# rail-berkeley/serl

Measured on AMD Instinct MI355X. Metric: learner grad-steps/sec (DrQ, bs256, 2x128x128 img), higher is better.
Workload: dtype f32 (trunk convs as split-fp16 MFMA x3, fp32 accumulate; <=1e-6 vs fp64); 1 GPU; async_drq_sim (DrQ, ResNet-10 frozen trunk, REDQ-10 critic); workload_key=drq, global_batch=256, per_gpu_batch=256, cameras=2, state_dim=24, act_dim=6, replay_capacity=200000, replay_fill=20000, parallelism=dp1, encoder=resnet-pretrained, trunk_passes_per_grad_step=2, trunk_arithmetic=f16x3, schedule=trunk(i+1) overlapped with update(i) on a 2nd stream; gather(i+2) on a 3rd

## Files before the change

### serl_amd/csrc/agent.hip

```cpp
#include <algorithm>
#include <cmath>
#include <cstdlib>
#include <cstring>
#include <string>
#include <vector>

#include "dense_layer.h"
#include "small_encoder.h"

using namespace serl;

namespace {

constexpr int kL = SERL_MAX_MLP_LAYERS;
inline int critic_smax(int layer) { return layer == 0 ? 4 : 2; }
inline int policy_smax(int layer) { return layer == 0 ? 8 : 4; }

struct Offs {
  long enc0, cam_stride;
  DenseLn cam, prop;
  DenseLn c[kL], a[kL];
  int nc, na;
  long c_hw, c_hb;
  long a_Wm, a_bm, a_Ws, a_bs;
// ... 216 lines not shown
    e.rstd = b.take<float>((long)c.n_cam * B);
    e.pxhat = b.take<float>(B * c.proprio_dim);
    e.prstd = b.take<float>(B);
    e.enc = nullptr; e.ld = 0;
  };
  enc(a->encP); enc(a->encT); enc(a->encO);
  float* encP_out = b.take<float>(B * a->E);
  a->encP.enc = encP_out; a->encP.ld = a->E;
  auto mlp = [&](MlpBuf& m, long rows, const serl_mlp_opts& net) {
    for (int j = 0; j < net.n_layers; ++j) {
      LayerBuf* l = &m.l[j];
      l->h = b.take<float>(rows * net.dims[j]); l->xhat = b.take<float>(rows * net.dims[j]); l->rstd = b.take<float>(rows);
    }
  };
  auto crit = [&](CritBuf& cb) {
    cb.x = b.take<float>(B * a->XA);
    mlp(cb.m, N * B, critic);
    cb.q = b.take<float>(N * B);
  };
  crit(a->critT); crit(a->crit);
  a->encT.enc = a->critT.x; a->encT.ld = a->XA;
  a->encO.enc = a->crit.x; a->encO.ld = a->XA;
  for (PolBuf* pbuf : {&a->pol, &a->polT}) {
    mlp(pbuf->m, B, policy);
    pbuf->pre = b.take<float>(2 * B * A); pbuf->std = b.take<float>(B * A); pbuf->logp = b.take<float>(B);
  }
  const long Bp = pad64(B);
  long cap = std::max<long>({(long)c.n_cam * 32 * Bp * c.bottleneck, N * Bp * pad64(a->XA), 8 * Bp * Wp, 4 * N * Bp * Wc, 16L * 64 * Hc});
  a->slabs_cap = cap;
  for (int k = 0; k < 3; ++k) a->slabs_lane[k] = b.take<float>(cap);
  a->slabs = a->slabs_lane[0];
  a->dq = b.take<float>(N * B); a->ytgt = b.take<float>(B);
  for (int j = std::max(critic.n_layers, policy.n_layers) - 1; j >= 0; --j) {
    const long n = std::max<long>(j < critic.n_layers ? N * B * critic.dims[j] : 0, j < policy.n_layers ? B * policy.dims[j] : 0);
    GradBuf* s = &a->s[j];
    s->dy = b.take<float>(n); s->dpre = b.take<float>(n); s->dg = b.take<float>(n);
  }
  a->dx = b.take<float>(B * a->XA);
  a->scam.dpre = b.take<float>((long)c.n_cam * B * c.bottleneck);
  a->scam.dg = b.take<float>((long)c.n_cam * B * c.bottleneck);
  a->df = b.take<float>((long)c.n_cam * B * a->D);
  a->sle_part = b.take<float>((long)c.n_cam * kSleSplit * a->HW * 512 * c.sle_features);
  a->sprop.dpre = b.take<float>(B * c.proprio_dim); a->sprop.dg = b.take<float>(B * c.proprio_dim);
  a->dpre = b.take<float>(2 * B * A); a->sprop.dy = b.take<float>(B * c.proprio_dim);
  for (int k = 0; k < 3; ++k) {
    a->eps_buf[k] = b.take<float>(B * A);
    a->mask_buf[k] = b.take<uint8_t>((long)c.n_cam * B * a->D);
  }
  a->act_tmp = b.take<float>(B * A);
  a->ctr = b.take<int>((long)kCtrPerLane * kCtrLanes);
  a->labels = b.take<float>(B); a->label_logits = b.take<float>(B); a->label_mean = b.take<float>(1);
  a->label_ctr = b.take<int>(1);
  a->eval_info = b.take<float>(8);
  if (a->small) {
    void* smem = b.take<uint8_t>(small_workspace_bytes(c.n_cam * c.batch, c.H, c.W, c.num_stack));
    if (base) small_workspace_bind(a->sws, smem, c.n_cam * c.batch, c.H, c.W, c.num_stack);
  } else if (!a->state_only) {
    const int nimg = 2 * c.n_cam * c.batch;
    void* tmem = b.take<uint8_t>(trunk_workspace_bytes(nimg, c.H, c.W));
    if (base) trunk_workspace_bind(a->tws, tmem, nimg, c.H, c.W);
    void* pmem = b.take<uint8_t>(trunk_packed_bytes());
    if (base) trunk_packed_bind(a->tpk, pmem);
    if (a->live) {
      static_assert(sizeof(a->feats_t_slot) / sizeof(a->feats_t_slot[0]) == serl_agent::kSlots + 1, "one target-feature buffer per slot");
      void* pmem_t = b.take<uint8_t>(trunk_packed_bytes());
      if (base) trunk_packed_bind(a->tpk_t, pmem_t);
      for (int k = 0; k <= serl_agent::kSlots; ++k) a->feats_t_slot[k] = b.take<float>((long)c.n_cam * B * a->HW * 512);
      a->feats_t = a->feats_t_slot[0];
    }
  }
  (void)persistent;
  return b.off;
}

int split_for(long agent_budget, int M, int N, int groups, int smax, long budget = 0) {
  if (budget <= 0) budget = agent_budget > 0 ? agent_budget : 512L;
  return split_under(M, N, groups, smax, budget);
}

struct EncJob {
  const float* P;
  int which;
  const uint8_t* mask;
  EncBuf* e;
  const float* act_src;
  float* act_dst;
  int gen_mask = 0;
  uint64_t mask_seed = 0;
  const uint32_t* tf_key = nullptr; long tf_rows = 0, tf_row0 = 0;
  const float* x = nullptr;
};
DenseLnIo cam_io(const serl_agent* a, const EncBuf& e) {
  return DenseLnIo{e.f, a->D, (long)a->cfg.batch * a->D, e.enc, e.ld, a->cfg.bottleneck, e.xhat, e.rstd};
}
DenseLnIo prop_io(const serl_agent* a, const EncBuf& e, const float* state) {
  return DenseLnIo{state, a->cfg.state_dim, 0, e.enc + (long)a->cfg.n_cam * a->cfg.bottleneck, e.ld, 0, e.pxhat, e.prstd};
}
int encode_multi(serl_agent* a, const EncJob* jobs, int n, int off, int cnt, hipStream_t st) {
  const serl_agent_cfg& c = a->cfg;
  const Offs& o = a->o;
  const long Bfull = a->cur.batch;
  SERL_REQUIRE(n >= 1 && n <= 3, "bad encode instance count");
  if (a->state_only) {
    CopyJob cj[kMaxMulti];
    int m = 0;
    for (int i = 0; i < n; ++i) {
      const EncJob& j = jobs[i];
      cj[m++] = CopyJob{a->cur.state + ((long)j.which * Bfull + off) * c.state_dim, c.state_dim, j.e->enc, j.e->ld, c.state_dim};
      if (j.act_dst) cj[m++] = CopyJob{j.act_src, c.act_dim, j.act_dst, a->XA, c.act_dim};
    }
    return copy_cols_multi(cj, m, cnt, st);
  }
  SleFwdArgs sv[3];
  GemmDesc gd[3];
  LnFwdArgs lv[3];
  ProprioArgs pv[3];
  const int S = split_for(a->split_budget, cnt, c.bottleneck, c.n_cam * n, 32);
  for (int i = 0; i < n; ++i) {
    const EncJob& j = jobs[i];
    EncBuf& e = *j.e;
    sv[i] = SleFwdArgs{};
    sv[i].x = (j.x ? j.x : a->feats + ((long)j.which * c.n_cam) * c.batch * a->HW * 512) + (long)off * a->HW * 512;
    sv[i].K = j.P + o.enc0;
    sv[i].mask = j.mask ? j.mask + (long)off * a->D : nullptr;
    sv[i].f = e.f;
    gd[i] = layer_fwd(o.cam, j.P, cam_io(a, e), cnt, a->slabs_lane[i], S);
    lv[i] = layer_ln_fwd(o.cam, j.P, cam_io(a, e), cnt, gd[i]);
    ProprioArgs& pr = pv[i];
    pr = layer_row_fwd(o.prop, j.P, prop_io(a, e, a->cur.state + ((long)j.which * Bfull + off) * c.state_dim));
    if (j.act_dst) {
      pr.copy_src = j.act_src; pr.ld_copy_src = c.act_dim; pr.copy_dst = j.act_dst; pr.ld_copy_dst = a->XA;
      pr.copy_cols = c.act_dim;
    }
  }
  if (a->fuse) {
    for (int i = 0; i < n; ++i) {
      sv[i].gen = jobs[i].gen_mask; sv[i].seed = jobs[i].mask_seed;
      sv[i].row_offset = a->shard_off + off; sv[i].rows_global = a->shard_global ? a->shard_global : Bfull;
      if (jobs[i].gen_mask == 2) sle_tf_masks(sv[i], jobs[i].tf_key, c.n_cam, jobs[i].tf_rows, jobs[i].tf_row0);
    }
  }
  if (a->small) {
    const size_t fbytes = (size_t)c.H * c.W * 3;
    for (int i = 0; i < n; ++i) {
      const EncJob& j = jobs[i];
      int dup = -1;
      for (int k = i + 1; k < n; ++k)
        if (jobs[k].P == j.P && jobs[k].which == j.which) dup = k;
      if (dup >= 0) { gd[i].A = jobs[dup].e->f; continue; }
      const uint8_t* fr = a->cur.frames + (((size_t)j.which * c.n_cam) * Bfull + off) * c.num_stack * fbytes;
      RC(small_forward(a->sws, j.P, o.enc0, o.cam_stride, fr, Bfull, c.n_cam, cnt, j.e->f, (long)c.batch * a->D, st));
    }
  } else if (a->fuse) {
    RC(sle_proprio_fwd_multi(sv, pv, n, 1.0f - c.dropout, cnt, a->HW, 512, c.n_cam, (long)c.batch * a->HW * 512, o.cam_stride,
                             Bfull * a->D, (long)c.batch * a->D, c.state_dim, st));
  } else {
    RC(sle_fwd_multi(sv, n, 1.0f / (1.0f - c.dropout), cnt, a->HW, 512, c.n_cam, (long)c.batch * a->HW * 512, o.cam_stride,
                     Bfull * a->D, (long)c.batch * a->D, st));
  }
  RC(gemm_f32_multi(gd, n, st));
  RC(ln_fwd_multi(lv, n, c.bottleneck, st));
  if (a->fuse && !a->small) return SERL_OK;
  return proprio_fwd_multi(pv, n, c.state_dim, cnt, st);
}

DenseLnIo mlp_io(const DenseLn& L, const float* x, long ldx, const LayerBuf& b, int rows) {
  return DenseLnIo{x, ldx, 0, b.h, L.N, (long)rows * L.N, b.xhat, b.rstd};
}
DenseLnIo mlp_io(const DenseLn& L, const LayerBuf& below, const LayerBuf& b, int rows) {
  return DenseLnIo{below.h, L.K, L.groups > 1 ? (long)rows * L.K : 0, b.h, L.N, (long)rows * L.N, b.xhat, b.rstd};
}
DenseLnGrad mlp_grad(const DenseLn& L, const GradBuf& s, int rows, bool dy_here = true) {
  return DenseLnGrad{dy_here ? s.dy : nullptr, L.N, (long)rows * L.N, s.dpre, s.dg};
}

struct RowDot { const float *w, *b; float* out; long w_gs, b_gs; };
struct LayerJob { const float* P; DenseLnIo t; RowDot dot; DenseLnDrop drop; };
int dense_ln_multi(serl_agent* a, const DenseLn& L, const LayerJob* jobs, int n, int rows, int smax, hipStream_t st) {
  SERL_REQUIRE(n >= 1 && n <= 3, "bad dense instance count");
  const int splitk = split_for(a->split_budget, rows, L.N, L.groups * n, smax);
  SERL_REQUIRE((long)L.groups * splitk * rows * L.N <= a->slabs_cap,
               "Dense layer: %d groups x %d K-splits x %d rows x width %d exceeds the slab scratch of %ld floats", L.groups, splitk,
               rows, L.N, a->slabs_cap);
  GemmDesc gd[3];
  LnFwdArgs lv[3];
  for (int i = 0; i < n; ++i) {
    const LayerJob& j = jobs[i];
    gd[i] = layer_fwd(L, j.P, j.t, rows, a->slabs_lane[i], splitk);
    lv[i] = layer_ln_fwd(L, j.P, j.t, rows, gd[i], j.drop);
    lv[i].dot_w = j.dot.w; lv[i].dot_b = j.dot.b; lv[i].dot_out = j.dot.out;
    lv[i].dot_gstride = j.dot.w_gs; lv[i].dot_b_gstride = j.dot.b_gs;
  }
  RC(gemm_f32_multi(gd, n, st));
  return ln_fwd_multi(lv, n, L.N, st);
}

struct PolJob {
  const float* P; PolBuf* pb;
  const float* enc; long ld_enc;
  const float* eps;
  float* act_out; long ld_act;
  float* sum_logp;
  float* alpha_out;
  float* eps_out = nullptr; uint64_t eps_seed = 0; long eps_row0 = 0;
  const uint32_t* tf_key = nullptr; long tf_rows = 0, tf_row0 = 0;
  DenseLnDrop drop[kL] = {};
};
int policy_mlp_multi(serl_agent* a, const PolJob* jobs, int n, int cnt, hipStream_t st) {
  const Offs& o = a->o;
  for (int l = 0; l < o.na; ++l) {
    LayerJob d[3];
    for (int i = 0; i < n; ++i) {
      const PolJob& j = jobs[i];
      MlpBuf& m = j.pb->m;
      d[i] = LayerJob{j.P, l ? mlp_io(o.a[l], m.l[l - 1], m.l[l], cnt) : mlp_io(o.a[0], j.enc, j.ld_enc, m.l[0], cnt), {}, j.drop[l]};
    }
    RC(dense_ln_multi(a, o.a[l], d, n, cnt, policy_smax(l), st));
  }
  return SERL_OK;
}
inline long head_stride(const serl_agent* a) { return a->o.a_bs >= 0 ? a->o.a_bs - a->o.a_bm : a->cfg.act_dim; }
inline const float* head_bias_ls(const serl_agent* a, const float* P) { return a->o.a_bs >= 0 ? P + a->o.a_bs : a->fixed_std_dev; }
int policy_fwd_multi(serl_agent* a, const PolJob* jobs, int n, int cnt, hipStream_t st) {
  const serl_agent_cfg& c = a->cfg;
  const Offs& o = a->o;
  const int Hd = o.a[o.na - 1].N, A = c.act_dim;
  SERL_REQUIRE(n >= 1 && n <= 3, "bad policy instance count");
  GemmDesc gd[3];
  PolicyDistArgs pv[3];
  for (int i = 0; i < n; ++i) {
    const PolJob& j = jobs[i];
    const float* P = j.P;
    PolBuf& pb = *j.pb;
    gd[i] = gemm_fwd(pb.m.l[o.na - 1].h, Hd, 0, P + o.a_Wm, head_stride(a), a->slabs_lane[i], a->head_groups, cnt, A, Hd, 4);
    pv[i] = PolicyDistArgs{};
    pv[i].mode = a->pol_mode;
    pv[i].slabs = a->slabs_lane[i]; pv[i].S = 4; pv[i].bias_mean = P + o.a_bm; pv[i].bias_ls = head_bias_ls(a, P); pv[i].pre = pb.pre;
    pv[i].eps = j.eps; pv[i].act = j.act_out; pv[i].ld_act = j.ld_act; pv[i].logp = pb.logp; pv[i].std_out = pb.std;
    pv[i].sum_logp = j.sum_logp; pv[i].lam = P + o.lam; pv[i].alpha_out = j.alpha_out;
  }
  RC(policy_mlp_multi(a, jobs, n, cnt, st));
  if (a->fuse) {
    SERL_REQUIRE(A <= 64, "the fused policy-head epilogue holds one 64-wide slab row per sample (act_dim %d)", A);
    SERL_REQUIRE(cdiv(cnt, 64) <= kCtrPerLane && 8 * pad64(cnt) * 64 <= a->slabs_cap, "policy head exceeds the fused epilogue's scratch");
    for (int i = 0; i < n; ++i) {
      const PolJob& j = jobs[i];
      GemmDesc& g = gd[i];
      g.ldc = 64; g.sCz = pad64(cnt) * 64;
      g.epi = kEpiPolicy; g.ctr = a->ctr + (long)i * kCtrPerLane;
      g.pd = pv[i];
      g.pd.sum_logp = nullptr;
      g.pd.eps_out = j.eps_out; g.pd.seed = j.eps_seed; g.pd.row_offset = j.eps_row0;
      g.pd.tf = j.tf_key ? 1 : 0;
      if (j.tf_key) { g.pd.tf_key[0] = j.tf_key[0]; g.pd.tf_key[1] = j.tf_key[1]; g.pd.tf_rows = j.tf_rows; g.pd.tf_row0 = j.tf_row0; }
      g.pd.B = cnt; g.pd.A = A; g.pd.std_min = c.std_min; g.pd.std_max = c.std_max;
      g.pd.slab_ld = g.ldc; g.pd.slab_stride = g.sCz;
      SERL_REQUIRE(j.eps || j.eps_out, "policy noise: neither draws nor a buffer for hashed ones");
      if (j.sum_logp) {
        SERL_REQUIRE(a->pg_defer && a->pg_ncs < kMaxColsum, "no room for the log-prob sum job");
        a->pg_cs[a->pg_ncs++] = Colsum3Args{j.pb->logp, nullptr, nullptr, 1, cnt, 1, nullptr, j.sum_logp, nullptr, 0, 2};
      }
    }
    return gemm_f32_multi(gd, n, st);
  }
  RC(gemm_f32_multi(gd, n, st));
  return policy_dist_fwd_multi(pv, n, cnt, A, c.std_min, c.std_max, st);
}

struct CritJob { const float* P; CritBuf* cb; DenseLnDrop drop[kL]; };
int critic_fwd_multi(serl_agent* a, const CritJob* jobs, int n, int cnt, hipStream_t st) {
  const Offs& o = a->o;
  SERL_REQUIRE(n >= 1 && n <= 3, "bad critic instance count");
  for (int l = 0; l < o.nc; ++l) {
    LayerJob d[3];
    for (int i = 0; i < n; ++i) {
      const float* P = jobs[i].P;
      CritBuf& cb = *jobs[i].cb;
      d[i] = LayerJob{P, l ? mlp_io(o.c[l], cb.m.l[l - 1], cb.m.l[l], cnt) : mlp_io(o.c[0], cb.x, a->XA, cb.m.l[0], cnt), {}, jobs[i].drop[l]};
      if (l == o.nc - 1)
        d[i].dot = RowDot{P + o.c_hw, P + o.c_hb, cb.q, a->state_only ? o.c[l].N : 0, a->state_only ? 1 : 0};
    }
    RC(dense_ln_multi(a, o.c[l], d, n, cnt, critic_smax(l), st));
  }
  return SERL_OK;
}

int flush_param_grads(serl_agent* a, hipStream_t st) {
  if (a->pg_ncs) RC(colsum3_multi(a->pg_cs, a->pg_ncs, st));
  if (a->pg_nwg) RC(gemm_f32_multi(a->pg_wg, a->pg_nwg, st));
  a->pg_ncs = a->pg_nwg = 0;
  return SERL_OK;
}

int wgrad(serl_agent* a, const GemmDesc& g, hipStream_t st) {
  if (a->pg_defer && a->pg_nwg < kMaxGemmGroups) {
    a->pg_wg[a->pg_nwg++] = g;
    return SERL_OK;
  }
  return gemm_f32(g, st);
}

struct HeadDq {
  const float* dq; const float* w; float dq_const; long w_gs; const LossArgs* loss;
};
int dense_ln_bwd(serl_agent* a, const DenseLn& L, const float* P, const DenseLnIo& t, const DenseLnGrad& d, int rows, float* G,
                 hipStream_t st, const HeadDq* head = nullptr, const DenseLnDrop& site = DenseLnDrop{}) {
  LnBwdArgs l = layer_ln_bwd(L, P, t, d, rows, site);
  if (head) { l.dq = head->dq; l.dq_w = head->w; l.dq_const = head->dq_const; l.dq_w_gstride = head->w_gs; }
  if (head && head->loss) {
    l.dq_inline = 1;
    RC(ln_bwd_multi(&l, 1, *head->loss, st));
  } else {
    RC(ln_bwd(l, st));
  }
  if (!G) return SERL_OK;
  const Colsum3Args cs = layer_colsum(L, t, d, rows, G);
  if (a->pg_defer && a->pg_ncs < kMaxColsum) a->pg_cs[a->pg_ncs++] = cs;
  else RC(colsum3_multi(&cs, 1, st));
  return wgrad(a, layer_wgrad(L, t, d, rows, G), st);
}


int igrad_sum(serl_agent* a, GemmDesc g, float* out, long ldo, hipStream_t st) {
  const int groups = g.nbatch, rows = g.M, Kin = g.N;
  g.C = a->slabs;
  if (!a->fuse) {
    g.ldc = Kin; g.sCz = (long)rows * Kin;
    RC(gemm_f32(g, st));
    return reduce_slabs(a->slabs, groups, (long)rows * Kin, 1, rows, Kin, nullptr, 0, out, ldo, 0, false, st);
  }
  g.ldc = pad64(Kin); g.sCz = pad64(rows) * g.ldc;
  g.epi = kEpiReduce; g.zred = groups; g.ctr = a->ctr; g.out = out; g.ld_out = ldo; g.out_gstride = 0;
  SERL_REQUIRE((long)cdiv(rows, 64) * cdiv(Kin, 64) <= kCtrPerLane && groups * g.sCz <= a->slabs_cap,
               "input gradient: %d groups x %d rows x %d columns exceeds the fused epilogue's slab scratch of %ld floats, or its tiles the %d "
               "arrival counters", groups, rows, Kin, a->slabs_cap, kCtrPerLane);
  return gemm_f32(g, st);
}

int head_kernel_grad(serl_agent* a, CritBuf& cb, int cnt, hipStream_t st) {
  const int Hd = a->o.c[a->o.nc - 1].N, N = a->cfg.ensemble;
  const int groups = a->state_only ? N : 1, K = a->state_only ? cnt : N * cnt, split = K <= 1024 ? 1 : (a->state_only ? 4 : 8);
  float* out = a->Gc + a->o.c_hw;
  GemmDesc g{};
  g.A = a->dq; g.sAm = a->fuse ? 1 : 0; g.sAk = 1; g.sAb = a->state_only ? cnt : 0;
  g.B = cb.m.l[a->o.nc - 1].h; g.sBk = Hd; g.sBn = 1; g.sBb = a->state_only ? (long)cnt * Hd : 0;
  g.C = split == 1 ? out : a->slabs; g.ldc = Hd; g.sCz = Hd;
  g.M = 1; g.N = Hd; g.K = K; g.nbatch = groups; g.splitk = split;
  if (!a->fuse) {
    RC(gemm_f32(g, st));
    return split == 1 ? SERL_OK : reduce_slabs(a->slabs, split, Hd, groups, 1, Hd, nullptr, 0, out, Hd, a->state_only ? Hd : 0, false, st);
  }
  if (split > 1) {
    g.sCz = 64L * Hd;
    g.epi = kEpiReduce; g.zred = split; g.ctr = a->ctr; g.out = out; g.ld_out = Hd; g.out_gstride = Hd;
    SERL_REQUIRE((long)groups * split * g.sCz <= a->slabs_cap && groups * cdiv(Hd, 64) <= kCtrPerLane,
                 "head gradient: %d groups x %d K-splits x 64 rows x width %d exceeds the slab scratch of %ld floats, or its %d tiles the %d "
                 "arrival counters", groups, split, Hd, a->slabs_cap, groups * cdiv(Hd, 64), kCtrPerLane);
  }
  SERL_REQUIRE(a->pg_defer && a->pg_nwg < kMaxGemmGroups, "no room for the deferred head-gradient GEMM");
  a->pg_wg[a->pg_nwg++] = g;
  return SERL_OK;
}

int critic_loss_or_rider(serl_agent* a, const LossArgs& L, hipStream_t st, const LossArgs** rider) {
  *rider = nullptr;
  if (a->fuse) { *rider = &L; return SERL_OK; }
  return critic_loss(L.qt, L.q, L.reward, L.mask, L.sel, L.E, L.B, L.discount, L.inv_norm, L.y_out, L.dq, L.scalars, L.dbias, st,
                     L.per_member != 0, L.logp_next, L.alpha);
}

int head_bias_grad(serl_agent* a, int cnt, float* out, long out_gstride, hipStream_t st) {
  const int A = a->cfg.act_dim;
  const int groups = a->opts.std_param == SERL_STD_FIXED ? 1 : 2;
  if (!a->fuse) return colsum(a->dpre, nullptr, groups, cnt, A, out, out_gstride, false, st);
  SERL_REQUIRE(a->pg_ncs < kMaxColsum, "no room for the head-bias gradient job");
  a->pg_cs[a->pg_ncs++] = Colsum3Args{a->dpre, nullptr, nullptr, groups, cnt, A, nullptr, out, nullptr, out_gstride, 1};
  return SERL_OK;
}

int critic_bwd(serl_agent* a, const float* P, CritBuf& cb, int cnt, bool pg, hipStream_t st, const LossArgs* loss, float dq_const,
               const DenseLnDrop* sites) {
  const Offs& o = a->o;
  float* G = pg ? a->Gc : nullptr;
  const LossArgs* rider = nullptr;
  if (loss) RC(critic_loss_or_rider(a, *loss, st, &rider));
  if (pg) RC(head_kernel_grad(a, cb, cnt, st));
  const int top = o.nc - 1;
  const HeadDq head{loss ? loss->dq : nullptr, P + o.c_hw, dq_const, a->state_only ? o.c[top].N : 0, rider};
  for (int l = top; l >= 0; --l) {
    const DenseLnGrad d = mlp_grad(o.c[l], a->s[l], cnt, l != top);
    const DenseLnIo t = l ? mlp_io(o.c[l], cb.m.l[l - 1], cb.m.l[l], cnt) : mlp_io(o.c[0], cb.x, a->XA, cb.m.l[0], cnt);
    RC(dense_ln_bwd(a, o.c[l], P, t, d, cnt, G, st, l == top ? &head : nullptr, sites[l]));
    if (l) RC(gemm_f32(layer_igrad(o.c[l], P, d, cnt, mlp_grad(o.c[l - 1], a->s[l - 1], cnt)), st));
    else return igrad_sum(a, layer_igrad(o.c[0], P, d, cnt, nullptr, 0, 0), a->dx, a->XA, st);
  }
  return SERL_OK;
}

int enc_bwd_critic(serl_agent* a, const float* P, EncBuf& e, int off, int cnt, hipStream_t st, void* event_bucket0) {
  const serl_agent_cfg& c = a->cfg;
  const Offs& o = a->o;
  const DenseLnIo tc = cam_io(a, e), tp = prop_io(a, e, a->cur.state + (long)off * c.state_dim);
  const DenseLnGrad dc{a->dx, a->XA, o.cam.N, a->scam.dpre, a->scam.dg};
  const DenseLnGrad dp{a->dx + (long)c.n_cam * o.cam.N, a->XA, 0, a->sprop.dpre, a->sprop.dg};
  if (a->fuse && !a->state_only) {
    LnBwdArgs lb[2] = {layer_ln_bwd(o.cam, P, tc, dc, cnt), layer_ln_bwd(o.prop, P, tp, dp, cnt)};
    RC(ln_bwd_multi(lb, 2, LossArgs{}, st));
    SERL_REQUIRE(a->pg_defer && a->pg_ncs + 2 <= kMaxColsum, "no room for the deferred LayerNorm gradients");
    a->pg_cs[a->pg_ncs++] = layer_colsum(o.prop, tp, dp, cnt, a->Gc);
    a->pg_cs[a->pg_ncs++] = layer_colsum(o.cam, tc, dc, cnt, a->Gc);
    RC(wgrad(a, layer_wgrad(o.prop, tp, dp, cnt, a->Gc), st));
  } else if (!a->state_only) {
    RC(dense_ln_bwd(a, o.prop, P, tp, dp, cnt, a->Gc, st));
  }
  if (event_bucket0) {
    RC(flush_param_grads(a, st));
    SERL_HIP(hipEventRecord((hipEvent_t)event_bucket0, st));
  }
  if (a->state_only) return SERL_OK;
  if (a->fuse) RC(wgrad(a, layer_wgrad(o.cam, tc, dc, cnt, a->Gc), st));
  else RC(dense_ln_bwd(a, o.cam, P, tc, dc, cnt, a->Gc, st));
  RC(gemm_f32(layer_igrad(o.cam, P, dc, cnt, a->df, a->D, (long)cnt * a->D), st));
  if (a->small)
    return small_backward(a->sws, P, o.enc0, o.cam_stride, c.n_cam, cnt, a->df, (long)cnt * a->D, a->Gc, st);
  const long sle_n = (long)a->HW * 512 * c.sle_features;
  const float* x = a->feats + (long)off * a->HW * 512;
  if (a->fuse) {
    SERL_REQUIRE((long)c.n_cam * a->HW * 2 <= kCtrPerLane, "SLE gradient exceeds the arrival counters");
    return sle_bwd_fused(x, a->df, a->sle_part, cnt, a->HW, 512, kSleSplit, c.n_cam, (long)c.batch * a->HW * 512, (long)cnt * a->D,
                         (long)kSleSplit * sle_n, a->Gc + o.enc0, o.cam_stride, a->ctr, st);
  }
  RC(sle_bwd(x, a->df, a->sle_part, cnt, a->HW, 512, kSleSplit, c.n_cam, (long)c.batch * a->HW * 512,
             (long)cnt * a->D, (long)kSleSplit * sle_n, st));
  return reduce_slabs(a->sle_part, kSleSplit, sle_n, c.n_cam, 1, (int)sle_n, nullptr, 0, a->Gc + o.enc0, sle_n,
                      o.cam_stride, false, st);
}

static long tf_row0_of(const serl_agent* a, int cnt) {
  return a->shard_global ? (a->shard_off * (long)cnt) / std::max<long>(a->cur.batch, 1) : 0;
}

struct PhaseNoise {
  const float* eps; float* eps_out;
  const uint32_t* tf_eps; uint64_t eps_seed;
  const uint8_t* mask; uint8_t* mask_out;
  int gen_mask; const uint32_t* tf_mask; uint64_t mask_seed;
};
PhaseNoise draw_noise(serl_agent* a, const float* given_eps, const uint8_t* given_mask, int slot, const uint32_t* key_eps,
                      const uint32_t* key_mask) {
  const serl_agent_cfg& c = a->cfg;
  PhaseNoise z{};
  z.eps = given_eps; z.eps_out = a->eps_buf[slot];
  z.mask_out = a->mask_buf[slot];
  if (!given_eps) {
    if (key_eps) z.tf_eps = key_eps;
    else z.eps_seed = c.seed ^ (0xA5A5ull + 7919ull * (++a->noise_ctr));
  }
  if (given_mask || a->state_only || a->small) z.mask = a->small ? nullptr : given_mask;
  else if (key_mask) { z.gen_mask = 2; z.tf_mask = key_mask; }
  else { z.gen_mask = 1; z.mask_seed = c.seed ^ (0x5A5Aull + 104729ull * (++a->noise_ctr)); }
  return z;
}
int materialise_noise(serl_agent* a, PhaseNoise* v, int n, int off, int cnt, long global_count, hipStream_t st) {
  if (a->fuse) return SERL_OK;
  const serl_agent_cfg& c = a->cfg;
  const long rows = a->cur.batch, row0 = tf_row0_of(a, cnt);
  NoiseJob gen[kMaxMulti];
  int ngen = 0;
  for (int i = 0; i < n; ++i) {
    PhaseNoise& z = v[i];
    serl_jax_job jobs[1 + SERL_MAX_CAMS];
    int nj = 0;
    if (!z.eps && z.tf_eps) {
      serl_jax_job& j = jobs[nj++];
      j = serl_jax_job{};
      j.key[0] = z.tf_eps[0]; j.key[1] = z.tf_eps[1]; j.kind = SERL_JAX_NORMAL;
      j.n_total = global_count * c.act_dim; j.first = row0 * c.act_dim; j.count = (long)cnt * c.act_dim;
      j.out = z.eps_out + (long)off * c.act_dim;
    } else if (!z.eps) {
      gen[ngen++] = NoiseJob{z.eps_out, rows * c.act_dim, z.eps_seed, 0, 0.f, rows, a->shard_global, a->shard_off, c.act_dim};
    }
    for (int k = 0; k < c.n_cam && z.gen_mask == 2; ++k) {
      serl_jax_job& j = jobs[nj++];
      j = serl_jax_job{};
      j.key[0] = z.tf_mask[2 * k]; j.key[1] = z.tf_mask[2 * k + 1]; j.kind = SERL_JAX_BERNOULLI_U8; j.p = 1.0f - c.dropout;
      j.n_total = global_count * a->D; j.first = row0 * a->D; j.count = (long)cnt * a->D;
      j.out = z.mask_out + ((long)k * rows + off) * a->D;
    }
    if (z.gen_mask == 1)
      gen[ngen++] = NoiseJob{z.mask_out, (long)c.n_cam * rows * a->D, z.mask_seed, 1, 1.0f - c.dropout, rows, a->shard_global, a->shard_off, a->D};
    if (nj) RC(serl_jax_fill(c.device, jobs, nj, (void*)st));
    z = PhaseNoise{z.eps ? z.eps : z.eps_out, z.eps_out, nullptr, 0, z.gen_mask ? z.mask_out : z.mask, z.mask_out, 0, nullptr, 0};
  }
  return ngen ? gen_noise_multi(gen, ngen, st) : SERL_OK;
}
void set_noise(const serl_agent* a, EncJob& e, PolJob& p, const PhaseNoise& z, long off, int cnt, long global_count) {
  const int A = a->cfg.act_dim;
  const long tf_row0 = tf_row0_of(a, cnt);
  e.mask = z.mask; e.gen_mask = z.gen_mask; e.mask_seed = z.mask_seed;
  e.tf_key = z.tf_mask; e.tf_rows = global_count; e.tf_row0 = tf_row0;
  p.eps = z.eps ? z.eps + off * A : nullptr;
  p.eps_out = z.eps_out + off * A; p.eps_seed = z.eps_seed; p.eps_row0 = a->shard_off + off;
  p.tf_key = z.tf_eps; p.tf_rows = global_count; p.tf_row0 = tf_row0;
}

void mlp_sites(serl_agent* a, int site, double rate, int off, int cnt, long global_count, int key_row, DenseLnDrop (&out)[kL]) {
  for (DenseLnDrop& d : out) d = DenseLnDrop{};
  if (!(rate > 0.0)) return;
  const serl_mlp_noise& z = a->mlp_cur;
  const bool critic = site == SERL_SITE_Q_TARGET || site == SERL_SITE_Q_ONLINE || site == SERL_SITE_Q_ACTOR;
  const serl_mlp_opts& net = critic ? a->opts.critic : a->opts.policy;
  const int* dims = net.dims;
  const int n = net.n_layers;
  long below = 0;
  for (int l = 0; l < n; below += dims[l], ++l) {
    DenseLnDrop& d = out[l];
    d.train = 1;
    if (z.mask[site]) d.mask = z.mask[site] + below * a->cur.batch + (long)off * dims[l];
    else if (z.key[site]) { d.key = z.key[site] + ((long)key_row * n + l) * 2; d.key_rows = global_count; d.key_row0 = tf_row0_of(a, cnt); }
    else { d.seed = a->cfg.seed ^ (0xD0D0ull + 15485863ull * (++a->noise_ctr)); d.hash_row0 = a->shard_off + off; }
  }
}
int mlp_masks_fit(const serl_agent* a) {
  for (int s = 0; s < SERL_MLP_SITES; ++s)
    SERL_REQUIRE(!a->mlp_cur.mask[s] || a->mlp_cur.mask_rows == a->cur.batch,
                 "serl_mlp_noise: the masks of site %d hold %d rows per layer, the batch has %d", s, a->mlp_cur.mask_rows, a->cur.batch);
  return SERL_OK;
}
struct MlpNoiseScope {
  serl_agent* a;
  explicit MlpNoiseScope(serl_agent* a_) : a(a_) {
    if (a && a->mlp_depth++ == 0) { a->mlp_cur = a->mlp_bound; a->mlp_bound = serl_mlp_noise{}; }
  }
  ~MlpNoiseScope() {
    if (a && --a->mlp_depth == 0) a->mlp_cur = serl_mlp_noise{};
  }
};

float lr_at(const serl_agent_cfg& c, int64_t count, int tx) {
  const float peak = (c.tx_lr_set[tx] || c.tx_lr[tx] > 0.f) ? c.tx_lr[tx] : c.lr;
  int warm = (tx == SERL_TX_TEMPERATURE && c.temp_warmup_steps >= 0) ? c.temp_warmup_steps : c.warmup_steps;
  if (c.tx_warmup[tx] > 0) warm = c.tx_warmup[tx] - 1;
  if (count < warm) return (float)((double)peak * (double)count / (double)warm);
  if (c.tx_cosine_steps[tx] > 0) {
    const double T = (double)std::max(c.tx_cosine_steps[tx] - warm, 1);
    const double k = std::min((double)(count - warm), T);
    return (float)((double)peak * 0.5 * (1.0 + std::cos(M_PI * k / T)));
// ... 479 lines not shown
}

static int check_label_fresh(serl_agent* a) {
  if (!a->cls) return SERL_OK;
  const bool mine = a->trunk_gen != a->attach_gen, theirs = classifier_view(a->cls).trunk_gen != a->attach_cls_gen;
  if (mine || theirs) {
    set_error("stale reward-classifier attachment: a trunk leaf of the %s was set after serl_agent_set_reward_classifier; attach again",
              mine ? "agent" : "classifier");
    return SERL_ERR_STATE;
  }
  return SERL_OK;
}

int serl_agent_set_reward_classifier(serl_agent* a, serl_classifier* cls, const int* cam_of, int* mode_out) {
  SERL_REQUIRE(a, "NULL agent");
  if (!cls) {
    a->cls = nullptr;
    a->label_mode = SERL_LABEL_NONE;
    a->labelled = false;
    if (mode_out) *mode_out = SERL_LABEL_NONE;
    return SERL_OK;
  }
  SERL_REQUIRE(cam_of, "NULL camera map");
  const serl_agent_cfg& c = a->cfg;
  SERL_REQUIRE(!a->state_only, "a state-only agent has no frames for a reward classifier to label");
  SERL_REQUIRE(c.num_stack == 1, "the reward classifier reads single frames (its pretrained conv_init takes 3 channels): an agent with num_stack %d "
               "cannot be labelled by it", c.num_stack);
  const ClassifierView v = classifier_view(cls);
  SERL_REQUIRE(v.cfg.device == c.device, "the classifier lives on device %d, the agent on %d", v.cfg.device, c.device);
  for (int k = 0; k < v.cfg.n_cam; ++k)
    SERL_REQUIRE(cam_of[k] >= 0 && cam_of[k] < c.n_cam, "classifier camera %d maps to agent camera %d, the agent has %d", k, cam_of[k], c.n_cam);
  SERL_REQUIRE(v.cfg.H == c.H && v.cfg.W == c.W, "the classifier takes %dx%d images, the agent %dx%d", v.cfg.H, v.cfg.W, c.H, c.W);
  SERL_REQUIRE(v.cfg.max_batch >= c.batch, "classifier max_batch %d is below the agent's batch %d", v.cfg.max_batch, c.batch);
  SERL_HIP(hipSetDevice(c.device));
  int mode = SERL_LABEL_FRAMES;
  if (!a->small && !a->live && v.trunk_count == a->trunk_count) {
    SERL_HIP(hipDeviceSynchronize());
    std::vector<float> mine(a->trunk_count), theirs(a->trunk_count);
    SERL_HIP(hipMemcpy(mine.data(), a->trunk, sizeof(float) * mine.size(), hipMemcpyDeviceToHost));
    SERL_HIP(hipMemcpy(theirs.data(), v.trunk, sizeof(float) * theirs.size(), hipMemcpyDeviceToHost));
    if (std::memcmp(mine.data(), theirs.data(), sizeof(float) * mine.size()) == 0) mode = SERL_LABEL_FEATURES;
  }
  a->cls = cls;
  for (int k = 0; k < v.cfg.n_cam; ++k) a->cls_cam[k] = cam_of[k];
  a->label_mode = mode;
  a->attach_gen = a->trunk_gen;
  a->attach_cls_gen = v.trunk_gen;
  a->labelled = false;
  if (mode_out) *mode_out = mode;
  return SERL_OK;
}

int serl_agent_label_rewards(serl_agent* a, void* stream) {
  SERL_REQUIRE(a && a->has_batch, "serl_agent_encode / serl_agent_select_slot must run first");
  if (!a->cls) {
    set_error("no reward classifier is attached (serl_agent_set_reward_classifier)");
    return SERL_ERR_STATE;
  }
  RC(check_label_fresh(a));
  const serl_agent_cfg& c = a->cfg;
  hipStream_t st = (hipStream_t)stream;
  SERL_HIP(hipSetDevice(c.device));
  const int n = a->cur.batch, nc = classifier_view(a->cls).cfg.n_cam;
  SERL_HIP(hipMemsetAsync(a->label_ctr, 0, sizeof(int), st));
  if (a->label_mode == SERL_LABEL_FEATURES) {
    const long cam_stride = (long)c.batch * a->HW * 512;
    RC(classifier_label(a->cls, a->feats + c.n_cam * cam_stride, cam_stride, a->cls_cam, nullptr, n, a->labels, a->label_logits,
                        a->label_mean, a->label_ctr, st));
  } else {
    const size_t fbytes = (size_t)c.H * c.W * 3;
    const uint8_t* cams[SERL_MAX_CAMS];
    for (int k = 0; k < nc; ++k) cams[k] = a->cur.frames + ((size_t)(c.n_cam + a->cls_cam[k]) * n) * fbytes;
    RC(classifier_label(a->cls, nullptr, 0, nullptr, cams, n, a->labels, a->label_logits, a->label_mean, a->label_ctr, st));
  }
  a->label_n = n;
  a->labelled = true;
  return SERL_OK;
}

int serl_agent_reward_label_rows(serl_agent* a) { return a ? a->label_n : -1; }

int serl_agent_read_reward_labels(serl_agent* a, float* host_labels, float* host_logits, float* mean_out, void* stream) {
  SERL_REQUIRE(a, "NULL agent");
  SERL_REQUIRE(a->label_n > 0, "no rewards were labelled yet");
  hipStream_t st = (hipStream_t)stream;
  SERL_HIP(hipSetDevice(a->cfg.device));
  const size_t bytes = sizeof(float) * a->label_n;
  if (host_labels) SERL_HIP(hipMemcpyAsync(host_labels, a->labels, bytes, hipMemcpyDeviceToHost, st));
  if (host_logits) SERL_HIP(hipMemcpyAsync(host_logits, a->label_logits, bytes, hipMemcpyDeviceToHost, st));
  if (mean_out) SERL_HIP(hipMemcpyAsync(mean_out, a->label_mean, sizeof(float), hipMemcpyDeviceToHost, st));
  SERL_HIP(hipStreamSynchronize(st));
  return SERL_OK;
}

int serl_agent_critic_grads(serl_agent* a, int off, int cnt, int global_count, const serl_noise* noise,
                            int redq_row, void* stream) {
  return serl_agent_critic_grads_bucketed(a, off, cnt, global_count, noise, redq_row, stream, nullptr);
}

int serl_agent_grad_bucket(serl_agent* a, int bucket, float** dev_ptr, int64_t* count) {
  SERL_REQUIRE(a && dev_ptr && count, "NULL argument");
  SERL_REQUIRE(bucket == 0 || bucket == 1, "bucket must be 0 or 1");
  const Offs& o = a->o;
  if (bucket == 0) { *dev_ptr = a->Gc + o.c[0].W; *count = (o.Pc - o.c[0].W) + kScalars; }
  else { *dev_ptr = a->Gc; *count = o.c[0].W; }
  return SERL_OK;
}

int serl_agent_critic_grads_bucketed(serl_agent* a, int off, int cnt, int global_count, const serl_noise* noise,
                                     int redq_row, void* stream, void* event_bucket0) {
  MlpNoiseScope mlp_scope(a);
  SERL_REQUIRE(a && a->has_batch, "serl_agent_encode must run first");
  SERL_REQUIRE(off >= 0 && cnt >= 1 && off + cnt <= a->cur.batch && global_count >= cnt, "bad minibatch range");
  RC(mlp_masks_fit(a));
  if (a->cls && !a->labelled && !a->label_exempt) {
    set_error("a reward classifier is attached: serl_agent_label_rewards must follow serl_agent_select_slot (vice.py:594)");
    return SERL_ERR_STATE;
  }
  const serl_agent_cfg& c = a->cfg;
  const Offs& o = a->o;
  hipStream_t st = (hipStream_t)stream;
  SERL_HIP(hipSetDevice(c.device));
  const int m_sub = c.critic_subsample_size == 0 ? 2 : (c.critic_subsample_size < 0 ? 0 : c.critic_subsample_size);
  SERL_REQUIRE(m_sub <= 16, "critic_subsample_size %d exceeds 16", m_sub);
  RedqSel sel{};
  sel.n = m_sub;
  if (noise && noise->redq_idx) {
    for (int k = 0; k < m_sub; ++k) sel.idx[k] = noise->redq_idx[m_sub * redq_row + k];
  } else {
    uint64_t r = c.seed * 0x9E3779B97F4A7C15ull + (++a->noise_ctr) * 0xBF58476D1CE4E5B9ull;
    for (int k = 0; k < m_sub; ++k) {
      r ^= r >> 29; r *= 0x94D049BB133111EBull; r ^= r >> 32;
      sel.idx[k] = (int)(r % c.ensemble);
      r += 0x9E3779B97F4A7C15ull;
    }
  }
  for (int k = 0; k < m_sub; ++k) SERL_REQUIRE(sel.idx[k] >= 0 && sel.idx[k] < c.ensemble, "REDQ index out of range");
  a->pg_ncs = a->pg_nwg = 0;
  a->pg_defer = true;
  const int A = c.act_dim;
  PhaseNoise nz = draw_noise(a, noise ? noise->eps_next : nullptr, noise ? noise->mask_next : nullptr, 0,
                             noise && noise->key_eps_next ? noise->key_eps_next + 2 * redq_row : nullptr,
                             noise && noise->key_mask_next ? noise->key_mask_next + 2 * c.n_cam * redq_row : nullptr);
  RC(materialise_noise(a, &nz, 1, off, cnt, global_count, st));
  RC(live_features(a, off, cnt, true, st));
  EncJob ej[3] = {{a->theta, 1, nullptr, &a->encP, nullptr, nullptr},
                  {a->theta_t, 1, nullptr, &a->encT, nullptr, nullptr},
                  {a->theta, 0, nullptr, &a->encO, a->cur.action + (long)off * A, a->crit.x + a->E}};
  if (a->live) ej[1].x = a->feats_t;
  PolJob pj{a->theta, &a->pol, a->encP.enc, a->encP.ld, nullptr, a->critT.x + a->E, a->XA, nullptr,
            c.backup_entropy ? a->aux + X_ALPHA : nullptr};
  set_noise(a, ej[0], pj, nz, off, cnt, global_count);
  CritJob cj[2] = {{a->theta_t, &a->critT, {}}, {a->theta, &a->crit, {}}};
  mlp_sites(a, SERL_SITE_PI_NEXT, a->opts.policy.dropout, off, cnt, global_count, redq_row, pj.drop);
  mlp_sites(a, SERL_SITE_Q_TARGET, a->opts.critic.dropout, off, cnt, global_count, redq_row, cj[0].drop);
  mlp_sites(a, SERL_SITE_Q_ONLINE, a->opts.critic.dropout, off, cnt, global_count, redq_row, cj[1].drop);
  RC(encode_multi(a, ej, 3, off, cnt, st));
  RC(policy_fwd_multi(a, &pj, 1, cnt, st));
  RC(critic_fwd_multi(a, cj, 2, cnt, st));
  const float* reward = a->labelled ? a->labels : a->cur.reward;
  const LossArgs L{1, a->critT.q, a->crit.q, reward + off, a->cur.mask + off, sel, c.ensemble, cnt, c.discount,
                   1.0f / ((float)c.ensemble * (float)global_count), a->ytgt, a->dq, a->SC, a->Gc + o.c_hb, a->state_only ? 1 : 0,
                   c.backup_entropy ? a->pol.logp : nullptr, c.backup_entropy ? a->aux + X_ALPHA : nullptr};
  SERL_REQUIRE(!a->state_only || c.ensemble <= 16, "per-member head bias supports ensembles of at most 16");
  RC(critic_bwd(a, a->theta, a->crit, cnt, true, st, &L, 0.f, cj[1].drop));
  RC(enc_bwd_critic(a, a->theta, a->encO, off, cnt, st, event_bucket0));
  RC(flush_param_grads(a, st));
  a->last_global = global_count;
  return SERL_OK;
}

int serl_agent_actor_grads(serl_agent* a, int global_count, const serl_noise* noise, void* stream) {
  MlpNoiseScope mlp_scope(a);
  SERL_REQUIRE(a && a->has_batch, "serl_agent_encode must run first");
  const serl_agent_cfg& c = a->cfg;
  const Offs& o = a->o;
  hipStream_t st = (hipStream_t)stream;
  SERL_HIP(hipSetDevice(c.device));
  const int cnt = a->cur.batch, A = c.act_dim, top = o.na - 1, Hd = o.a[top].N;
  SERL_REQUIRE(global_count >= cnt, "global_count < local batch");
  RC(mlp_masks_fit(a));
  a->pg_ncs = a->pg_nwg = 0;
  a->pg_defer = true;
  enum { PI = 0, TEMP = 1 };
  PhaseNoise nz[2] = {draw_noise(a, noise ? noise->eps_pi : nullptr, noise ? noise->mask_obs_pi : nullptr, 1,
                                 noise ? noise->key_eps_pi : nullptr, noise ? noise->key_mask_obs_pi : nullptr),
                      draw_noise(a, noise ? noise->eps_temp : nullptr, noise ? noise->mask_next_temp : nullptr, 2,
                                 noise ? noise->key_eps_temp : nullptr, noise ? noise->key_mask_next_temp : nullptr)};
  RC(materialise_noise(a, nz, 2, 0, cnt, global_count, st));
  RC(live_features(a, 0, cnt, false, st));
  EncJob ej[3] = {{a->theta, 1, nullptr, &a->encT, nullptr, nullptr},
                  {a->theta, 0, nullptr, &a->encO, nullptr, nullptr},
                  {a->theta, 0, nullptr, &a->encP, nullptr, nullptr}};
  PolJob pj[2] = {{a->theta, &a->polT, a->encT.enc, a->encT.ld, nullptr, a->act_tmp, A, a->SC + S_LOGP_NEXT, a->aux + X_ALPHA},
                  {a->theta, &a->pol, a->encP.enc, a->encP.ld, nullptr, a->crit.x + a->E, a->XA, a->SC + S_LOGP, nullptr}};
  set_noise(a, ej[0], pj[0], nz[TEMP], 0, cnt, global_count);
  set_noise(a, ej[2], pj[1], nz[PI], 0, cnt, global_count);
  CritJob cj{a->theta, &a->crit, {}};
  mlp_sites(a, SERL_SITE_PI, a->opts.policy.dropout, 0, cnt, global_count, 0, pj[1].drop);
  mlp_sites(a, SERL_SITE_Q_ACTOR, a->opts.critic.dropout, 0, cnt, global_count, 0, cj.drop);
  mlp_sites(a, SERL_SITE_PI_TEMP, a->opts.policy.dropout, 0, cnt, global_count, 0, pj[0].drop);
  RC(encode_multi(a, ej, 3, 0, cnt, st));
  RC(policy_fwd_multi(a, pj, 2, cnt, st));
  const float* eps_pi = nz[PI].eps ? nz[PI].eps : nz[PI].eps_out;
  RC(critic_fwd_multi(a, &cj, 1, cnt, st));
  RC(critic_bwd(a, a->theta, a->crit, cnt, false, st, nullptr, -1.0f / ((float)c.ensemble * (float)global_count), cj.drop));
  RC(policy_dist_bwd(a->dx + a->E, a->XA, a->crit.x + a->E, a->XA, a->pol.pre, a->pol.std, eps_pi, a->aux + X_ALPHA,
                     1.0f / (float)global_count, cnt, A, c.std_min, c.std_max, a->dpre, a->crit.q, c.ensemble,
                     a->SC + S_QPI, st, a->pol_mode));
  const long hs = head_stride(a);
  const int hg = a->head_groups;
  float* Ga = a->Ga - o.Pa0;
  const float* P = a->theta;
  const MlpBuf& pm = a->pol.m;
  const auto io = [&](int l) { return l ? mlp_io(o.a[l], pm.l[l - 1], pm.l[l], cnt) : mlp_io(o.a[0], a->encP.enc, a->encP.ld, pm.l[0], cnt); };
  const DenseLnGrad dtop = mlp_grad(o.a[top], a->s[top], cnt), d1 = mlp_grad(o.a[0], a->s[0], cnt);
  RC(wgrad(a, gemm_wgrad(pm.l[top].h, Hd, 0, a->dpre, A, (long)cnt * A, Ga + o.a_Wm, A, hs, hg, Hd, A, cnt), st));
  RC(head_bias_grad(a, cnt, Ga + o.a_bm, hs, st));
  RC(igrad_sum(a, gemm_igrad(a->dpre, A, (long)cnt * A, P + o.a_Wm, A, hs, nullptr, 0, 0, hg, cnt, Hd, A), dtop.dy, dtop.ld_dy, st));
  for (int l = top; l >= 0; --l) {
    const DenseLnGrad d = mlp_grad(o.a[l], a->s[l], cnt);
    RC(dense_ln_bwd(a, o.a[l], P, io(l), d, cnt, Ga, st, nullptr, pj[1].drop[l]));
    if (l) RC(gemm_f32(layer_igrad(o.a[l], P, d, cnt, mlp_grad(o.a[l - 1], a->s[l - 1], cnt)), st));
  }
  if (!a->state_only) {
    const DenseLnGrad dp{a->sprop.dy, o.prop.N, 0, a->sprop.dpre, a->sprop.dg};
    RC(gemm_f32(gemm_igrad(d1.dpre, o.a[0].N, 0, P + o.a[0].W + (long)c.n_cam * o.cam.N * o.a[0].N, o.a[0].N, 0, dp.dy, dp.ld_dy, 0, 1, cnt,
                           o.prop.N, o.a[0].N), st));
    RC(dense_ln_bwd(a, o.prop, P, prop_io(a, a->encP, a->cur.state), dp, cnt, Ga, st));
  }
  RC(flush_param_grads(a, st));
  a->last_global = global_count;
  return SERL_OK;
}

int serl_agent_apply(serl_agent* a, int which, float info_weight, void* stream) {
  SERL_REQUIRE(a, "NULL agent");
  SERL_REQUIRE(which >= 1 && which <= 7, "bad `which` (a non-empty set of SERL_NET_* bits)");
  const serl_agent_cfg& c = a->cfg;
  const Offs& o = a->o;
  hipStream_t st = (hipStream_t)stream;
  SERL_HIP(hipSetDevice(c.device));
  const bool crit = which & SERL_NET_CRITIC, act = which & SERL_NET_ACTOR, temp = which & SERL_NET_TEMPERATURE;
  AdamArgs ad{};
  ad.theta = a->theta; ad.theta_target = a->theta_t;
  ad.P = o.P; ad.Pc = o.Pc; ad.Pa0 = o.Pa0; ad.Pa1 = o.Pa1;
  ad.g_critic = a->Gc; ad.g_actor = a->Ga;
  ad.m_c = a->m_c; ad.v_c = a->v_c; ad.m_a = a->m_a; ad.v_a = a->v_a; ad.m_t = a->m_t; ad.v_t = a->v_t;
  ad.sum_logp_next = a->SC + S_LOGP_NEXT; ad.temp_grad_out = a->aux + X_TGRAD;
  ad.critic_on = crit ? 1 : 0; ad.actor_on = act ? 1 : 0; ad.temp_on = temp ? 1 : 0;
  ad.ema_on = crit ? 1 : 0;
  ad.lr_a = lr_at(c, a->step, SERL_TX_ACTOR);
  ad.lr_c = lr_at(c, a->step, SERL_TX_CRITIC);
  ad.lr_t = lr_at(c, a->step, SERL_TX_TEMPERATURE);
  const int64_t t = a->step + 1;
  ad.bc1 = 1.0f - powf(0.9f, (float)t);
  ad.bc2 = 1.0f - powf(0.999f, (float)t);
  ad.tau = c.tau; ad.target_entropy = c.target_entropy;
  ad.inv_batch = a->last_global > 0 ? 1.0f / (float)a->last_global : 0.f;
  ad.frozen = a->trunk; ad.frozen_target = a->trunk_t; ad.n_frozen = a->trunk_count;
  if (!a->live && a->trunk_count > 0) {
    ad.n_frozen = 0;
    if (crit) a->trunk_ema_pending += 1;
  }
  ad.wd_a = c.tx_weight_decay_on[SERL_TX_ACTOR] ? c.tx_weight_decay[SERL_TX_ACTOR] : 0.f;
  ad.wd_c = c.tx_weight_decay_on[SERL_TX_CRITIC] ? c.tx_weight_decay[SERL_TX_CRITIC] : 0.f;
  ad.wd_t = c.tx_weight_decay_on[SERL_TX_TEMPERATURE] ? c.tx_weight_decay[SERL_TX_TEMPERATURE] : 0.f;
  ad.clip_a = c.tx_clip_norm[SERL_TX_ACTOR]; ad.clip_c = c.tx_clip_norm[SERL_TX_CRITIC]; ad.clip_t = c.tx_clip_norm[SERL_TX_TEMPERATURE];
  ad.norm2 = a->aux + X_NORM2;
  if ((ad.clip_c > 0.f && crit) || (ad.clip_a > 0.f && act))
    RC(grad_norm2(a->Gc, o.Pc, a->Ga, o.Pa1 - o.Pa0, a->aux + X_NORM2, st));
  ad.info_mode = (crit ? 1 : 0) | ((act || temp) ? 2 : 0);
  ad.info_reset = (crit && a->info_reset) ? 1 : 0;
  if (crit) a->info_reset = false;
  ad.scalars = a->SC; ad.alpha = a->aux + X_ALPHA; ad.info_acc = a->info_acc;
  ad.info_w = info_weight;
  ad.inv_eb = a->last_global > 0 ? 1.0f / ((float)c.ensemble * (float)a->last_global) : 0.f;
  RC(adam_ema(ad, st));
  if (a->live) {
    a->tpk.dirty = true; a->trunk_ver += 1;
    if (crit) { a->tpk_t.dirty = true; a->trunk_t_ver += 1; }
  }
  a->step += 1;
  a->lr_last[SERL_TX_ACTOR] = ad.lr_a; a->lr_last[SERL_TX_CRITIC] = ad.lr_c; a->lr_last[SERL_TX_TEMPERATURE] = ad.lr_t;
  return SERL_OK;
}

int serl_agent_grad_view(serl_agent* a, int which, float** dev_ptr, int64_t* count) {
  SERL_REQUIRE(a && dev_ptr && count, "NULL argument");
  SERL_REQUIRE(which >= 1 && which <= 7, "bad `which`");
  const Offs& o = a->o;
  const bool crit = which & SERL_NET_CRITIC, at = which & (SERL_NET_ACTOR | SERL_NET_TEMPERATURE);
  if (crit && at) { *dev_ptr = a->G; *count = o.Pc + kScalars + (o.Pa1 - o.Pa0); }
  else if (crit) { *dev_ptr = a->Gc; *count = o.Pc + kScalars; }
  else { *dev_ptr = a->SC; *count = kScalars + (o.Pa1 - o.Pa0); }
  return SERL_OK;
}

int serl_agent_update(serl_agent* a, const serl_batch* batch, int nets, const serl_noise* noise, void* stream) {
  MlpNoiseScope mlp_scope(a);
  SERL_REQUIRE(a && batch, "NULL argument");
  SERL_REQUIRE(nets >= 1 && nets <= 7, "Invalid gradient steps: %d", nets);
  RC(serl_agent_begin_update(a, stream));
  RC(serl_agent_encode(a, batch, stream));
  a->label_exempt = true;
  if (nets & SERL_NET_CRITIC) RC(serl_agent_critic_grads(a, 0, batch->batch, batch->batch, noise, 0, stream));
  if (nets & (SERL_NET_ACTOR | SERL_NET_TEMPERATURE)) RC(serl_agent_actor_grads(a, batch->batch, noise, stream));
  return serl_agent_apply(a, nets, 1.0f, stream);
}

int serl_agent_update_critics(serl_agent* a, const serl_batch* batch, const serl_noise* noise, void* stream) {
  MlpNoiseScope mlp_scope(a);
  SERL_REQUIRE(a, "NULL agent");
  RC(check_label_fresh(a));
  RC(serl_agent_begin_update(a, stream));
  RC(serl_agent_encode(a, batch, stream));
  if (a->cls) RC(serl_agent_label_rewards(a, stream));
  RC(serl_agent_critic_grads(a, 0, batch->batch, batch->batch, noise, 0, stream));
  return serl_agent_apply(a, SERL_APPLY_CRITIC, 1.0f, stream);
}

int serl_agent_update_high_utd(serl_agent* a, const serl_batch* batch, int utd_ratio, const serl_noise* noise,
                               void* stream) {
  MlpNoiseScope mlp_scope(a);
  SERL_REQUIRE(a && batch, "NULL argument");
  SERL_REQUIRE(utd_ratio >= 1 && batch->batch % utd_ratio == 0,
               "Batch size %d must be divisible by UTD ratio %d", batch->batch, utd_ratio);
  RC(check_label_fresh(a));
  RC(serl_agent_begin_update(a, stream));
  RC(serl_agent_encode(a, batch, stream));
  if (a->cls) RC(serl_agent_label_rewards(a, stream));
  const int mb = batch->batch / utd_ratio;
  for (int i = 0; i < utd_ratio; ++i) {
    RC(serl_agent_critic_grads(a, i * mb, mb, mb, noise, i, stream));
    RC(serl_agent_apply(a, SERL_APPLY_CRITIC, 1.0f / (float)utd_ratio, stream));
  }
  RC(serl_agent_actor_grads(a, batch->batch, noise, stream));
  return serl_agent_apply(a, SERL_APPLY_ACTOR_TEMP, 1.0f, stream);
}

int serl_agent_read_info(serl_agent* a, serl_info* out, void* stream) {
  SERL_REQUIRE(a && out, "NULL argument");
  SERL_HIP(hipSetDevice(a->cfg.device));
  float acc[I_N];
  SERL_HIP(hipMemcpyAsync(acc, a->info_acc, sizeof(acc), hipMemcpyDeviceToHost, (hipStream_t)stream));
  SERL_HIP(hipStreamSynchronize((hipStream_t)stream));
  out->critic_loss = acc[I_CL]; out->predicted_qs = acc[I_PQ]; out->target_qs = acc[I_TQ];
  out->actor_loss = acc[I_AL]; out->temperature = acc[I_TEMP]; out->entropy = acc[I_ENT];
  out->temperature_loss = acc[I_TL];
  out->actor_lr = a->lr_last[SERL_TX_ACTOR]; out->critic_lr = a->lr_last[SERL_TX_CRITIC];
  out->temperature_lr = a->lr_last[SERL_TX_TEMPERATURE];
  return SERL_OK;
}

struct EvalScope {
  serl_agent* a;
  serl_batch cur; bool has_batch, labelled, label_exempt; float* feats; int last_global; uint64_t noise_ctr;
  float* feats_t; serl_agent::FeatRows feats_on, feats_tg;
  explicit EvalScope(serl_agent* a_)
// ... 230 lines not shown
```

### serl_amd/csrc/bc.hip

```cpp
#include <cmath>
#include <string>
#include <vector>

#include "dense_layer.h"
#include "jaxrng.h"

using namespace serl;

namespace {
constexpr int kHidden = 256, kBottleneck = 256, kSleFeatures = 8, kProprio = 64, kMaxAct = 64;
}

struct serl_bc {
  serl_bc_cfg cfg{};
  int HW = 0, D = 0, Eimg = 0, E = 0;
  std::vector<Leaf> leaves;
  long n_params = 0, t0 = 0, nt = 0;
  TrunkOffsets to{};
  CamHeadOffsets cam{};
  DenseLn prop{};
  long o_w1 = 0, o_b1 = 0, o_w2 = 0, o_b2 = 0, o_Wm = 0, o_bm = 0, o_Ws = 0, o_bs = 0;
  void* arena = nullptr;
  float* params = nullptr;
  AdamSlice opt{};
// ... 33 lines not shown
  c->o_bs = add_leaf(L, off, "actor/logstd/bias", A);
  c->nt = off - c->t0;
  c->n_params = off;
}

size_t carve(serl_bc* c, uint8_t* base) {
  const serl_bc_cfg& g = c->cfg;
  Bump b(base);
  const long n = g.max_batch, A = g.act_dim;
  c->params = b.take<float>(c->n_params + 1);
  c->opt.carve(b, c->t0, c->nt);
  c->info = b.take<float>(2);
  uint8_t* pk = b.take<uint8_t>(trunk_packed_bytes());
  uint8_t* ws = b.take<uint8_t>(trunk_workspace_bytes(g.n_cam * g.max_batch, g.H, g.W));
  c->feats = b.take<float>((size_t)g.n_cam * n * c->HW * 512);
  c->f = b.take<float>((size_t)g.n_cam * n * c->D);
  c->slabs_cap = (long)std::max(32 * g.n_cam, 8) * n * kBottleneck;
  c->slabs = b.take<float>(c->slabs_cap);
  c->enc = b.take<float>(n * c->E);
  c->pxhat = b.take<float>(n * kProprio);
  c->prstd = b.take<float>(n);
  c->h1 = b.take<float>(n * kHidden);
  c->h2 = b.take<float>(n * kHidden);
  c->mu = b.take<float>(n * A);
  c->dhead = b.take<float>(2 * n * A);
  c->dpre1 = b.take<float>(n * kHidden);
  c->dpre2 = b.take<float>(n * kHidden);
  c->dprop = b.take<float>(n * kProprio);
  c->dpp = b.take<float>(n * kProprio);
  c->dgp = b.take<float>(n * kProprio);
  if (base) {
    trunk_packed_bind(c->tpk, pk);
    trunk_workspace_bind(c->tws, ws, g.n_cam * g.max_batch, g.H, g.W);
    c->tw = trunk_weights(c->params, c->to);
  }
  return b.off;
}

__global__ __launch_bounds__(256) void bc_dense_tanh_fwd_kernel(const float* slabs, int S, long sstride, const float* bias,
                                                                 float* y, int rows, int N) {
  const long e = (long)blockIdx.x * 256 + threadIdx.x;
  if (e >= (long)rows * N) return;
  const int col = (int)(e % N);
  float acc = 0.f;
  for (int s = 0; s < S; ++s) acc += slabs[(long)s * sstride + e];
  y[e] = tanhf(acc + bias[col]);
}

__global__ __launch_bounds__(256) void bc_dense_tanh_bwd_kernel(const float* slabs, int S, long sstride, const float* y,
                                                                 float* dpre, int rows, int N) {
  const long e = (long)blockIdx.x * 256 + threadIdx.x;
  if (e >= (long)rows * N) return;
  float acc = 0.f;
  for (int s = 0; s < S; ++s) acc += slabs[(long)s * sstride + e];
  const float t = y[e];
  dpre[e] = acc * (1.f - t * t);
}

struct BcHeadArgs {
  const float* slabs; int S; long sstride;
  const float *bias_m, *bias_s;
  int B, A; float std_min, std_max, temp;
  const float* action;
  float* mu;
  float *logp, *mse;
  float *dmu, *dls;
  float* info;
  float* act; const float* eps;
  int sample, tf; uint32_t tf_key[2];
};
__global__ __launch_bounds__(256) void bc_gauss_head_kernel(BcHeadArgs a) {
  __shared__ float red[2][256];
  const int tid = threadIdx.x;
  const float half_log_2pi = 0.918938533204672742f;
  const float sq = sqrtf(a.temp);
  float s_lp = 0.f, s_mse = 0.f;
  for (int b = tid; b < a.B; b += 256) {
    float lp = 0.f, se = 0.f;
    for (int j = 0; j < a.A; ++j) {
      const long e = (long)b * a.A + j;
      float pm = 0.f, ps = 0.f;
      for (int s = 0; s < a.S; ++s) {
        pm += a.slabs[(long)s * a.sstride + e];
        ps += a.slabs[(long)(a.S + s) * a.sstride + e];
      }
      const float mean = pm + a.bias_m[j], ls = ps + a.bias_s[j];
      const float raw = expf(ls);
      const float sd = fminf(fmaxf(raw, a.std_min), a.std_max) * sq;
      if (a.mu) a.mu[e] = mean;
      if (a.act) {
        float out = mean;
        if (a.sample) {
          const float z = a.tf ? normal_from_bits(random_bits_at(a.tf_key[0], a.tf_key[1], (uint64_t)a.B * a.A, (uint64_t)e)) : a.eps[e];
          out = mean + sd * z;
        }
        a.act[e] = out;
      }
      if (a.action) {
        const float d = a.action[e] - mean;
        const float z = d / sd;
        lp += -0.5f * z * z - logf(sd) - half_log_2pi;
        se += d * d;
        if (a.dmu) a.dmu[e] = -(z / sd) / (float)a.B;
        if (a.dls) a.dls[e] = (raw > a.std_min && raw < a.std_max) ? -(z * z - 1.f) / (float)a.B : 0.f;
      }
    }
    if (a.action) {
      if (a.logp) a.logp[b] = lp;
      if (a.mse) a.mse[b] = se;
      s_lp += lp;
      s_mse += se;
    }
  }
  if (!a.info) return;
  red[0][tid] = s_lp;
  red[1][tid] = s_mse;
  __syncthreads();
  for (int o = 128; o > 0; o >>= 1) {
    if (tid < o) { red[0][tid] += red[0][tid + o]; red[1][tid] += red[1][tid + o]; }
    __syncthreads();
  }
  if (tid == 0) {
    a.info[0] = -red[0][0] / (float)a.B;
    a.info[1] = red[1][0] / (float)a.B;
  }
}

int dense_tanh_fwd(const float* slabs, int S, long sstride, const float* bias, float* y, int rows, int N, hipStream_t st) {
  hipLaunchKernelGGL(bc_dense_tanh_fwd_kernel, dim3(cdiv((long)rows * N, 256)), dim3(256), 0, st, slabs, S, sstride, bias, y, rows, N);
  SERL_HIP(hipGetLastError());
  return SERL_OK;
}

int dense_tanh_bwd(const float* slabs, int S, long sstride, const float* y, float* dpre, int rows, int N, hipStream_t st) {
  hipLaunchKernelGGL(bc_dense_tanh_bwd_kernel, dim3(cdiv((long)rows * N, 256)), dim3(256), 0, st, slabs, S, sstride, y, dpre, rows, N);
  SERL_HIP(hipGetLastError());
  return SERL_OK;
}

DenseLnIo prop_io(const serl_bc* c, const float* state) {
  return DenseLnIo{state, c->cfg.state_dim, 0, c->enc + c->Eimg, c->E, 0, c->pxhat, c->prstd};
}

int forward(serl_bc* c, const uint8_t* frames, const float* state, int n, const uint8_t* mask, const uint32_t* mask_keys,
            int* head_split, hipStream_t st) {
  const serl_bc_cfg& g = c->cfg;
  const float* P = c->params;
  const int A = g.act_dim;
  RC(trunk_forward(c->tw, c->tws, frames, g.n_cam * n, c->feats, st, &c->tpk));
  SleFwdArgs sv{};
  sv.x = c->feats; sv.K = P + c->cam.first; sv.mask = mask; sv.f = c->f;
  if (!mask && mask_keys) sle_tf_masks(sv, mask_keys, g.n_cam, n, 0);
  const ProprioArgs pv = layer_row_fwd(c->prop, P, prop_io(c, state));
  RC(sle_proprio_fwd_multi(&sv, &pv, 1, 1.0f - g.dropout, n, c->HW, 512, g.n_cam, (long)n * c->HW * 512, c->cam.stride,
                           (long)n * c->D, (long)n * c->D, g.state_dim, st));
  const int S0 = split_under(n, kBottleneck, g.n_cam, 32);
  const DenseLnIo tc{c->f, c->D, (long)n * c->D, c->enc, c->E, kBottleneck, nullptr, nullptr};
  const GemmDesc g0 = layer_fwd(c->cam.dense, P, tc, n, c->slabs, S0);
  const LnFwdArgs l0 = layer_ln_fwd(c->cam.dense, P, tc, n, g0);
  RC(gemm_f32_multi(&g0, 1, st));
  RC(ln_fwd_multi(&l0, 1, kBottleneck, st));
  const int S1 = split_under(n, kHidden, 1, 8);
  const GemmDesc g1 = gemm_fwd(c->enc, c->E, 0, P + c->o_w1, 0, c->slabs, 1, n, kHidden, c->E, S1);
  RC(gemm_f32_multi(&g1, 1, st));
  RC(dense_tanh_fwd(c->slabs, S1, g1.sCz, P + c->o_b1, c->h1, n, kHidden, st));
  const int S2 = split_under(n, kHidden, 1, 4);
  const GemmDesc g2 = gemm_fwd(c->h1, kHidden, 0, P + c->o_w2, 0, c->slabs, 1, n, kHidden, kHidden, S2);
  RC(gemm_f32_multi(&g2, 1, st));
  RC(dense_tanh_fwd(c->slabs, S2, g2.sCz, P + c->o_b2, c->h2, n, kHidden, st));
  const int S3 = 4;
  const GemmDesc g3 = gemm_fwd(c->h2, kHidden, 0, P + c->o_Wm, c->o_Ws - c->o_Wm, c->slabs, 2, n, A, kHidden, S3);
  RC(gemm_f32_multi(&g3, 1, st));
  *head_split = S3;
  return SERL_OK;
}

BcHeadArgs head_args(serl_bc* c, int n, int S) {
  BcHeadArgs h{};
  h.slabs = c->slabs; h.S = S; h.sstride = (long)n * c->cfg.act_dim;
  h.bias_m = c->params + c->o_bm; h.bias_s = c->params + c->o_bs;
  h.B = n; h.A = c->cfg.act_dim; h.std_min = c->cfg.std_min; h.std_max = c->cfg.std_max; h.temp = 1.0f;
  return h;
}

int launch_head(const BcHeadArgs& h, hipStream_t st) {
  hipLaunchKernelGGL(bc_gauss_head_kernel, dim3(1), dim3(256), 0, st, h);
  SERL_HIP(hipGetLastError());
  return SERL_OK;
}

int check_batch(serl_bc* c, const serl_batch* b) {
  const serl_bc_cfg& g = c->cfg;
  SERL_REQUIRE(b && b->frames && b->state && b->action, "serl_batch has NULL members");
  SERL_REQUIRE(b->batch >= 1 && b->batch <= g.max_batch, "batch %d not in [1,%d]", b->batch, g.max_batch);
  SERL_REQUIRE(b->n_cam == g.n_cam && b->H == g.H && b->W == g.W && b->C == 3 && b->state_dim == g.state_dim &&
                   b->act_dim == g.act_dim, "serl_batch shape does not match the BC agent");
  SERL_REQUIRE(b->num_stack <= 1, "the BC agent takes single-frame observations (serl_batch.num_stack %d)", b->num_stack);
  return SERL_OK;
}

int resolve(serl_bc* c, const char* section, const char* leaf, float** ptr, long* count) {
  const Leaf* l = find(c->leaves, leaf);
  SERL_REQUIRE(l, "unknown BC leaf '%s'", leaf);
  *count = l->count;
  if (std::string(section) == "params") { *ptr = c->params + l->off; return SERL_OK; }
  SERL_REQUIRE(c->opt.moment(section, *l, ptr), "unknown BC section '%s' (params, opt/mu, opt/nu)", section);
  return SERL_OK;
}

}

extern "C" {

int serl_bc_create(const serl_bc_cfg* cfg, serl_bc** out) {
  SERL_REQUIRE(cfg && out, "NULL argument");
  SERL_REQUIRE(cfg->n_cam >= 1 && cfg->n_cam <= SERL_MAX_CAMS, "n_cam %d not in [1,%d]", cfg->n_cam, SERL_MAX_CAMS);
  SERL_REQUIRE(cfg->H >= 32 && cfg->W >= 32 && cfg->max_batch >= 1, "bad BC shape");
  SERL_REQUIRE(cfg->state_dim >= 1 && cfg->act_dim >= 1 && cfg->act_dim <= kMaxAct, "state_dim %d / act_dim %d unsupported",
               cfg->state_dim, cfg->act_dim);
  SERL_REQUIRE(cfg->dropout >= 0.f && cfg->dropout < 1.f && cfg->std_min > 0.f && cfg->std_max > cfg->std_min, "bad BC hyper-parameters");
  SERL_HIP(hipSetDevice(cfg->device));
  serl_bc* c = new serl_bc();
  c->cfg = *cfg;
  layout(c);
  if (int rc = alloc_zeroed(&c->arena, carve(c, nullptr), "BC arena")) {
    delete c;
    return rc;
  }
  carve(c, (uint8_t*)c->arena);
  *out = c;
  return SERL_OK;
}

int serl_bc_destroy(serl_bc* c) {
  if (!c) return SERL_OK;
  if (c->arena) (void)hipFree(c->arena);
  delete c;
  return SERL_OK;
}

int serl_bc_num_leaves(serl_bc* c) { return c ? (int)c->leaves.size() : 0; }

int serl_bc_leaf_info(serl_bc* c, int i, char* name_out, int name_cap, int64_t* count, int* trainable) {
  SERL_REQUIRE(c && i >= 0 && i < (int)c->leaves.size(), "leaf index %d out of range", i);
  const Leaf& l = c->leaves[i];
  if (name_out && name_cap > 0) snprintf(name_out, name_cap, "%s", l.name.c_str());
  if (count) *count = l.count;
  if (trainable) *trainable = l.off >= c->t0 ? 1 : 0;
  return SERL_OK;
}

int serl_bc_set(serl_bc* c, const char* section, const char* leaf, const float* host, int64_t count) {
  SERL_REQUIRE(c && section && leaf && host, "NULL argument");
  float* p = nullptr;
  long n = 0;
  RC(resolve(c, section, leaf, &p, &n));
  SERL_REQUIRE(count == n, "leaf '%s' has %ld elements, got %ld", leaf, n, (long)count);
  SERL_HIP(hipSetDevice(c->cfg.device));
  RC(leaf_copy(p, host, n, hipMemcpyHostToDevice, section, leaf, kFrozenMoment));
  if (std::string(leaf).rfind("trunk/", 0) == 0 && std::string(section) == "params") c->tpk.dirty = true;
  return SERL_OK;
}

int serl_bc_get(serl_bc* c, const char* section, const char* leaf, float* host_out, int64_t count) {
  SERL_REQUIRE(c && section && leaf && host_out, "NULL argument");
  float* p = nullptr;
  long n = 0;
  RC(resolve(c, section, leaf, &p, &n));
  SERL_REQUIRE(count == n, "leaf '%s' has %ld elements, got %ld", leaf, n, (long)count);
  SERL_HIP(hipSetDevice(c->cfg.device));
  return leaf_copy(host_out, p, n, hipMemcpyDeviceToHost, section, leaf, kFrozenMoment);
}

int serl_bc_set_step(serl_bc* c, int64_t step) {
  SERL_REQUIRE(c && step >= 0, "bad step");
  c->opt.step = step;
  return SERL_OK;
}

int64_t serl_bc_get_step(serl_bc* c) { return c ? c->opt.step : -1; }

int serl_bc_update(serl_bc* c, const serl_batch* batch, const uint8_t* dev_masks, const uint32_t* host_mask_keys, void* stream) {
  SERL_REQUIRE(c, "NULL BC agent");
  RC(check_batch(c, batch));
  SERL_REQUIRE(dev_masks || host_mask_keys, "the Dropout of the update needs keep-masks or jax.random keys");
  const serl_bc_cfg& g = c->cfg;
  SERL_HIP(hipSetDevice(g.device));
  hipStream_t st = (hipStream_t)stream;
  const int n = batch->batch, A = g.act_dim;
  const float* P = c->params;
  float* G = c->opt.grad();
  int S3 = 0;
  RC(forward(c, batch->frames, batch->state, n, dev_masks, host_mask_keys, &S3, st));
  BcHeadArgs h = head_args(c, n, S3);
  h.action = batch->action; h.mu = c->mu;
  h.dmu = c->dhead; h.dls = c->dhead + (long)n * A; h.info = c->info;
  RC(launch_head(h, st));
  const GemmDesc gh = gemm_igrad(c->dhead, A, (long)n * A, P + c->o_Wm, A, c->o_Ws - c->o_Wm, c->slabs, kHidden, (long)n * kHidden, 2, n, kHidden, A);
  RC(gemm_f32_multi(&gh, 1, st));
  RC(dense_tanh_bwd(c->slabs, 2, gh.sCz, c->h2, c->dpre2, n, kHidden, st));
  const int S2 = split_under(n, kHidden, 1, 4);
  const GemmDesc gd = gemm_igrad(c->dpre2, kHidden, 0, P + c->o_w2, kHidden, 0, c->slabs, kHidden, (long)n * kHidden, 1, n, kHidden, kHidden, S2);
  RC(gemm_f32_multi(&gd, 1, st));
  RC(dense_tanh_bwd(c->slabs, S2, gd.sCz, c->h1, c->dpre1, n, kHidden, st));
  const GemmDesc gp = gemm_igrad(c->dpre1, kHidden, 0, P + c->o_w1 + (long)c->Eimg * kHidden, kHidden, 0, c->dprop, kProprio, 0, 1, n, kProprio, kHidden);
  RC(gemm_f32_multi(&gp, 1, st));
  const DenseLnIo tp = prop_io(c, batch->state);
// ... 67 lines not shown
```

### serl_amd/csrc/classifier.hip

```cpp
#include <algorithm>
#include <cmath>
#include <string>
#include <vector>

#include "dense_layer.h"
#include "jaxrng.h"
#include "ln_stats.h"

using namespace serl;

namespace {
constexpr int kHidden = 256, kBottleneck = 256, kSleFeatures = 8, kSleSplit = 8;

struct ClsTrain {
  int max_batch = 0;
  float lr = 0.f;
  void* arena = nullptr;
  AdamSlice opt{};
  float *info = nullptr;
  TrunkWorkspace tws{};
  float *feats = nullptr;
  float *f = nullptr;
  float *slabs = nullptr;
  float *enc = nullptr;
// ... 259 lines not shown
  const bool train = inst == 0;
  const float* sl = a.slabs + inst * a.istride + (long)row * kHidden;
  float v[4];
  bool keep[4];
#pragma unroll
  for (int j = 0; j < 4; ++j) {
    const int col = lane * 4 + j;
    float x = a.b1[col];
    for (int s = 0; s < a.S; ++s) x += sl[(long)s * a.sstride + col];
    keep[j] = true;
    if (train) {
      const long e = (long)row * kHidden + col;
      keep[j] = a.mask ? a.mask[e] != 0
                       : (a.gen ? bits_to_unit(random_bits_at(a.key[0], a.key[1], (uint64_t)a.n * kHidden, (uint64_t)e)) < a.keep : true);
      x = keep[j] ? x / a.keep : 0.f;
    }
    v[j] = x;
  }
  float s1 = 0.f, s2 = 0.f;
#pragma unroll
  for (int j = 0; j < 4; ++j) { s1 += v[j]; s2 += v[j] * v[j]; }
  wave_sum2(s1, s2);
  float mean, rstd;
  ln_mean_rstd<kHidden>(s1, s2, mean, rstd);
  float xh[4], pre[4], h[4], d = 0.f;
#pragma unroll
  for (int j = 0; j < 4; ++j) {
    const int col = lane * 4 + j;
    xh[j] = (v[j] - mean) * rstd;
    pre[j] = xh[j] * a.g1[col] + a.be1[col];
    h[j] = fmaxf(pre[j], 0.f);
    d += h[j] * a.w2[col];
  }
#pragma unroll
  for (int off = 1; off < 64; off <<= 1) d += __shfl_xor(d, off);
  const float logit = d + a.b2[0];
  if (lane == 0) a.logits[(long)inst * a.n + row] = logit;
  if (!a.labels) return;
  const float y = a.labels[row];
  const float p = 1.f / (1.f + expf(-logit));
  if (!train) {
    if (lane == 0) a.rowcorr[row] = ((p >= 0.5f ? 1.f : 0.f) == y) ? 1.f : 0.f;
    return;
  }
  const float dl = (p - y) / (float)a.n;
  if (lane == 0) {
    a.rowloss[row] = y * cls_softplus(-logit) + (1.f - y) * cls_softplus(logit);
    a.dlogit[row] = dl;
  }
  float dA[4], dxh[4];
  s1 = 0.f; s2 = 0.f;
#pragma unroll
  for (int j = 0; j < 4; ++j) {
    const int col = lane * 4 + j;
    dA[j] = pre[j] > 0.f ? dl * a.w2[col] : 0.f;
    dxh[j] = dA[j] * a.g1[col];
    s1 += dxh[j];
    s2 += dxh[j] * xh[j];
  }
  wave_sum2(s1, s2);
  const float m1 = s1 * (1.0f / kHidden), m2 = s2 * (1.0f / kHidden);
#pragma unroll
  for (int j = 0; j < 4; ++j) {
    const long e = (long)row * kHidden + lane * 4 + j;
    const float dx = rstd * (dxh[j] - m1 - xh[j] * m2);
    a.dz[e] = keep[j] ? dx / a.keep : 0.f;
    a.xhat[e] = xh[j];
    a.dg[e] = dA[j];
    a.dw2in[e] = dl * h[j];
  }
}

__global__ __launch_bounds__(256) void cls_info_kernel(const float* rowloss, const float* rowcorr, int n, float* info) {
  __shared__ float red[2][256];
  const int tid = threadIdx.x;
  float sl = 0.f, sc = 0.f;
  for (int r = tid; r < n; r += 256) { sl += rowloss[r]; sc += rowcorr[r]; }
  red[0][tid] = sl;
  red[1][tid] = sc;
  __syncthreads();
  for (int o = 128; o > 0; o >>= 1) {
    if (tid < o) { red[0][tid] += red[0][tid + o]; red[1][tid] += red[1][tid + o]; }
    __syncthreads();
  }
  if (tid == 0) {
    info[0] = red[0][0] / (float)n;
    info[1] = red[1][0] / (float)n;
  }
}

struct ClsDropArgs { float* df; long per_cam; const uint8_t* mask; uint32_t key[SERL_MAX_CAMS][2]; float keep; };
__global__ __launch_bounds__(256) void cls_dropout_bwd_kernel(ClsDropArgs a) {
  const long e = (long)blockIdx.x * 256 + threadIdx.x;
  if (e >= a.per_cam) return;
  const int cam = blockIdx.y;
  const long i = (long)cam * a.per_cam + e;
  const bool k = a.mask ? a.mask[i] != 0
                        : bits_to_unit(random_bits_at(a.key[cam][0], a.key[cam][1], (uint64_t)a.per_cam, (uint64_t)e)) < a.keep;
  a.df[i] = k ? a.df[i] / a.keep : 0.f;
}

size_t carve_train(serl_classifier* c, ClsTrain* t, uint8_t* base) {
  const serl_classifier_cfg& g = c->cfg;
  Bump b(base);
  const long n = t->max_batch, nc = g.n_cam;
  t->opt.carve(b, c->t0, c->nt);
  t->info = b.take<float>(2);
  uint8_t* ws = b.take<uint8_t>(trunk_workspace_bytes((int)(nc * n), g.H, g.W));
  t->feats = b.take<float>((size_t)nc * n * c->HW * 512);
  t->f = b.take<float>((size_t)2 * nc * n * c->D);
  t->slabs_cap = 2L * 32 * nc * n * kBottleneck;
  t->slabs = b.take<float>(t->slabs_cap);
  t->enc = b.take<float>((size_t)2 * n * c->E);
  t->xhat = b.take<float>((size_t)nc * n * kBottleneck);
  t->rstd = b.take<float>((size_t)nc * n);
  t->logits = b.take<float>((size_t)2 * n);
  t->hxhat = b.take<float>((size_t)n * kHidden);
  t->hdg = b.take<float>((size_t)n * kHidden);
  t->dz = b.take<float>((size_t)n * kHidden);
  t->dw2in = b.take<float>((size_t)n * kHidden);
  t->dlogit = b.take<float>(n);
  t->rowloss = b.take<float>(n);
  t->rowcorr = b.take<float>(n);
  t->denc = b.take<float>((size_t)n * c->E);
  t->dzc = b.take<float>((size_t)nc * n * kBottleneck);
  t->dgc = b.take<float>((size_t)nc * n * kBottleneck);
  t->df = b.take<float>((size_t)nc * n * c->D);
  t->sle_part = b.take<float>((size_t)nc * kSleSplit * c->HW * 512 * kSleFeatures);
  t->ctr = b.take<int>((size_t)nc * c->HW * cdiv(512, 256));
  if (base) trunk_workspace_bind(t->tws, ws, (int)(nc * n), g.H, g.W);
  return b.off;
}

constexpr float kKeep = 0.9f;

DenseLnIo train_cam_io(const serl_classifier* c, int n, int i) {
  const ClsTrain* t = c->tr;
  const long nD = (long)n * c->D;
  return DenseLnIo{t->f + i * c->cfg.n_cam * nD, c->D, nD, t->enc + (long)i * n * c->E, c->E, kBottleneck, i ? nullptr : t->xhat, i ? nullptr : t->rstd};
}

int train_forward(serl_classifier* c, const uint8_t* frames, int n, const float* labels, const uint8_t* masks,
                  const uint32_t* keys, bool eval, hipStream_t st) {
  const serl_classifier_cfg& g = c->cfg;
  ClsTrain* t = c->tr;
  const float* P = c->params;
  const int nc = g.n_cam, ni = eval ? 2 : 1;
  const long nD = (long)n * c->D;
  RC(trunk_forward(c->tw, t->tws, frames, nc * n, t->feats, st, &c->tpk));
  SleFwdArgs sv[2] = {SleFwdArgs{}, SleFwdArgs{}};
  for (int i = 0; i < ni; ++i) { sv[i].x = t->feats; sv[i].K = P + c->cam.first; sv[i].f = t->f + i * nc * nD; }
  sv[0].mask = masks;
  if (!masks) sle_tf_masks(sv[0], keys, nc, n, 0);
  RC(sle_proprio_fwd_multi(sv, nullptr, ni, kKeep, n, c->HW, 512, nc, (long)n * c->HW * 512, c->cam.stride, nD, nD, 0, st));
  const int S0 = split_under(n, kBottleneck, nc * ni, 32);
  GemmDesc g0[2];
  LnFwdArgs l0[2];
  for (int i = 0; i < ni; ++i) {
    g0[i] = layer_fwd(c->cam.dense, P, train_cam_io(c, n, i), n, t->slabs + (long)i * nc * S0 * n * kBottleneck, S0);
    l0[i] = layer_ln_fwd(c->cam.dense, P, train_cam_io(c, n, i), n, g0[i]);
  }
  RC(gemm_f32_multi(g0, ni, st));
  RC(ln_fwd_multi(l0, ni, kBottleneck, st));
  const int S1 = split_under(n, kHidden, ni, 8);
  GemmDesc g1[2];
  for (int i = 0; i < ni; ++i)
    g1[i] = gemm_fwd(t->enc + (long)i * n * c->E, c->E, 0, P + c->o_w1, 0, t->slabs + (long)i * S1 * n * kHidden, 1, n, kHidden, c->E, S1);
  RC(gemm_f32_multi(g1, ni, st));
  ClsHeadArgs h{};
  h.slabs = t->slabs; h.S = S1; h.sstride = (long)n * kHidden; h.istride = (long)S1 * n * kHidden;
  h.b1 = P + c->o_b1; h.g1 = P + c->o_g1; h.be1 = P + c->o_be1; h.w2 = P + c->o_w2; h.b2 = P + c->o_b2;
  h.n = n; h.keep = kKeep;
  h.mask = masks ? masks + (long)nc * nD : nullptr;
  if (!masks) { h.gen = 1; h.key[0] = keys[2 * nc]; h.key[1] = keys[2 * nc + 1]; }
  h.labels = labels; h.logits = t->logits;
  h.xhat = t->hxhat; h.dg = t->hdg; h.dz = t->dz; h.dw2in = t->dw2in; h.dlogit = t->dlogit; h.rowloss = t->rowloss; h.rowcorr = t->rowcorr;
  hipLaunchKernelGGL(cls_head_kernel, dim3(cdiv(n, 4), ni), dim3(256), 0, st, h);
  SERL_HIP(hipGetLastError());
  return SERL_OK;
}

int check_train(serl_classifier* c, int n) {
  SERL_REQUIRE(c, "NULL classifier");
  if (!c->tr) {
    serl::set_error("classifier training is not initialised (serl_classifier_train_init)");
    return SERL_ERR_STATE;
  }
  SERL_REQUIRE(n >= 1 && n <= c->tr->max_batch, "n = %d not in [1, training max_batch = %d]", n, c->tr->max_batch);
  return SERL_OK;
}

int resolve_moment(serl_classifier* c, const char* section, const char* leaf, float** ptr, long* count) {
  SERL_REQUIRE(section && leaf, "NULL argument");
  const Leaf* l = find(c->leaves, leaf);
  SERL_REQUIRE(l, "unknown classifier leaf '%s'", leaf);
  *count = l->count;
  SERL_REQUIRE(c->tr->opt.moment(section, *l, ptr), "unknown classifier section '%s' (opt/mu, opt/nu)", section);
  return SERL_OK;
}

}

extern "C" {

int serl_classifier_train_init(serl_classifier* c, int max_batch, float lr, float b1, float b2, float eps) {
  SERL_REQUIRE(c, "NULL classifier");
  SERL_REQUIRE(!c->tr, "classifier training is already initialised");
  SERL_REQUIRE(max_batch >= 1 && lr > 0.f, "bad training max_batch %d / learning rate %g", max_batch, (double)lr);
  SERL_REQUIRE(b1 == 0.9f && b2 == 0.999f && eps == 1e-8f, "only optax.adam's defaults b1 = 0.9, b2 = 0.999, eps = 1e-8 are implemented");
  SERL_HIP(hipSetDevice(c->cfg.device));
  ClsTrain* t = new ClsTrain();
  t->max_batch = max_batch;
  t->lr = lr;
  if (int rc = alloc_zeroed(&t->arena, carve_train(c, t, nullptr), "classifier training arena")) {
    delete t;
    return rc;
  }
  carve_train(c, t, (uint8_t*)t->arena);
  c->tr = t;
  return SERL_OK;
}

int serl_classifier_train_forward(serl_classifier* c, const uint8_t* dev_frames, int n, const uint8_t* dev_masks,
                                  const uint32_t* host_mask_keys, float* dev_logits, void* stream) {
  RC(check_train(c, n));
  SERL_REQUIRE(dev_frames && dev_logits && (dev_masks || host_mask_keys), "NULL argument (the Dropout needs keep-masks or keys)");
  hipStream_t st = (hipStream_t)stream;
  SERL_HIP(hipSetDevice(c->cfg.device));
  RC(train_forward(c, dev_frames, n, nullptr, dev_masks, host_mask_keys, false, st));
  SERL_HIP(hipMemcpyAsync(dev_logits, c->tr->logits, (size_t)n * 4, hipMemcpyDeviceToDevice, st));
  return SERL_OK;
}

int serl_classifier_train_step(serl_classifier* c, const uint8_t* dev_frames, int n, const float* dev_labels,
                               const uint8_t* dev_masks, const uint32_t* host_mask_keys, void* stream) {
  RC(check_train(c, n));
  SERL_REQUIRE(dev_frames && dev_labels && (dev_masks || host_mask_keys), "NULL argument (the Dropout needs keep-masks or keys)");
  const serl_classifier_cfg& g = c->cfg;
  ClsTrain* t = c->tr;
  hipStream_t st = (hipStream_t)stream;
  SERL_HIP(hipSetDevice(g.device));
  const float* P = c->params;
  float* G = t->opt.grad();
  const int nc = g.n_cam;
  const long nD = (long)n * c->D;
  RC(train_forward(c, dev_frames, n, dev_labels, dev_masks, host_mask_keys, true, st));
  hipLaunchKernelGGL(cls_info_kernel, dim3(1), dim3(256), 0, st, t->rowloss, t->rowcorr, n, t->info);
  SERL_HIP(hipGetLastError());
  const GemmDesc gi = gemm_igrad(t->dz, kHidden, 0, P + c->o_w1, kHidden, 0, t->denc, c->E, 0, 1, n, c->E, kHidden);
  RC(gemm_f32_multi(&gi, 1, st));
  const DenseLn& cam = c->cam.dense;
  const DenseLnIo tc = train_cam_io(c, n, 0);
  const DenseLnGrad dc{t->denc, c->E, kBottleneck, t->dzc, t->dgc};
  RC(ln_bwd(layer_ln_bwd(cam, P, tc, dc, n), st));
  const GemmDesc gf = layer_igrad(cam, P, dc, n, t->df, c->D, nD);
  RC(gemm_f32_multi(&gf, 1, st));
  ClsDropArgs da{};
  da.df = t->df; da.per_cam = nD; da.mask = dev_masks; da.keep = kKeep;
  if (!dev_masks)
    for (int k = 0; k < nc; ++k) { da.key[k][0] = host_mask_keys[2 * k]; da.key[k][1] = host_mask_keys[2 * k + 1]; }
  hipLaunchKernelGGL(cls_dropout_bwd_kernel, dim3(cdiv(nD, 256), nc), dim3(256), 0, st, da);
  SERL_HIP(hipGetLastError());
  const long sle_n = (long)c->HW * 512 * kSleFeatures;
  RC(sle_bwd_fused(t->feats, t->df, t->sle_part, n, c->HW, 512, kSleSplit, nc, (long)n * c->HW * 512, nD, kSleSplit * sle_n,
                   G + c->cam.first, c->cam.stride, t->ctr, st));
  const Colsum3Args cs[4] = {
      {t->hdg, t->hxhat, t->dz, 1, n, kHidden, G + c->o_g1, G + c->o_be1, G + c->o_b1, 0, 0},
      {t->dw2in, nullptr, nullptr, 1, n, kHidden, nullptr, G + c->o_w2, nullptr, 0, 1},
      {t->dlogit, nullptr, nullptr, 1, n, 1, nullptr, G + c->o_b2, nullptr, 0, 2},
      layer_colsum(cam, tc, dc, n, G),
  };
  RC(colsum3_multi(cs, 4, st));
  const GemmDesc wg[2] = {
      gemm_wgrad(t->enc, c->E, 0, t->dz, kHidden, 0, G + c->o_w1, kHidden, 0, 1, c->E, kHidden, n),
      layer_wgrad(cam, tc, dc, n, G),
  };
  RC(gemm_f32_multi(wg, 2, st));
  return t->opt.apply(c->params, t->lr, st);
}

int serl_classifier_read_train_info(serl_classifier* c, float out[2], void* stream) {
  RC(check_train(c, 1));
  SERL_REQUIRE(out, "NULL argument");
  SERL_HIP(hipSetDevice(c->cfg.device));
  SERL_HIP(hipMemcpyAsync(out, c->tr->info, 2 * sizeof(float), hipMemcpyDefault, (hipStream_t)stream));
  return SERL_OK;
}

int serl_classifier_train_set_step(serl_classifier* c, int64_t step) {
  RC(check_train(c, 1));
  SERL_REQUIRE(step >= 0, "negative step");
  c->tr->opt.step = step;
  return SERL_OK;
}

int serl_classifier_train_get_step(serl_classifier* c, int64_t* step_out) {
  RC(check_train(c, 1));
  SERL_REQUIRE(step_out, "NULL argument");
  *step_out = c->tr->opt.step;
  return SERL_OK;
}

int serl_classifier_train_set(serl_classifier* c, const char* section, const char* leaf, const float* host, int64_t count) {
  RC(check_train(c, 1));
  SERL_REQUIRE(host, "NULL argument");
  float* p = nullptr;
  long n = 0;
// ... 19 lines not shown
```

### serl_amd/csrc/dense_layer.h

```cpp
#pragma once
#include "heads.h"

namespace serl {

struct DenseLn {
  long W, b, g, be;
  long w_gs, p_gs;
  int groups, K, N, act;
  int ln;
  float keep;
};
struct DenseLnDrop {
  int train;
  const uint8_t* mask;
  const uint32_t* key;
  uint64_t seed;
  long key_rows, key_row0, hash_row0;
};
inline LnDrop layer_drop(const DenseLn& L, const DenseLnDrop& s) {
  LnDrop d{};
  if (!(L.keep > 0.f) || !s.train) return d;
  d.keep = L.keep;
  if (s.mask) { d.mode = kLnDropMask; d.mask = s.mask; }
  else if (s.key) { d.mode = kLnDropKey; d.key[0] = s.key[0]; d.key[1] = s.key[1]; d.total_rows = s.key_rows; d.row0 = s.key_row0; }
  else { d.mode = kLnDropHash; d.seed = s.seed; d.row0 = s.hash_row0; }
  return d;
}
inline DenseLn add_dense_ln_leaves(std::vector<Leaf>& v, long& off, const std::string& kernel, const std::string& bias,
                                   const std::string& ln, int groups, int K, int N, int act, double drop = 0.0, bool layer_norm = true) {
  DenseLn l{};
  l.W = add_leaf(v, off, kernel, (long)groups * K * N);
  l.b = add_leaf(v, off, bias, (long)groups * N);
  l.ln = layer_norm ? 1 : 0;
  l.g = layer_norm ? add_leaf(v, off, ln + "/scale", (long)groups * N) : -1;
  l.be = layer_norm ? add_leaf(v, off, ln + "/bias", (long)groups * N) : -1;
  l.w_gs = groups > 1 ? (long)K * N : 0; l.p_gs = groups > 1 ? N : 0; l.groups = groups; l.K = K; l.N = N; l.act = act;
  l.keep = drop > 0.0 ? (float)(1.0 - drop) : 0.f;
  return l;
}

struct DenseLnIo {
  const float* x; long ldx, x_gs;
  float* y; long ld_y, y_goff;
  float *xhat, *rstd;
};
struct DenseLnGrad {
  float* dy; long ld_dy, dy_goff;
  float *dpre, *dg;
};

inline GemmDesc layer_fwd(const DenseLn& L, const float* P, const DenseLnIo& t, int rows, float* slabs, int splitk) {
  return gemm_fwd(t.x, t.ldx, t.x_gs, P + L.W, L.w_gs, slabs, L.groups, rows, L.N, L.K, splitk);
}
inline LnFwdArgs layer_ln_fwd(const DenseLn& L, const float* P, const DenseLnIo& t, int rows, const GemmDesc& g,
                              const DenseLnDrop& site = DenseLnDrop{}) {
  LnFwdArgs l{};
  l.slabs = g.C; l.S = g.splitk; l.slab_stride = g.sCz;
  l.bias = P + L.b; l.pstride = L.p_gs;
  if (L.ln) { l.gamma = P + L.g; l.beta = P + L.be; }
  l.rows = L.groups * rows; l.rows_per_group = rows;
  l.y = t.y; l.ld_y = t.ld_y; l.y_goff = t.y_goff;
  l.xhat = t.xhat; l.rstd = t.rstd; l.act = L.act;
  l.drop = layer_drop(L, site);
  return l;
}
inline ProprioArgs layer_row_fwd(const DenseLn& L, const float* P, const DenseLnIo& t) {
  return ProprioArgs{t.x, P + L.W, P + L.b, P + L.g, P + L.be, t.y, t.ld_y, t.xhat, t.rstd, nullptr, 0, nullptr, 0, 0};
}
inline LnBwdArgs layer_ln_bwd(const DenseLn& L, const float* P, const DenseLnIo& t, const DenseLnGrad& d, int rows,
                              const DenseLnDrop& site = DenseLnDrop{}) {
  LnBwdArgs l{};
  l.dy = d.dy; l.ld_dy = d.ld_dy; l.dy_goff = d.dy_goff;
  l.y = t.y; l.ld_y = t.ld_y; l.y_goff = t.y_goff;
  l.xhat = t.xhat; l.rstd = t.rstd; l.pstride = L.p_gs;
  if (L.ln) { l.gamma = P + L.g; l.beta = P + L.be; }
  l.rows = L.groups * rows; l.rows_per_group = rows; l.D = L.N;
  l.dx = d.dpre; l.dg = d.dg; l.act = L.act;
  l.drop = layer_drop(L, site);
  return l;
}
inline Colsum3Args layer_colsum(const DenseLn& L, const DenseLnIo& t, const DenseLnGrad& d, int rows, float* G) {
  if (!L.ln) return Colsum3Args{d.dpre, nullptr, nullptr, L.groups, rows, L.N, nullptr, G + L.b, nullptr, L.p_gs, 1};
  return Colsum3Args{d.dg, t.xhat, d.dpre, L.groups, rows, L.N, G + L.g, G + L.be, G + L.b, L.p_gs, 0};
}
inline GemmDesc layer_wgrad(const DenseLn& L, const DenseLnIo& t, const DenseLnGrad& d, int rows, float* G) {
  return gemm_wgrad(t.x, t.ldx, t.x_gs, d.dpre, L.N, (long)rows * L.N, G + L.W, L.N, L.w_gs, L.groups, L.K, L.N, rows);
}
inline GemmDesc layer_igrad(const DenseLn& L, const float* P, const DenseLnGrad& d, int rows, float* out, long ldo, long out_zs,
                            int splitk = 1) {
  return gemm_igrad(d.dpre, L.N, (long)rows * L.N, P + L.W, L.N, L.w_gs, out, ldo, out_zs, L.groups, rows, L.K, L.N, splitk);
}
inline GemmDesc layer_igrad(const DenseLn& L, const float* P, const DenseLnGrad& d, int rows, const DenseLnGrad& below) {
  return layer_igrad(L, P, d, rows, below.dy, below.ld_dy, below.dy_goff);
}

struct CamHeadOffsets { long first, stride; DenseLn dense; };
template <typename F>
CamHeadOffsets add_cam_head_leaves(std::vector<Leaf>& v, long& off, int n_cam, int D, int N, F front) {
  CamHeadOffsets o{};
  for (int k = 0; k < n_cam; ++k) {
    const std::string p = "enc/" + std::to_string(k) + "/";
    const long first = off;
    front(p);
    const DenseLn l = add_dense_ln_leaves(v, off, p + "dense/kernel", p + "dense/bias", p + "ln", 1, D, N, kActTanh);
    if (k == 0) o = CamHeadOffsets{first, off - first, l};
  }
  o.dense.groups = n_cam; o.dense.w_gs = o.dense.p_gs = o.stride;
  return o;
}

}
```

### serl_amd/csrc/heads.h

```cpp
#pragma once
#include <cmath>

#include "internal.h"

namespace serl {

extern long g_chain_launches;

constexpr int kMaxMulti = 4;
template <typename T>
struct Multi { T v[kMaxMulti]; };
constexpr int kMaxGemmGroups = 6;
int gemm_f32_multi(const GemmDesc* groups, int n, hipStream_t stream);

int reduce_slabs(const float* slabs, int S, long slab_stride, int groups, int rows, int N, const float* bias,
                 long bias_gstride, float* out, long ld_out, long out_gstride, bool accumulate,
                 hipStream_t stream, float scale = 1.0f);

int ln_fwd_multi(const LnFwdArgs* a, int n, int D, hipStream_t stream);
int label_rows(const LnFwdArgs& a, float* label, float* mean, int* ctr, hipStream_t stream);

struct RedqSel { int n; int idx[16]; };
struct LossArgs {
  int on;
  const float *qt, *q, *reward, *mask; RedqSel sel; int E, B; float discount, inv_norm;
  float *y_out, *dq, *scalars, *dbias; int per_member; const float *logp_next, *alpha;
};
struct LnBwdArgs {
  const float* dy; long ld_dy; long dy_goff;
  const float* dq; const float* dq_w; float dq_const;
  long dq_w_gstride;
  const float* y; long ld_y; long y_goff;
  const float* xhat; const float* rstd;
  const float* gamma; long pstride;
  int rows, rows_per_group;
  float* dx;
  float* dg;
  int act;
  const float* beta;
  int D;
  int dq_inline;
  LnDrop drop;
};
int ln_bwd_multi(const LnBwdArgs* a, int n, const LossArgs& loss, hipStream_t stream);
inline int ln_bwd(const LnBwdArgs& a, hipStream_t stream) { return ln_bwd_multi(&a, 1, LossArgs{}, stream); }

int colsum(const float* X, const float* Y, int groups, int rows_per_group, int D, float* out,
           long out_gstride, bool accumulate, hipStream_t stream);
struct Colsum3Args {
  const float *dg, *xhat, *dpre; int groups, rows_per_group, D;
  float *o_gamma, *o_beta, *o_bias; long gstride;
  int mode;
};
constexpr int kMaxColsum = 8;
int colsum3_multi(const Colsum3Args* layers, int n, hipStream_t stream);
int colsum3(const float* dg, const float* xhat, const float* dpre, int groups, int rows_per_group, int D,
            float* o_gamma, float* o_beta, float* o_bias, long gstride, hipStream_t stream);
struct SleFwdArgs {
  const float* x; const float* K; const uint8_t* mask; float* f;
  int gen; uint64_t seed; long row_offset, rows_global;
  uint32_t tf_key[4][2]; long tf_rows, tf_row0;
};
struct ProprioArgs;
int sle_proprio_fwd_multi(const SleFwdArgs* v, const ProprioArgs* pv, int n, float keep, int N, int HW, int Cc, int groups, long x_gs,
                          long k_gs, long mask_gs, long f_gs, int state_dim, hipStream_t stream);
int sle_fwd_multi(const SleFwdArgs* v, int n, float keep_scale, int N, int HW, int Cc, int groups, long x_gs, long k_gs,
                  long mask_gs, long f_gs, hipStream_t stream);
int sle_bwd(const float* x, const float* df, float* partial, int N, int HW, int Cc, int nsplit, int groups,
            long x_gs, long df_gs, long part_gs, hipStream_t stream);
int sle_bwd_fused(const float* x, const float* df, float* partial, int N, int HW, int Cc, int nsplit, int groups,
                  long x_gs, long df_gs, long part_gs, float* out, long out_gs, int* ctr, hipStream_t stream);
int critic_loss(const float* qt, const float* q, const float* reward, const float* mask, RedqSel sel, int E,
                int B, float discount, float inv_norm, float* y_out, float* dq, float* scalars, float* dbias,
                hipStream_t stream, bool per_member_bias = false, const float* logp_next = nullptr, const float* alpha = nullptr);
int policy_dist_fwd_multi(const PolicyDistArgs* v, int n, int B, int A, float std_min, float std_max, hipStream_t stream);
struct PolicyStatsArgs {
  const float* slabs; int S;
  const float *bias_mean, *bias_ls, *act;
  float *mean, *std, *mode_out, *logp;
  int rows, A; float std_min, std_max;
  int mode;
};
int policy_stats(const PolicyStatsArgs& v, hipStream_t stream);
struct ProprioArgs {
  const float* state; const float *W, *b, *gamma, *beta;
  float* y; long ld_y; float* xhat; float* rstd;
  const float* copy_src; long ld_copy_src; float* copy_dst; long ld_copy_dst; int copy_cols;
};
int proprio_fwd_multi(const ProprioArgs* v, int n, int S, int rows, hipStream_t stream);
int policy_dist_bwd(const float* da, long ld_da, const float* act, long ld_act, const float* pre,
                    const float* stdv, const float* eps, const float* alpha, float coef, int B, int A,
                    float std_min, float std_max, float* dpre, const float* q, int E, float* qmean_out,
                    hipStream_t stream, int mode = kPolExp);
struct CopyJob { const float* src; long ld_src; float* dst; long ld_dst; int cols; };
int copy_cols_multi(const CopyJob* jobs, int n, int rows, hipStream_t stream);
int fill(float* p, float v, long n, hipStream_t stream);

struct AdamArgs {
  float *theta, *theta_target;
  long P, Pc, Pa0, Pa1;
  const float *g_critic, *g_actor;
  float *m_c, *v_c, *m_a, *v_a, *m_t, *v_t;
  const float* sum_logp_next;
  float* temp_grad_out;
  int critic_on, actor_on, temp_on;
  float lr_c, lr_a, lr_t, bc1, bc2, tau, target_entropy, inv_batch;
  int ema_on;
  float wd_c, wd_a, wd_t;
  float clip_c, clip_a, clip_t;
  const float* norm2;
  float* frozen; float* frozen_target; long n_frozen;
  long n_frozen_live; int vec_ok;
  int info_mode, info_reset;
  const float* scalars; const float* alpha; float* info_acc;
  float info_w, inv_eb;
};
int adam_ema(const AdamArgs& a, hipStream_t stream);
int adam_info_only(const AdamArgs& a, hipStream_t stream);
inline AdamArgs adam_slice(float* theta, long nt, const float* g, float* m, float* v, float lr, int64_t step) {
  AdamArgs a{};
  a.theta = theta; a.theta_target = nullptr;
  a.P = nt + 1; a.Pc = 0; a.Pa0 = 0; a.Pa1 = nt;
  a.g_actor = g; a.m_a = m; a.v_a = v;
  a.m_t = m + nt; a.v_t = v + nt;
  a.actor_on = 1;
  a.lr_a = lr;
  a.bc1 = 1.0f - powf(0.9f, (float)step);
  a.bc2 = 1.0f - powf(0.999f, (float)step);
  return a;
}
constexpr const char* kFrozenMoment = "'%s' of the frozen leaf '%s' must be zero";
struct AdamSlice {
  long t0 = 0, nt = 0;
  float *m = nullptr, *v = nullptr, *G = nullptr;
  int64_t step = 0;
  void carve(Bump& b, long t0_, long nt_) {
    t0 = t0_; nt = nt_;
    m = b.take<float>(nt + 1);
    v = b.take<float>(nt + 1);
    G = b.take<float>(nt);
  }
  float* grad() const { return G - t0; }
  bool moment(const char* section, const Leaf& l, float** ptr) const {
    const std::string s = section;
    if (s != "opt/mu" && s != "opt/nu") return false;
    *ptr = l.off < t0 ? nullptr : (s == "opt/mu" ? m : v) + (l.off - t0);
    return true;
  }
  int apply(float* params, float lr, hipStream_t stream) {
    RC(adam_ema(adam_slice(params + t0, nt, G, m, v, lr, step + 1), stream));
    step += 1;
    return SERL_OK;
  }
};
int frozen_ema(const float* frozen, float* frozen_target, long n, float tau, long steps, hipStream_t stream);
int grad_norm2(const float* g_critic, long nc, const float* g_actor, long na, float* out, hipStream_t stream);
struct NoiseJob { void* out; long n; uint64_t seed; int kind; float keep; long rows_local, rows_global, row_offset, row_elems; };
int gen_noise_multi(const NoiseJob* v, int n, hipStream_t stream);

inline GemmDesc gemm_fwd(const float* X, long ldx, long x_gs, const float* W, long w_gs, float* slabs, int groups, int rows, int N,
                         int K, int splitk) {
  GemmDesc g{};
  g.A = X; g.sAm = ldx; g.sAk = 1; g.sAb = x_gs;
  g.B = W; g.sBk = N; g.sBn = 1; g.sBb = w_gs;
  g.C = slabs; g.ldc = N; g.sCz = (long)rows * N;
  g.M = rows; g.N = N; g.K = K; g.nbatch = groups; g.splitk = splitk;
  return g;
}
inline GemmDesc gemm_igrad(const float* dY, long ldy, long dy_gs, const float* W, long ldw, long w_gs, float* out, long ldo,
                           long out_zs, int groups, int rows, int Kin, int Nout, int splitk = 1) {
  GemmDesc g{};
  g.A = dY; g.sAm = ldy; g.sAk = 1; g.sAb = dy_gs;
  g.B = W; g.sBk = 1; g.sBn = ldw; g.sBb = w_gs;
  g.C = out; g.ldc = ldo; g.sCz = out_zs;
  g.M = rows; g.N = Kin; g.K = Nout; g.nbatch = groups; g.splitk = splitk;
  return g;
}
inline GemmDesc gemm_wgrad(const float* X, long ldx, long x_gs, const float* dY, long ldy, long dy_gs, float* out, long ldo,
                           long out_gs, int groups, int Mx, int Ny, int rows) {
  GemmDesc g{};
  g.A = X; g.sAm = 1; g.sAk = ldx; g.sAb = x_gs;
  g.B = dY; g.sBk = ldy; g.sBn = 1; g.sBb = dy_gs;
  g.C = out; g.ldc = ldo; g.sCz = out_gs;
  g.M = Mx; g.N = Ny; g.K = rows; g.nbatch = groups; g.splitk = 1;
  return g;
}

inline void sle_tf_masks(SleFwdArgs& s, const uint32_t* keys, int n_cam, long rows, long row0) {
  s.gen = 2;
  for (int k = 0; k < n_cam; ++k) { s.tf_key[k][0] = keys[2 * k]; s.tf_key[k][1] = keys[2 * k + 1]; }
  s.tf_rows = rows; s.tf_row0 = row0;
}

}
```

### serl_amd/csrc/heads.hip

```cpp
#include <algorithm>
#include <cstdlib>

#include "heads.h"
#include "jaxrng.h"
#include "ln_stats.h"
#include "prof.h"

namespace serl {

long g_chain_launches = 0;
#define SERL_LAUNCH_CHAIN(...) do { ++g_chain_launches; hipLaunchKernelGGL(__VA_ARGS__); } while (0)

typedef float f32x16 __attribute__((ext_vector_type(16)));

constexpr int kGBM = 64, kGBN = 64, kGBK = 32, kGP = 36, kGPT = 68;
constexpr int kGTile = kGBM * kGP;
static_assert(kGBK * kGPT <= kGTile, "the [k][row] layout must fit the tile");
typedef float f32x4 __attribute__((ext_vector_type(4)));
typedef float f32x4u __attribute__((ext_vector_type(4), aligned(4)));

__device__ __forceinline__ f32x4 ld4(const float* p, int valid) {
  f32x4 v = {0.f, 0.f, 0.f, 0.f};
  if (valid >= 4) {
    v = *reinterpret_cast<const f32x4u*>(p);
// ... 683 lines not shown
          acc = __builtin_amdgcn_mfma_f32_32x32x16_bf16(a[0], b[0], acc, 0, 0, 0);
        }
        __syncthreads();
      }
    }
  }
  if (g.epi) { gemm_epilogue<ALT>(g, acc, C, z, batch, m0, n0, reinterpret_cast<float*>(AB), tid); return; }
#pragma unroll
  for (int r = 0; r < 16; ++r) {
    const int m = m0 + wm * 32 + (r & 3) + 8 * (r >> 2) + 4 * lh;
    const int n = n0 + wn * 32 + li;
    if (m < g.M && n < g.N) C[(long)m * g.ldc + n] = g.relu ? fmaxf(acc[r], 0.f) : acc[r];
  }
}

__global__ __launch_bounds__(256) void gemm_f32_strided_kernel(GemmDesc g) {
  constexpr int BK = 16, P = 68, LD = kGBM * BK / 256;
  __shared__ float As[BK][P];
  __shared__ float Bs[BK][P];
  const int tid = threadIdx.x, lane = tid & 63, wave = tid >> 6;
  const int wm = wave >> 1, wn = wave & 1;
  const int z = blockIdx.z, batch = z / g.splitk, split = z - batch * g.splitk;
  const int m0 = blockIdx.y * kGBM, n0 = blockIdx.x * kGBN;
  const int kper = ((g.K + g.splitk - 1) / g.splitk + kGBK - 1) / kGBK * kGBK;
  const int k_begin = split * kper, k_end = min(g.K, k_begin + kper);
  const float* A = g.A + (long)batch * g.sAb;
  const float* B = g.B + (long)batch * g.sBb;
  float* C = g.C + (long)z * g.sCz;
  f32x16 acc;
#pragma unroll
  for (int r = 0; r < 16; ++r) acc[r] = 0.f;
  const int li = lane & 31, lh = lane >> 5;
  for (int k0 = k_begin; k0 < k_end; k0 += BK) {
#pragma unroll
    for (int i = 0; i < LD; ++i) {
      const int x = tid & 63, k = (tid >> 6) + 4 * i, gk = k0 + k;
      As[k][x] = (m0 + x < g.M && gk < k_end) ? A[(long)(m0 + x) * g.sAm + (long)gk * g.sAk] : 0.f;
      Bs[k][x] = (n0 + x < g.N && gk < k_end) ? B[(long)gk * g.sBk + (long)(n0 + x) * g.sBn] : 0.f;
    }
    __syncthreads();
#pragma unroll
    for (int ks = 0; ks < BK / 2; ++ks)
      acc = __builtin_amdgcn_mfma_f32_32x32x2f32(As[2 * ks + lh][wm * 32 + li], Bs[2 * ks + lh][wn * 32 + li], acc, 0, 0, 0);
    __syncthreads();
  }
#pragma unroll
  for (int r = 0; r < 16; ++r) {
    const int m = m0 + wm * 32 + (r & 3) + 8 * (r >> 2) + 4 * lh;
    const int n = n0 + wn * 32 + li;
    if (m < g.M && n < g.N) C[(long)m * g.ldc + n] = acc[r];
  }
}

int gemm_f32_multi(const GemmDesc* gs, int n, hipStream_t stream) {
  SERL_REQUIRE(n >= 1 && n <= kMaxGemmGroups, "bad GEMM group count %d", n);
  GemmMulti mm{};
  mm.n = n;
  int gx = 0, gy = 0, z = 0;
  bool a_k = true, a_m = true, b_k = true, b_n = true;
  for (int i = 0; i < n; ++i) {
    a_k = a_k && gs[i].sAk == 1; a_m = a_m && gs[i].sAm == 1;
    b_k = b_k && gs[i].sBk == 1; b_n = b_n && gs[i].sBn == 1;
  }
  const bool vec = (a_k || a_m) && (b_k || b_n);
  SERL_REQUIRE(vec || n == 1, "mixed operand layouts in a GEMM group");
  bool gather = false;
  for (int i = 0; i < n; ++i) {
    gather = gather || gs[i].gtab != nullptr || gs[i].relu;
    SERL_REQUIRE(!gs[i].gtab || (gs[i].gseg > 0 && gs[i].gseg % 16 == 0 && (gs[i].sAk == 1 || gs[i].sAm == 1)), "bad gather GEMM");
    SERL_REQUIRE(!gs[i].relu || gs[i].splitk == 1, "relu epilogue with a K-split");
  }
  SERL_REQUIRE(!gather || vec, "gather GEMM needs a vector layout");
  for (int i = 0; i < n; ++i) {
    const GemmDesc& g = gs[i];
    SERL_REQUIRE(g.M > 0 && g.N > 0 && g.K > 0 && g.nbatch > 0 && g.splitk > 0, "bad GEMM shape");
    mm.d[i] = g;
    gx = std::max(gx, cdiv(g.N, kGBN));
    gy = std::max(gy, cdiv(g.M, kGBM));
    z += g.nbatch * g.splitk;
    mm.zend[i] = z;
  }
  dim3 grid(gx, gy, z);
  static const bool exact = []() { const char* e = getenv("SERL_GEMM"); return e && e[0] == 'f'; }();
  bool any_epi = false;
  for (int i = 0; i < n; ++i) any_epi = any_epi || gs[i].epi != kEpiNone;
  SERL_REQUIRE(!any_epi || vec, "epilogue GEMMs need a vector layout");
  bool alt = false;
  for (int i = 0; i < n; ++i) alt = alt || (gs[i].epi == kEpiPolicy && gs[i].pd.mode != kPolExp);
  if (alt) {
    for (int i = 0; i < n; ++i)
      SERL_REQUIRE(gs[i].epi == kEpiPolicy && gs[i].pd.mode == gs[0].pd.mode && !gs[i].gtab, "a policy-head launch mixes distributions or kinds of GEMM");
    SERL_REQUIRE(a_k && b_n, "the policy head's GEMM reads row-major activations and a row-major kernel");
    if (!exact) SERL_LAUNCH_CHAIN((gemm_bf16x3_kernel<true, false, 16, false, true>), grid, dim3(256), 0, stream, mm);
    else SERL_LAUNCH_CHAIN((gemm_f32_kernel<true, false, true>), grid, dim3(256), 0, stream, mm);
    SERL_HIP(hipGetLastError());
    return SERL_OK;
  }
  if (vec && (!exact || gather)) {
    bool any_tab = false;
    for (int i = 0; i < n; ++i) any_tab = any_tab || gs[i].gtab != nullptr;
    for (int i = 0; i < n; ++i) SERL_REQUIRE(!any_tab || gs[i].gtab != nullptr, "a gather launch mixes gathered and plain operands");
    if (any_tab) {
      if (a_k && b_k) SERL_LAUNCH_CHAIN((gemm_bf16x3_kernel<true, true, 16, true>), grid, dim3(256), 0, stream, mm);
      else if (a_k) SERL_LAUNCH_CHAIN((gemm_bf16x3_kernel<true, false, 16, true>), grid, dim3(256), 0, stream, mm);
      else if (b_k) SERL_LAUNCH_CHAIN((gemm_bf16x3_kernel<false, true, 16, true>), grid, dim3(256), 0, stream, mm);
      else SERL_LAUNCH_CHAIN((gemm_bf16x3_kernel<false, false, 16, true>), grid, dim3(256), 0, stream, mm);
    } else if (a_k && b_k) SERL_LAUNCH_CHAIN((gemm_bf16x3_kernel<true, true, 16>), grid, dim3(256), 0, stream, mm);
    else if (a_k) SERL_LAUNCH_CHAIN((gemm_bf16x3_kernel<true, false, 16>), grid, dim3(256), 0, stream, mm);
    else if (b_k) SERL_LAUNCH_CHAIN((gemm_bf16x3_kernel<false, true, 16>), grid, dim3(256), 0, stream, mm);
    else SERL_LAUNCH_CHAIN((gemm_bf16x3_kernel<false, false, 16>), grid, dim3(256), 0, stream, mm);
  } else if (vec) {
    if (a_k && b_k) SERL_LAUNCH_CHAIN((gemm_f32_kernel<true, true>), grid, dim3(256), 0, stream, mm);
    else if (a_k) SERL_LAUNCH_CHAIN((gemm_f32_kernel<true, false>), grid, dim3(256), 0, stream, mm);
    else if (b_k) SERL_LAUNCH_CHAIN((gemm_f32_kernel<false, true>), grid, dim3(256), 0, stream, mm);
    else SERL_LAUNCH_CHAIN((gemm_f32_kernel<false, false>), grid, dim3(256), 0, stream, mm);
  } else {
    for (int i = 0; i < n; ++i) {
      const GemmDesc& g = gs[i];
      SERL_LAUNCH_CHAIN(gemm_f32_strided_kernel, dim3(cdiv(g.N, kGBN), cdiv(g.M, kGBM), g.nbatch * g.splitk), dim3(256), 0,
                         stream, g);
    }
  }
  SERL_HIP(hipGetLastError());
  return SERL_OK;
}

int gemm_f32(const GemmDesc& g, hipStream_t stream) { return gemm_f32_multi(&g, 1, stream); }

__global__ void reduce_slabs_kernel(const float* slabs, int S, long slab_stride, int rows, int N,
                                    const float* bias, long bias_gstride, float* out, long ld_out,
                                    long out_gstride, int accumulate, float scale) {
  const long e = (long)blockIdx.x * blockDim.x + threadIdx.x;
  const int grp = blockIdx.y;
  if (e >= (long)rows * N) return;
  const int row = (int)(e / N), col = (int)(e - (long)row * N);
  float v = 0.f;
  for (int s = 0; s < S; ++s) v += slabs[((long)grp * S + s) * slab_stride + e];
  v *= scale;
  if (bias) v += bias[(long)grp * bias_gstride + col];
  float* o = out + (long)grp * out_gstride + (long)row * ld_out + col;
  *o = accumulate ? *o + v : v;
}

int reduce_slabs(const float* slabs, int S, long slab_stride, int groups, int rows, int N, const float* bias,
                 long bias_gstride, float* out, long ld_out, long out_gstride, bool accumulate,
                 hipStream_t stream, float scale) {
  dim3 grid(cdiv((long)rows * N, 256), groups);
  SERL_LAUNCH_CHAIN(reduce_slabs_kernel, grid, dim3(256), 0, stream, slabs, S, slab_stride, rows, N, bias,
                     bias_gstride, out, ld_out, out_gstride, accumulate ? 1 : 0, scale);
  SERL_HIP(hipGetLastError());
  return SERL_OK;
}

template <int VPL, bool BLOCKED>
__global__ __launch_bounds__(256) void ln_fwd_kernel(Multi<LnFwdArgs> mv) {
  const LnFwdArgs& a = mv.v[blockIdx.y];
  const int row = blockIdx.x * 4 + (threadIdx.x >> 6), lane = threadIdx.x & 63;
  if (row >= a.rows) return;
  ln_row<VPL, BLOCKED>(a, row, lane);
}
template <int VPL, bool BLOCKED>
__global__ __launch_bounds__(256) void ln_fwd_drop_kernel(Multi<LnFwdArgs> mv) {
  const LnFwdArgs& a = mv.v[blockIdx.y];
  const int row = blockIdx.x * 4 + (threadIdx.x >> 6), lane = threadIdx.x & 63;
  if (row >= a.rows) return;
  ln_row<VPL, BLOCKED, true>(a, row, lane);
}
template <int VPL, bool BLOCKED>
__global__ __launch_bounds__(256) void plain_fwd_kernel(Multi<LnFwdArgs> mv) {
  const LnFwdArgs& a = mv.v[blockIdx.y];
  const int row = blockIdx.x * 4 + (threadIdx.x >> 6), lane = threadIdx.x & 63;
  if (row >= a.rows) return;
  plain_row<VPL, BLOCKED>(a, row, lane);
}

__global__ __launch_bounds__(256) void label_rows_kernel(LnFwdArgs a, float* label, float* mean, int* ctr) {
  __shared__ float red[256 + 1];
  const int tid = threadIdx.x, row = blockIdx.x * 4 + (tid >> 6), lane = tid & 63;
  const __amdgpu_buffer_rsrc_t lab = rsrc_of(label);
  if (row < a.rows) {
    const float logit = ln_row<4, true>(a, row, lane);
    const float p = 1.f / (1.f + expf(-logit));
    if (lane == 0) __builtin_amdgcn_raw_buffer_store_b32(__builtin_bit_cast(unsigned, p >= 0.5f ? 1.f : 0.f), lab, row * 4, 0, kSc1);
  }
  if (!arrive_is_last(ctr, (int)gridDim.x, reinterpret_cast<int*>(&red[256]))) return;
  float s = 0.f;
  for (int r = tid; r < a.rows; r += 256) s += ld1_sc1(lab, r);
  red[tid] = s;
  __syncthreads();
  for (int o = 128; o > 0; o >>= 1) {
    if (tid < o) red[tid] += red[tid + o];
    __syncthreads();
  }
  if (tid == 0) mean[0] = red[0] / (float)a.rows;
}

int label_rows(const LnFwdArgs& a, float* label, float* mean, int* ctr, hipStream_t stream) {
  SERL_REQUIRE(a.rows >= 1 && a.rows == a.rows_per_group && a.act == kActRelu && a.dot_out && label && mean && ctr, "bad label launch");
  SERL_LAUNCH_CHAIN(label_rows_kernel, dim3(cdiv(a.rows, 4)), dim3(256), 0, stream, a, label, mean, ctr);
  SERL_HIP(hipGetLastError());
  return SERL_OK;
}

#define SERL_LN_WIDTH_OK(D) ((D) >= 64 && (D) <= 1024 && (D) % 64 == 0)
static bool ln_drop_ok(const LnDrop& d, long rows) {
  if (d.mode == kLnDropNone) return true;
  if (!(d.keep > 0.f && d.keep <= 1.f)) return false;
  if (d.mode == kLnDropMask) return d.mask != nullptr;
  if (d.mode == kLnDropKey) return d.row0 >= 0 && d.row0 + rows <= d.total_rows;
  return d.mode == kLnDropHash && d.row0 >= 0;
}
#define SERL_LN_CASE(V, K, ...) case V: SERL_LAUNCH_CHAIN(K, __VA_ARGS__); break;
#define SERL_LN_STRIDED(V, K, ...) SERL_LN_CASE(V, (K<V, false>), __VA_ARGS__)
#define SERL_LN_LAUNCH(D, K64, K256, K, ...)                                                                              \
  switch ((D) / 64) {                                                                                                     \
    SERL_LN_CASE(1, K64, __VA_ARGS__) SERL_LN_CASE(4, K256, __VA_ARGS__)                                                  \
    SERL_LN_STRIDED(2, K, __VA_ARGS__) SERL_LN_STRIDED(3, K, __VA_ARGS__) SERL_LN_STRIDED(5, K, __VA_ARGS__)              \
    SERL_LN_STRIDED(6, K, __VA_ARGS__) SERL_LN_STRIDED(7, K, __VA_ARGS__) SERL_LN_STRIDED(8, K, __VA_ARGS__)              \
    SERL_LN_STRIDED(9, K, __VA_ARGS__) SERL_LN_STRIDED(10, K, __VA_ARGS__) SERL_LN_STRIDED(11, K, __VA_ARGS__)            \
    SERL_LN_STRIDED(12, K, __VA_ARGS__) SERL_LN_STRIDED(13, K, __VA_ARGS__) SERL_LN_STRIDED(14, K, __VA_ARGS__)           \
    SERL_LN_STRIDED(15, K, __VA_ARGS__) SERL_LN_STRIDED(16, K, __VA_ARGS__)                                               \
    default: serl::set_error("LayerNorm width %d has no kernel", (int)(D)); return SERL_ERR_INVALID;                      \
  }

int ln_fwd_multi(const LnFwdArgs* as, int n, int D, hipStream_t stream) {
  SERL_REQUIRE(SERL_LN_WIDTH_OK(D), "LayerNorm width %d unsupported (a multiple of 64 in [64, 1024])", D);
  SERL_REQUIRE(n >= 1 && n <= kMaxMulti, "bad instance count %d", n);
  Multi<LnFwdArgs> mv{};
  int rows = 0;
  bool drop = false;
  for (int i = 0; i < n; ++i) {
    SERL_REQUIRE(as[i].act >= 0 && as[i].act < kActCount, "LayerNorm row: activation code %d is not tanh (0), relu (1) or swish (2)", as[i].act);
    SERL_REQUIRE(ln_drop_ok(as[i].drop, as[i].rows_per_group), "LayerNorm row: bad Dropout description (mode %d, keep %g)", as[i].drop.mode, as[i].drop.keep);
    mv.v[i] = as[i];
    rows = std::max(rows, as[i].rows);
    drop = drop || as[i].drop.mode != kLnDropNone;
    SERL_REQUIRE((as[i].gamma == nullptr) == (as[0].gamma == nullptr) && (as[i].gamma == nullptr) == (as[i].beta == nullptr),
                 "LayerNorm row: instance %d %s a LayerNorm and instance 0 %s; plain and LayerNorm rows do not share a launch", i,
                 as[i].gamma ? "has" : "lacks", as[0].gamma ? "has" : "lacks");
  }
  dim3 grid(cdiv(rows, 4), n);
  if (!as[0].gamma) {
    SERL_REQUIRE(!drop, "plain row (no LayerNorm) with Dropout: not served");
    SERL_LN_LAUNCH(D, (plain_fwd_kernel<1, false>), (plain_fwd_kernel<4, true>), plain_fwd_kernel, grid, dim3(256), 0, stream, mv)
  } else if (drop) SERL_LN_LAUNCH(D, (ln_fwd_drop_kernel<1, false>), (ln_fwd_drop_kernel<4, true>), ln_fwd_drop_kernel, grid, dim3(256), 0, stream, mv)
  else SERL_LN_LAUNCH(D, (ln_fwd_kernel<1, false>), (ln_fwd_kernel<4, true>), ln_fwd_kernel, grid, dim3(256), 0, stream, mv)
  SERL_HIP(hipGetLastError());
  return SERL_OK;
}

__device__ __forceinline__ float redq_target(const LossArgs& L, int b) {
  float mq;
  if (L.sel.n > 0) {
    mq = L.qt[(long)L.sel.idx[0] * L.B + b];
    for (int k = 1; k < L.sel.n; ++k) mq = fminf(mq, L.qt[(long)L.sel.idx[k] * L.B + b]);
  } else {
    mq = L.qt[b];
    for (int e = 1; e < L.E; ++e) mq = fminf(mq, L.qt[(long)e * L.B + b]);
  }
  float y = L.reward[b] + L.discount * L.mask[b] * mq;
  if (L.logp_next) y -= L.alpha[0] * L.logp_next[b];
  return y;
}

__device__ void critic_loss_body(const LossArgs& L, float (*red)[256]) {
  float s_d2 = 0.f, s_q = 0.f, s_y = 0.f, s_dq = 0.f;
  float s_e[16];
#pragma unroll
  for (int e = 0; e < 16; ++e) s_e[e] = 0.f;
  for (int b = threadIdx.x; b < L.B; b += 256) {
    const float y = redq_target(L, b);
    L.y_out[b] = y;
    s_y += y;
    for (int e = 0; e < L.E; ++e) {
      const float qv = L.q[(long)e * L.B + b];
      const float d = qv - y;
      const float g = 2.f * d * L.inv_norm;
      L.dq[(long)e * L.B + b] = g;
      s_d2 += d * d;
      s_q += qv;
      s_dq += g;
      if (L.per_member) {
#pragma unroll
        for (int k = 0; k < 16; ++k)
          if (k == e) s_e[k] += g;
      }
    }
  }
  red[0][threadIdx.x] = s_d2; red[1][threadIdx.x] = s_q; red[2][threadIdx.x] = s_y; red[3][threadIdx.x] = s_dq;
  __syncthreads();
  for (int o = 128; o > 0; o >>= 1) {
    if ((int)threadIdx.x < o)
      for (int k = 0; k < 4; ++k) red[k][threadIdx.x] += red[k][threadIdx.x + o];
    __syncthreads();
  }
  if (threadIdx.x == 0) {
    L.scalars[0] = red[0][0]; L.scalars[1] = red[1][0]; L.scalars[2] = red[2][0];
    if (!L.per_member) *L.dbias = red[3][0];
  }
  if (L.per_member) {
#pragma unroll
    for (int k = 0; k < 16; ++k) {
      if (k < L.E) {
        __syncthreads();
        red[0][threadIdx.x] = s_e[k];
        __syncthreads();
        for (int o = 128; o > 0; o >>= 1) {
          if ((int)threadIdx.x < o) red[0][threadIdx.x] += red[0][threadIdx.x + o];
          __syncthreads();
        }
        if (threadIdx.x == 0) L.dbias[k] = red[0][0];
      }
    }
  }
}

template <int VPL, bool BLOCKED, bool DROP = false>
__device__ __forceinline__ void ln_bwd_row(const LnBwdArgs& a, const LossArgs& L, int row, int lane) {
  const int grp = row / a.rows_per_group;
  constexpr int D = VPL * 64;
  float dg[VPL], dxh[VPL], xh[VPL], y[VPL], gam[VPL];
  float s1 = 0.f, s2 = 0.f;
  const long lr = row - grp * a.rows_per_group;
  const int c0 = ln_col0<VPL, BLOCKED>(lane);
  float dqr = 0.f;
  if (a.dq_w) dqr = a.dq_inline ? 2.f * (L.q[row] - redq_target(L, (int)lr)) * L.inv_norm : (a.dq ? a.dq[row] : a.dq_const);
#pragma unroll
  for (int j = 0; j < VPL; ++j) {
    const int col = c0 + kLnStep<BLOCKED> * j;
    y[j] = a.y[lr * a.ld_y + (long)grp * a.y_goff + col];
    dg[j] = a.dq_w ? dqr * a.dq_w[(long)grp * a.dq_w_gstride + col] : a.dy[lr * a.ld_dy + (long)grp * a.dy_goff + col];
    xh[j] = a.xhat[(long)row * D + col];
    gam[j] = a.gamma[(long)grp * a.pstride + col];
  }
  ln_act_grad<VPL, BLOCKED ? 1 : 64>(a.act, dg, y, xh, gam, a.beta, (long)grp * a.pstride + c0);
#pragma unroll
  for (int j = 0; j < VPL; ++j) {
    dxh[j] = dg[j] * gam[j];
    s1 += dxh[j];
    s2 += dxh[j] * xh[j];
  }
  wave_sum2(s1, s2);
  const float m1 = s1 * (1.0f / D), m2 = s2 * (1.0f / D), rstd = a.rstd[row];
  if constexpr (!DROP) {
#pragma unroll
    for (int j = 0; j < VPL; ++j) {
      const int col = c0 + kLnStep<BLOCKED> * j;
      a.dx[(long)row * D + col] = rstd * (dxh[j] - m1 - xh[j] * m2);
      a.dg[(long)row * D + col] = dg[j];
    }
  } else {
#pragma unroll
    for (int j = 0; j < VPL; ++j) dxh[j] = rstd * (dxh[j] - m1 - xh[j] * m2);
    if (a.drop.mode != kLnDropNone) ln_dropout<VPL, BLOCKED>(a.drop, lr, c0, dxh);
#pragma unroll
    for (int j = 0; j < VPL; ++j) {
      const int col = c0 + kLnStep<BLOCKED> * j;
      a.dx[(long)row * D + col] = dxh[j];
      a.dg[(long)row * D + col] = dg[j];
    }
  }
}

template <int VPL, bool BLOCKED>
__device__ __forceinline__ void plain_bwd_row(const LnBwdArgs& a, const LossArgs& L, int row, int lane) {
  const int grp = row / a.rows_per_group;
  constexpr int D = VPL * 64, kStep = kLnStep<BLOCKED>;
  float dg[VPL], y[VPL];
  const long lr = row - grp * a.rows_per_group;
  const int c0 = ln_col0<VPL, BLOCKED>(lane);
  float dqr = 0.f;
  if (a.dq_w) dqr = a.dq_inline ? 2.f * (L.q[row] - redq_target(L, (int)lr)) * L.inv_norm : (a.dq ? a.dq[row] : a.dq_const);
#pragma unroll
  for (int j = 0; j < VPL; ++j) {
    const int col = c0 + kStep * j;
    y[j] = a.y[lr * a.ld_y + (long)grp * a.y_goff + col];
    dg[j] = a.dq_w ? dqr * a.dq_w[(long)grp * a.dq_w_gstride + col] : a.dy[lr * a.ld_dy + (long)grp * a.dy_goff + col];
  }
  if (a.act == kActTanh) {
#pragma unroll
    for (int j = 0; j < VPL; ++j) dg[j] *= 1.f - y[j] * y[j];
  } else if (a.act == kActRelu) {
#pragma unroll
    for (int j = 0; j < VPL; ++j) dg[j] = y[j] > 0.f ? dg[j] : 0.f;
  } else {
#pragma unroll
    for (int j = 0; j < VPL; ++j) {
      const float sg = sigmoid_stable(a.xhat[(long)row * D + c0 + kStep * j]);
      dg[j] *= sg + y[j] * (1.f - sg);
    }
  }
#pragma unroll
  for (int j = 0; j < VPL; ++j) a.dx[(long)row * D + c0 + kStep * j] = dg[j];
}
// ... 88 lines not shown
  if (part == 0 && col < D) {
    const float t = (red[0][threadIdx.x] + red[1][threadIdx.x]) + (red[2][threadIdx.x] + red[3][threadIdx.x]);
    float* o = out + (long)grp * out_gstride + col;
    *o = accumulate ? *o + t : t;
  }
}

int colsum(const float* X, const float* Y, int groups, int rows_per_group, int D, float* out,
           long out_gstride, bool accumulate, hipStream_t stream) {
  SERL_LAUNCH_CHAIN(colsum_kernel, dim3(cdiv(D, 64), groups), dim3(256), 0, stream, X, Y, rows_per_group, D,
                     out, out_gstride, accumulate ? 1 : 0);
  SERL_HIP(hipGetLastError());
  return SERL_OK;
}

struct ColsumMulti { Colsum3Args v[kMaxColsum]; };
__global__ __launch_bounds__(512) void colsum3_kernel(ColsumMulti mv) {
  const Colsum3Args& a = mv.v[blockIdx.z];
  __shared__ float red[3][8][64];
  const int grp = blockIdx.y, col = blockIdx.x * 64 + (threadIdx.x & 63), part = threadIdx.x >> 6;
  if (grp >= a.groups || (int)blockIdx.x * 64 >= a.D) return;
  float s0 = 0.f, s1 = 0.f, s2 = 0.f;
  if (a.mode == 2) {
    float* r1 = &red[0][0][0];
    if (threadIdx.x < 256) {
      for (int r = threadIdx.x; r < a.rows_per_group; r += 256) s1 += a.dg[r];
      r1[threadIdx.x] = s1;
    }
    __syncthreads();
    for (int o = 128; o > 0; o >>= 1) {
      if ((int)threadIdx.x < o) r1[threadIdx.x] += r1[threadIdx.x + o];
      __syncthreads();
    }
    if (threadIdx.x == 0) a.o_beta[0] = r1[0];
    return;
  }
  if (col < a.D) {
    const long base = (long)grp * a.rows_per_group;
    if (a.mode == 1) {
      if (part < 4)
        for (int r = part; r < a.rows_per_group; r += 4) s1 += a.dg[(base + r) * a.D + col];
    } else {
      for (int r = part; r < a.rows_per_group; r += 8) {
        const long e = (base + r) * a.D + col;
        const float g = a.dg[e];
        s0 += g * a.xhat[e];
        s1 += g;
        s2 += a.dpre[e];
      }
    }
  }
  red[0][part][threadIdx.x & 63] = s0;
  red[1][part][threadIdx.x & 63] = s1;
  red[2][part][threadIdx.x & 63] = s2;
  __syncthreads();
  if (a.mode == 1) {
    if (part == 1 && col < a.D) {
      const int c = threadIdx.x & 63;
      a.o_beta[(long)grp * a.gstride + col] = (red[1][0][c] + red[1][1][c]) + (red[1][2][c] + red[1][3][c]);
    }
    return;
  }
  if (part < 3 && col < a.D) {
    const int c = threadIdx.x & 63;
    float t = 0.f;
#pragma unroll
    for (int k = 0; k < 8; ++k) t += red[part][k][c];
    float* o = (part == 0 ? a.o_gamma : (part == 1 ? a.o_beta : a.o_bias)) + (long)grp * a.gstride + col;
    *o = t;
  }
}

int colsum3_multi(const Colsum3Args* vs, int n, hipStream_t stream) {
  SERL_REQUIRE(n >= 1 && n <= kMaxColsum, "bad layer count %d", n);
  ColsumMulti mv{};
  int gx = 0, gy = 0;
  for (int i = 0; i < n; ++i) {
    mv.v[i] = vs[i];
    gx = std::max(gx, cdiv(vs[i].D, 64));
    gy = std::max(gy, vs[i].groups);
  }
  SERL_LAUNCH_CHAIN(colsum3_kernel, dim3(gx, gy, n), dim3(512), 0, stream, mv);
  SERL_HIP(hipGetLastError());
  return SERL_OK;
}

int colsum3(const float* dg, const float* xhat, const float* dpre, int groups, int rows_per_group, int D,
            float* o_gamma, float* o_beta, float* o_bias, long gstride, hipStream_t stream) {
  const Colsum3Args v{dg, xhat, dpre, groups, rows_per_group, D, o_gamma, o_beta, o_bias, gstride, 0};
  return colsum3_multi(&v, 1, stream);
}

__global__ __launch_bounds__(256) void sle_fwd_kernel(Multi<SleFwdArgs> mv, float keep_scale, int N, int HW, int Cc,
                                                     long xs, long ks, long ms, long fs) {
  const long e = (long)blockIdx.x * 256 + threadIdx.x;
  if (e >= (long)N * Cc) return;
  const SleFwdArgs& v = mv.v[blockIdx.z];
  const float* x = v.x + blockIdx.y * xs;
  const float* K = v.K + blockIdx.y * ks;
  float* f = v.f + blockIdx.y * fs;
  const uint8_t* mask = v.mask ? v.mask + blockIdx.y * ms : nullptr;
  const int n = (int)(e / Cc), c = (int)(e - (long)n * Cc);
  float acc[8] = {0, 0, 0, 0, 0, 0, 0, 0};
#pragma unroll 4
  for (int hw = 0; hw < HW; ++hw) {
    const float xv = x[((long)n * HW + hw) * Cc + c];
    const float4 k0 = *reinterpret_cast<const float4*>(K + ((long)hw * Cc + c) * 8);
    const float4 k1 = *reinterpret_cast<const float4*>(K + ((long)hw * Cc + c) * 8 + 4);
    acc[0] += xv * k0.x; acc[1] += xv * k0.y; acc[2] += xv * k0.z; acc[3] += xv * k0.w;
    acc[4] += xv * k1.x; acc[5] += xv * k1.y; acc[6] += xv * k1.z; acc[7] += xv * k1.w;
  }
  float* o = f + (long)n * Cc * 8 + (long)c * 8;
  if (mask) {
    const uint8_t* m = mask + (long)n * Cc * 8 + (long)c * 8;
#pragma unroll
    for (int j = 0; j < 8; ++j) acc[j] = m[j] ? acc[j] * keep_scale : 0.f;
  }
  *reinterpret_cast<float4*>(o) = make_float4(acc[0], acc[1], acc[2], acc[3]);
  *reinterpret_cast<float4*>(o + 4) = make_float4(acc[4], acc[5], acc[6], acc[7]);
}

int sle_fwd_multi(const SleFwdArgs* vs, int n, float keep_scale, int N, int HW, int Cc, int groups, long x_gs, long k_gs,
                  long mask_gs, long f_gs, hipStream_t stream) {
  SERL_REQUIRE(n >= 1 && n <= kMaxMulti, "bad instance count %d", n);
  Multi<SleFwdArgs> mv{};
  for (int i = 0; i < n; ++i) mv.v[i] = vs[i];
  SERL_LAUNCH_CHAIN(sle_fwd_kernel, dim3(cdiv((long)N * Cc, 256), groups, n), dim3(256), 0, stream, mv, keep_scale, N,
                     HW, Cc, x_gs, k_gs, mask_gs, f_gs);
  SERL_HIP(hipGetLastError());
  return SERL_OK;
}


__device__ __forceinline__ void proprio_row(const ProprioArgs& a, int S, int row, int lane) {
  float v = a.b[lane];
  for (int s0 = 0; s0 < S; s0 += 64) {
    const float mine = (s0 + lane < S) ? a.state[(long)row * S + s0 + lane] : 0.f;
    const int cnt = min(64, S - s0);
    int s = 0;
    for (; s + 8 <= cnt; s += 8) {
      float w[8];
#pragma unroll
      for (int j = 0; j < 8; ++j) w[j] = a.W[(s0 + s + j) * 64 + lane];
#pragma unroll
      for (int j = 0; j < 8; ++j) v += __shfl(mine, s + j) * w[j];
    }
    for (; s < cnt; ++s) v += __shfl(mine, s) * a.W[(s0 + s) * 64 + lane];
  }
  float s1 = v, s2 = v * v;
  wave_sum2(s1, s2);
  float mean, rstd;
  ln_mean_rstd<64>(s1, s2, mean, rstd);
  const float xh = (v - mean) * rstd;
  a.y[(long)row * a.ld_y + lane] = tanhf(xh * a.gamma[lane] + a.beta[lane]);
  if (a.xhat) a.xhat[(long)row * 64 + lane] = xh;
  if (a.rstd && lane == 0) a.rstd[row] = rstd;
  if (a.copy_dst && lane < a.copy_cols) a.copy_dst[(long)row * a.ld_copy_dst + lane] = a.copy_src[(long)row * a.ld_copy_src + lane];
}

template <int kSleNb, int kPx>
__global__ __launch_bounds__(256) void sle_proprio_fwd_kernel(Multi<SleFwdArgs> mv, Multi<ProprioArgs> pv, int has_proprio,
                                                              float keep_scale, unsigned keep_thr, float keep_p, int N, int HW, int Cc,
                                                              long xs, long ks, long ms, long fs, int S, int nb_sle) {
  if ((int)blockIdx.x >= nb_sle) {
    if (!has_proprio || blockIdx.y != 0) return;
    const int row = ((int)blockIdx.x - nb_sle) * 4 + (threadIdx.x >> 6);
    if (row < N) proprio_row(pv.v[blockIdx.z], S, row, threadIdx.x & 63);
    return;
  }
  const SleFwdArgs& v = mv.v[blockIdx.z];
  const int cblocks = (Cc + 255) / 256;
  const int c = ((int)blockIdx.x % cblocks) * 256 + threadIdx.x, n0 = ((int)blockIdx.x / cblocks) * kSleNb;
  if (c >= Cc) return;
  const float* x = v.x + blockIdx.y * xs + (long)n0 * HW * Cc + c;
  const float* K = v.K + blockIdx.y * ks + (long)c * 8;
  const int ns = min(kSleNb, N - n0);
  float acc[kSleNb][8];
#pragma unroll
  for (int s = 0; s < kSleNb; ++s)
#pragma unroll
    for (int j = 0; j < 8; ++j) acc[s][j] = 0.f;
  for (int hw0 = 0; hw0 < HW; hw0 += kPx) {
    float4 k0[kPx], k1[kPx];
#pragma unroll
    for (int i = 0; i < kPx; ++i) {
      const int hw = min(hw0 + i, HW - 1);
      k0[i] = *reinterpret_cast<const float4*>(K + (long)hw * Cc * 8);
      k1[i] = *reinterpret_cast<const float4*>(K + (long)hw * Cc * 8 + 4);
    }
    float xv[kSleNb][kPx];
#pragma unroll
    for (int s = 0; s < kSleNb; ++s)
#pragma unroll
      for (int i = 0; i < kPx; ++i) xv[s][i] = x[((long)min(s, ns - 1) * HW + min(hw0 + i, HW - 1)) * Cc];
#pragma unroll
    for (int i = 0; i < kPx; ++i) {
      if (hw0 + i < HW) {
#pragma unroll
        for (int s = 0; s < kSleNb; ++s) {
          acc[s][0] += xv[s][i] * k0[i].x; acc[s][1] += xv[s][i] * k0[i].y; acc[s][2] += xv[s][i] * k0[i].z; acc[s][3] += xv[s][i] * k0[i].w;
          acc[s][4] += xv[s][i] * k1[i].x; acc[s][5] += xv[s][i] * k1[i].y; acc[s][6] += xv[s][i] * k1[i].z; acc[s][7] += xv[s][i] * k1[i].w;
        }
      }
    }
  }
  float* f = v.f + blockIdx.y * fs + (long)n0 * Cc * 8 + (long)c * 8;
  const uint8_t* mask = v.mask ? v.mask + blockIdx.y * ms + (long)n0 * Cc * 8 + (long)c * 8 : nullptr;
#pragma unroll
  for (int s = 0; s < kSleNb; ++s) {
    if (s >= ns) break;
    if (mask) {
      const uint8_t* m = mask + (long)s * Cc * 8;
#pragma unroll
      for (int j = 0; j < 8; ++j) acc[s][j] = m[j] ? acc[s][j] * keep_scale : 0.f;
    } else if (v.gen == 2) {
      const uint32_t k0 = v.tf_key[blockIdx.y][0], k1 = v.tf_key[blockIdx.y][1];
      const uint64_t rowlen = (uint64_t)Cc * 8ull, total = (uint64_t)v.tf_rows * rowlen;
      const uint64_t e0 = (uint64_t)(v.tf_row0 + n0 + s) * rowlen + (uint64_t)c * 8ull;
#pragma unroll
      for (int j = 0; j < 8; ++j)
        acc[s][j] = bits_to_unit(random_bits_at(k0, k1, total, e0 + (uint64_t)j)) < keep_p ? acc[s][j] * keep_scale : 0.f;
    } else if (v.gen) {
      const uint64_t ctr = (((uint64_t)blockIdx.y * (uint64_t)v.rows_global + (uint64_t)(v.row_offset + n0 + s)) * (uint64_t)Cc + (uint64_t)c) * 3ull;
      const uint64_t h0 = mix64(v.seed ^ mix64(ctr)), h1 = mix64(v.seed ^ mix64(ctr + 1)), h2 = mix64(v.seed ^ mix64(ctr + 2));
      const unsigned u[8] = {(unsigned)(h0 & 0xFFFFFF), (unsigned)((h0 >> 24) & 0xFFFFFF), (unsigned)((h0 >> 48) | ((h1 & 0xFF) << 16)),
                             (unsigned)((h1 >> 8) & 0xFFFFFF), (unsigned)((h1 >> 32) & 0xFFFFFF), (unsigned)((h1 >> 56) | ((h2 & 0xFFFF) << 8)),
                             (unsigned)((h2 >> 16) & 0xFFFFFF), (unsigned)(h2 >> 40)};
#pragma unroll
      for (int j = 0; j < 8; ++j) acc[s][j] = u[j] < keep_thr ? acc[s][j] * keep_scale : 0.f;
    }
    *reinterpret_cast<float4*>(f + (long)s * Cc * 8) = make_float4(acc[s][0], acc[s][1], acc[s][2], acc[s][3]);
    *reinterpret_cast<float4*>(f + (long)s * Cc * 8 + 4) = make_float4(acc[s][4], acc[s][5], acc[s][6], acc[s][7]);
  }
}

int sle_proprio_fwd_multi(const SleFwdArgs* vs, const ProprioArgs* ps, int n, float keep, int N, int HW, int Cc, int groups, long x_gs,
                          long k_gs, long mask_gs, long f_gs, int state_dim, hipStream_t stream) {
  SERL_REQUIRE(n >= 1 && n <= kMaxMulti, "bad instance count %d", n);
  Multi<SleFwdArgs> mv{};
  Multi<ProprioArgs> pv{};
  for (int i = 0; i < n; ++i) {
    mv.v[i] = vs[i];
    if (ps) { pv.v[i] = ps[i]; SERL_REQUIRE(!ps[i].copy_dst || ps[i].copy_cols <= 64, "copy_cols > 64"); }
  }
  const int nb = N <= 64 ? 2 : 4;
  const int nb_sle = cdiv(Cc, 256) * cdiv(N, nb), nb_prop = ps ? cdiv(N, 4) : 0;
  if (nb == 2)
    SERL_LAUNCH_CHAIN((sle_proprio_fwd_kernel<2, 4>), dim3(nb_sle + nb_prop, groups, n), dim3(256), 0, stream, mv, pv, ps ? 1 : 0,
                      1.0f / keep, (unsigned)(keep * 16777216.0f), keep, N, HW, Cc, x_gs, k_gs, mask_gs, f_gs, state_dim, nb_sle);
  else
    SERL_LAUNCH_CHAIN((sle_proprio_fwd_kernel<4, 2>), dim3(nb_sle + nb_prop, groups, n), dim3(256), 0, stream, mv, pv, ps ? 1 : 0,
                      1.0f / keep, (unsigned)(keep * 16777216.0f), keep, N, HW, Cc, x_gs, k_gs, mask_gs, f_gs, state_dim, nb_sle);
  SERL_HIP(hipGetLastError());
  return SERL_OK;
}

__global__ __launch_bounds__(256) void sle_bwd_kernel(const float* x, const float* df, float* partial, int N,
                                                     int HW, int Cc, int nsplit, long x_gs, long df_gs, long part_gs) {
  const int c = blockIdx.x * 256 + threadIdx.x, hw = blockIdx.y, sp = blockIdx.z % nsplit, grp = blockIdx.z / nsplit;
  if (c >= Cc) return;
  x += grp * x_gs; df += grp * df_gs; partial += grp * part_gs;
  const int per = (N + nsplit - 1) / nsplit;
  const int nb = sp * per, ne = min(N, nb + per);
  float acc[8] = {0, 0, 0, 0, 0, 0, 0, 0};
  for (int n = nb; n < ne; ++n) {
    const float xv = x[((long)n * HW + hw) * Cc + c];
    const float4 d0 = *reinterpret_cast<const float4*>(df + (long)n * Cc * 8 + (long)c * 8);
    const float4 d1 = *reinterpret_cast<const float4*>(df + (long)n * Cc * 8 + (long)c * 8 + 4);
    acc[0] += xv * d0.x; acc[1] += xv * d0.y; acc[2] += xv * d0.z; acc[3] += xv * d0.w;
    acc[4] += xv * d1.x; acc[5] += xv * d1.y; acc[6] += xv * d1.z; acc[7] += xv * d1.w;
  }
  float* o = partial + (((long)sp * HW + hw) * Cc + c) * 8;
  *reinterpret_cast<float4*>(o) = make_float4(acc[0], acc[1], acc[2], acc[3]);
  *reinterpret_cast<float4*>(o + 4) = make_float4(acc[4], acc[5], acc[6], acc[7]);
}

__global__ __launch_bounds__(256) void sle_bwd_fused_kernel(const float* x, const float* df, float* partial, int N, int HW, int Cc,
                                                           int nsplit, long x_gs, long df_gs, long part_gs, float* out, long out_gs,
                                                           int* ctr) {
  __shared__ int s_last;
  const int c = blockIdx.x * 256 + threadIdx.x, hw = blockIdx.y, sp = blockIdx.z % nsplit, grp = blockIdx.z / nsplit;
  x += grp * x_gs; df += grp * df_gs; partial += grp * part_gs;
  const int per = (N + nsplit - 1) / nsplit;
  const int nb = sp * per, ne = min(N, nb + per);
  float acc[8] = {0, 0, 0, 0, 0, 0, 0, 0};
  if (c < Cc) {
    for (int n = nb; n < ne; ++n) {
      const float xv = x[((long)n * HW + hw) * Cc + c];
      const float4 d0 = *reinterpret_cast<const float4*>(df + (long)n * Cc * 8 + (long)c * 8);
      const float4 d1 = *reinterpret_cast<const float4*>(df + (long)n * Cc * 8 + (long)c * 8 + 4);
      acc[0] += xv * d0.x; acc[1] += xv * d0.y; acc[2] += xv * d0.z; acc[3] += xv * d0.w;
      acc[4] += xv * d1.x; acc[5] += xv * d1.y; acc[6] += xv * d1.z; acc[7] += xv * d1.w;
    }
    const __amdgpu_buffer_rsrc_t rs = rsrc_of(partial);
    const long o = (((long)sp * HW + hw) * Cc + c) * 8;
    __builtin_amdgcn_raw_buffer_store_b128(__builtin_bit_cast(u32x4_t, (f32x4){acc[0], acc[1], acc[2], acc[3]}), rs, (int)(o * 4), 0, kSc1);
    __builtin_amdgcn_raw_buffer_store_b128(__builtin_bit_cast(u32x4_t, (f32x4){acc[4], acc[5], acc[6], acc[7]}), rs, (int)(o * 4 + 16), 0, kSc1);
  }
  if (!arrive_is_last(ctr + ((long)grp * HW + hw) * gridDim.x + blockIdx.x, nsplit, &s_last)) return;
  if (c >= Cc) return;
  const __amdgpu_buffer_rsrc_t rs = rsrc_of(partial);
  f32x4 s0 = {0.f, 0.f, 0.f, 0.f}, s1 = {0.f, 0.f, 0.f, 0.f};
  for (int s = 0; s < nsplit; ++s) {
    const long o = (((long)s * HW + hw) * Cc + c) * 8;
    s0 += ld_sc1(rs, o);
    s1 += ld_sc1(rs, o + 4);
  }
  float* o = out + grp * out_gs + ((long)hw * Cc + c) * 8;
  *reinterpret_cast<f32x4*>(o) = s0;
  *reinterpret_cast<f32x4*>(o + 4) = s1;
}

int sle_bwd_fused(const float* x, const float* df, float* partial, int N, int HW, int Cc, int nsplit, int groups,
                  long x_gs, long df_gs, long part_gs, float* out, long out_gs, int* ctr, hipStream_t stream) {
  SERL_REQUIRE((long)nsplit * HW * Cc * 8 * 4 < (1L << 31), "SLE partial sums exceed 2 GB");
  SERL_LAUNCH_CHAIN(sle_bwd_fused_kernel, dim3(cdiv(Cc, 256), HW, nsplit * groups), dim3(256), 0, stream, x, df, partial, N,
                     HW, Cc, nsplit, x_gs, df_gs, part_gs, out, out_gs, ctr);
  SERL_HIP(hipGetLastError());
  return SERL_OK;
}

int sle_bwd(const float* x, const float* df, float* partial, int N, int HW, int Cc, int nsplit, int groups,
            long x_gs, long df_gs, long part_gs, hipStream_t stream) {
  SERL_LAUNCH_CHAIN(sle_bwd_kernel, dim3(cdiv(Cc, 256), HW, nsplit * groups), dim3(256), 0, stream, x, df, partial, N,
                     HW, Cc, nsplit, x_gs, df_gs, part_gs);
  SERL_HIP(hipGetLastError());
  return SERL_OK;
}

__global__ __launch_bounds__(256) void critic_loss_kernel(LossArgs L) {
  __shared__ float red[4][256];
  critic_loss_body(L, red);
}

int critic_loss(const float* qt, const float* q, const float* reward, const float* mask, RedqSel sel, int E,
                int B, float discount, float inv_norm, float* y_out, float* dq, float* scalars, float* dbias,
                hipStream_t stream, bool per_member_bias, const float* logp_next, const float* alpha) {
  SERL_REQUIRE(!per_member_bias || E <= 16, "per-member head bias supports ensembles of at most 16 (got %d)", E);
  SERL_REQUIRE(sel.n >= 0 && sel.n <= 16, "critic_subsample_size %d not in [0, 16]", sel.n);
  const LossArgs L{1, qt, q, reward, mask, sel, E, B, discount, inv_norm, y_out, dq, scalars, dbias, per_member_bias ? 1 : 0, logp_next, alpha};
  SERL_LAUNCH_CHAIN(critic_loss_kernel, dim3(1), dim3(256), 0, stream, L);
  SERL_HIP(hipGetLastError());
  return SERL_OK;
}

template <int MODE>
__global__ void policy_dist_fwd_kernel(Multi<PolicyDistArgs> mv, int B, int A, float std_min, float std_max) {
  const PolicyDistArgs& v = mv.v[blockIdx.x];
  __shared__ float red[256];
  float local = 0.f;
  for (int b = threadIdx.x; b < B; b += 256) {
    float lp = 0.f;
    for (int j = 0; j < A; ++j) {
      float mean = v.bias_mean[j], ls = v.bias_ls[j];
      for (int sp = 0; sp < v.S; ++sp) {
        mean += v.slabs[((long)sp * B + b) * A + j];
        if (policy_ls_group<MODE>()) ls += v.slabs[(((long)v.S + sp) * B + b) * A + j];
      }
      const float e = v.eps[(long)b * A + j];
      v.pre[(long)b * A + j] = mean;
      if (!policy_fixed<MODE>()) v.pre[((long)B + b) * A + j] = ls;
      const float sd = policy_std<MODE>(ls, std_min, std_max);
      const float u = mean + sd * e;
      v.act[(long)b * v.ld_act + j] = (MODE & kPolNoTanh) ? u : tanhf(u);
      v.std_out[(long)b * A + j] = sd;
      lp += -0.5f * e * e - logf(sd) - 0.91893853320467274f;
      if (!(MODE & kPolNoTanh)) lp -= 2.f * (0.69314718055994531f - u - softplusf(-2.f * u));
    }
    v.logp[b] = lp;
    local += lp;
  }
  red[threadIdx.x] = local;
  __syncthreads();
  for (int o = 128; o > 0; o >>= 1) {
    if ((int)threadIdx.x < o) red[threadIdx.x] += red[threadIdx.x + o];
    __syncthreads();
  }
  if (threadIdx.x == 0 && v.sum_logp) *v.sum_logp = red[0];
  if (threadIdx.x == 0 && v.alpha_out) v.alpha_out[0] = softplusf(v.lam[0]);
}

int policy_dist_fwd_multi(const PolicyDistArgs* vs, int n, int B, int A, float std_min, float std_max, hipStream_t stream) {
  SERL_REQUIRE(n >= 1 && n <= kMaxMulti, "bad instance count %d", n);
  Multi<PolicyDistArgs> mv{};
  for (int i = 0; i < n; ++i) {
    mv.v[i] = vs[i];
    SERL_REQUIRE(vs[i].mode == vs[0].mode, "the policy heads of one launch share a distribution mode");
  }
#define SERL_X(M) SERL_LAUNCH_CHAIN(policy_dist_fwd_kernel<M>, dim3(n), dim3(256), 0, stream, mv, B, A, std_min, std_max)
  SERL_POLICY_MODE_SWITCH(vs[0].mode, SERL_X, SERL_REQUIRE(false, "bad policy distribution mode %d", vs[0].mode))
#undef SERL_X
  SERL_HIP(hipGetLastError());
  return SERL_OK;
}

template <int MODE>
__global__ __launch_bounds__(256) void policy_stats_kernel(PolicyStatsArgs v) {
  const int row = blockIdx.x * 4 + (threadIdx.x >> 6), lane = threadIdx.x & 63;
  if (row >= v.rows) return;
  const int A = v.A;
  const bool live = lane < A;
  const int j = live ? lane : 0;
  const long e = (long)row * A + j;
  float mean = v.bias_mean[j], ls = v.bias_ls[j];
// ... 230 lines not shown
      if (a.info_reset)
        for (int k = 0; k < 8; ++k) acc[k] = 0.f;
      acc[0] += a.info_w * sc[0] * a.inv_eb;
      acc[1] += a.info_w * sc[1] * a.inv_eb;
      acc[2] += a.info_w * sc[2] * a.inv_batch;
    }
    if (a.info_mode & 2) {
      const float alpha = a.alpha[0];
      acc[3] = -(sc[3] - alpha * sc[4]) * a.inv_batch;
      acc[4] = alpha;
      acc[5] = -sc[4] * a.inv_batch;
      acc[6] = alpha * (-sc[5] * a.inv_batch - a.target_entropy);
    }
  }
  float cs_c = 1.f, cs_a = 1.f;
  if (a.clip_c > 0.f && a.critic_on) { const float n = sqrtf(a.norm2[0]); if (!(n < a.clip_c)) cs_c = a.clip_c / n; }
  if (a.clip_a > 0.f && a.actor_on) { const float n = sqrtf(a.norm2[1]); if (!(n < a.clip_a)) cs_a = a.clip_a / n; }
  const long i4 = 4 * t;
  const bool c_all = i4 + 3 < a.Pc, c_none = i4 >= a.Pc;
  const bool a_all = i4 >= a.Pa0 && i4 + 3 < a.Pa1, a_none = i4 + 3 < a.Pa0 || i4 >= a.Pa1;
  if (a.vec_ok && i4 + 3 < a.P - 1 && (c_all || c_none) && (a_all || a_none)) {
    const float b1 = 0.9f, b2 = 0.999f, eps = 1e-8f;
    const long ic = c_all ? i4 : 0, ka = a_all ? i4 - a.Pa0 : 0;
    const float4 p0 = *reinterpret_cast<const float4*>(a.theta + i4);
    const float4 tt = *reinterpret_cast<const float4*>((a.ema_on ? a.theta_target : a.theta) + i4);
    const float4 gc = *reinterpret_cast<const float4*>(a.g_critic + ic);
    const float4 mc = *reinterpret_cast<const float4*>(a.m_c + ic), vc = *reinterpret_cast<const float4*>(a.v_c + ic);
    const f32x4 ga = *reinterpret_cast<const f32x4u*>(a.g_actor + ka);
    const f32x4 ma = *reinterpret_cast<const f32x4u*>(a.m_a + ka), va = *reinterpret_cast<const f32x4u*>(a.v_a + ka);
    const float p0e[4] = {p0.x, p0.y, p0.z, p0.w}, tte[4] = {tt.x, tt.y, tt.z, tt.w};
    const float gce[4] = {gc.x, gc.y, gc.z, gc.w}, mce[4] = {mc.x, mc.y, mc.z, mc.w}, vce[4] = {vc.x, vc.y, vc.z, vc.w};
    const float gae[4] = {ga[0], ga[1], ga[2], ga[3]}, mae[4] = {ma[0], ma[1], ma[2], ma[3]}, vae[4] = {va[0], va[1], va[2], va[3]};
    float pn[4], tn[4], mcn[4], vcn[4], man[4], van[4];
#pragma unroll
    for (int e = 0; e < 4; ++e) {
      float ua = 0.f, uc = 0.f;
      {
        const float g = a.critic_on ? gce[e] * cs_c : 0.f;
        const float m = b1 * mce[e] + (1.f - b1) * g;
        const float v = b2 * vce[e] + (1.f - b2) * g * g;
        mcn[e] = m; vcn[e] = v;
        if (c_all) uc = -a.lr_c * (m / a.bc1) / (sqrtf(v / a.bc2) + eps);
      }
      {
        const float g = a.actor_on ? gae[e] * cs_a : 0.f;
        const float m = b1 * mae[e] + (1.f - b1) * g;
        const float v = b2 * vae[e] + (1.f - b2) * g * g;
        man[e] = m; van[e] = v;
        if (a_all) ua = -a.lr_a * (m / a.bc1) / (sqrtf(v / a.bc2) + eps);
      }
      float ut = 0.f;
      if (a.wd_a != 0.f) ua -= a.lr_a * a.wd_a * p0e[e];
      if (a.wd_c != 0.f) uc -= a.lr_c * a.wd_c * p0e[e];
      if (a.wd_t != 0.f) ut -= a.lr_t * a.wd_t * p0e[e];
      pn[e] = p0e[e] + ((ua + uc) + ut);
      tn[e] = pn[e] * a.tau + tte[e] * (1.f - a.tau);
    }
    if (c_all) {
      *reinterpret_cast<float4*>(a.m_c + i4) = make_float4(mcn[0], mcn[1], mcn[2], mcn[3]);
      *reinterpret_cast<float4*>(a.v_c + i4) = make_float4(vcn[0], vcn[1], vcn[2], vcn[3]);
    }
    if (a_all) {
      *reinterpret_cast<f32x4u*>(a.m_a + ka) = (f32x4){man[0], man[1], man[2], man[3]};
      *reinterpret_cast<f32x4u*>(a.v_a + ka) = (f32x4){van[0], van[1], van[2], van[3]};
    }
    *reinterpret_cast<float4*>(a.theta + i4) = make_float4(pn[0], pn[1], pn[2], pn[3]);
    if (a.ema_on) *reinterpret_cast<float4*>(a.theta_target + i4) = make_float4(tn[0], tn[1], tn[2], tn[3]);
    return;
  }
  const long total = a.P + a.n_frozen_live;
#pragma unroll 1
  for (int e = 0; e < 4; ++e)
    if (i4 + e < total) adam_elem(a, i4 + e, cs_c, cs_a);
}

__global__ __launch_bounds__(256) void frozen_ema_kernel(const float* frozen, float* frozen_target, long n, float tau, long steps) {
  const long i = (long)blockIdx.x * 256 + threadIdx.x;
  if (i >= n) return;
  const float p = frozen[i];
  float t = frozen_target[i];
  for (long k = 0; k < steps; ++k) {
    const float u = p * tau + t * (1.f - tau);
    if (u == t) break;
    t = u;
  }
  frozen_target[i] = t;
}
int frozen_ema(const float* frozen, float* frozen_target, long n, float tau, long steps, hipStream_t stream) {
  if (n <= 0 || steps <= 0) return SERL_OK;
  SERL_LAUNCH_CHAIN(frozen_ema_kernel, dim3(cdiv(n, 256)), dim3(256), 0, stream, frozen, frozen_target, n, tau, steps);
  SERL_HIP(hipGetLastError());
  return SERL_OK;
}

int adam_ema(const AdamArgs& a, hipStream_t stream) {
  ProfScope prof("adam_ema", stream);
  const bool frozen = a.n_frozen > 0 && (a.ema_on || a.wd_c != 0.f || a.wd_a != 0.f || a.wd_t != 0.f);
  AdamArgs v = a;
  v.n_frozen_live = frozen ? a.n_frozen : 0;
  auto al16 = [](const void* p) { return (reinterpret_cast<uintptr_t>(p) & 15) == 0; };
  v.vec_ok = a.Pc >= 4 && a.Pa1 - a.Pa0 >= 4 && al16(a.theta) && al16(a.theta_target) && al16(a.g_critic) && al16(a.m_c) &&
             al16(a.v_c) && a.g_critic && a.g_actor && a.m_a && a.v_a;
  SERL_LAUNCH_CHAIN(adam_ema_kernel, dim3(cdiv(cdiv(a.P + v.n_frozen_live, 4), 256)), dim3(256), 0, stream, v);
  SERL_HIP(hipGetLastError());
  return SERL_OK;
}

int adam_info_only(const AdamArgs& a, hipStream_t stream) {
  AdamArgs v = a;
  v.P = v.Pc = v.Pa0 = v.Pa1 = 0;
  v.n_frozen = v.n_frozen_live = 0;
  v.vec_ok = 0;
  v.critic_on = v.actor_on = v.temp_on = v.ema_on = 0;
  v.clip_c = v.clip_a = v.clip_t = 0.f;
  SERL_REQUIRE(v.info_mode != 0 && v.info_acc && v.scalars, "the info rider needs its mode, its scalars and a place for the result");
  SERL_LAUNCH_CHAIN(adam_ema_kernel, dim3(1), dim3(256), 0, stream, v);
  SERL_HIP(hipGetLastError());
  return SERL_OK;
}

__global__ __launch_bounds__(1024) void grad_norm2_kernel(const float* gc, long nc, const float* ga, long na, float* out) {
  const float* g = blockIdx.x ? ga : gc;
  const long n = blockIdx.x ? na : nc;
  double s = 0.0;
  for (long i = threadIdx.x; i < n; i += 1024) s += (double)g[i] * (double)g[i];
  __shared__ double red[1024];
  red[threadIdx.x] = s;
  __syncthreads();
  for (int o = 512; o > 0; o >>= 1) {
    if ((int)threadIdx.x < o) red[threadIdx.x] += red[threadIdx.x + o];
    __syncthreads();
  }
  if (threadIdx.x == 0) out[blockIdx.x] = (float)red[0];
}
int grad_norm2(const float* g_critic, long nc, const float* g_actor, long na, float* out, hipStream_t stream) {
  SERL_LAUNCH_CHAIN(grad_norm2_kernel, dim3(2), dim3(1024), 0, stream, g_critic, nc, g_actor, na, out);
  SERL_HIP(hipGetLastError());
  return SERL_OK;
}

__device__ __forceinline__ void gen_one(const NoiseJob& j, long i0) {
  if (i0 >= j.n) return;
  long i = i0;
  if (j.rows_global) {
    const long e = i0 % j.row_elems, rr = i0 / j.row_elems, r = rr % j.rows_local, plane = rr / j.rows_local;
    i = (plane * j.rows_global + j.row_offset + r) * j.row_elems + e;
  }
  if (j.kind == 0) {
    const uint64_t r = mix64(j.seed ^ mix64((uint64_t)i));
    const float u1 = ((float)(uint32_t)(r >> 40) + 1.0f) * (1.0f / 16777217.0f);
    const float u2 = (float)(uint32_t)((r >> 8) & 0xFFFFFF) * (1.0f / 16777216.0f);
    static_cast<float*>(j.out)[i0] = sqrtf(-2.f * logf(u1)) * cosf(6.283185307179586f * u2);
  } else {
    const uint64_t r = mix64(j.seed ^ mix64((uint64_t)i + 0x51ED270Bull));
    static_cast<uint8_t*>(j.out)[i0] = ((float)(uint32_t)(r >> 40) * (1.0f / 16777216.0f)) < j.keep ? 1 : 0;
  }
}
__global__ void gen_noise_kernel(Multi<NoiseJob> mv) {
  gen_one(mv.v[blockIdx.y], (long)blockIdx.x * 256 + threadIdx.x);
}
int gen_noise_multi(const NoiseJob* vs, int n, hipStream_t stream) {
  SERL_REQUIRE(n >= 1 && n <= kMaxMulti, "bad job count %d", n);
  Multi<NoiseJob> mv{};
  long nmax = 0;
  for (int i = 0; i < n; ++i) { mv.v[i] = vs[i]; nmax = std::max(nmax, vs[i].n); }
  SERL_LAUNCH_CHAIN(gen_noise_kernel, dim3(cdiv(nmax, 256), n), dim3(256), 0, stream, mv);
  SERL_HIP(hipGetLastError());
  return SERL_OK;
}
}
```

Before: 438.6 grad-steps/s.

## Compute only REDQ-selected target critic members and share duplicate encoder passes

The target critic forward now runs only the REDQ-sampled ensemble members, using per-group dense jobs with slab slots, instead of all ensemble groups. Duplicate encoder SLE/proprio jobs are merged so one pass writes both outputs. The policy-loss critic backward computes the input gradient only for the action columns. LayerNorm launches switch to a flattened variable-length grid, and host-side mask generation now uses the kernel's hash so both paths agree. This adds bookkeeping, and the mask RNG stream changes.

```diff
diff --git a/serl_amd/csrc/agent.hip b/serl_amd/csrc/agent.hip
--- a/serl_amd/csrc/agent.hip
+++ b/serl_amd/csrc/agent.hip
@@ -392,7 +392,18 @@
       RC(small_forward(a->sws, j.P, o.enc0, o.cam_stride, fr, Bfull, c.n_cam, cnt, j.e->f, (long)c.batch * a->D, st));
     }
   } else if (a->fuse) {
-    RC(sle_proprio_fwd_multi(sv, pv, n, 1.0f - c.dropout, cnt, a->HW, 512, c.n_cam, (long)c.batch * a->HW * 512, o.cam_stride,
+    SleFwdArgs s1[3], s2[3];
+    ProprioArgs p1[3];
+    int m = 0, first[3];
+    for (int i = 0; i < n; ++i) {
+      int k = 0;
+      while (k < m && !(!s2[k].f && !jobs[i].act_dst && jobs[first[k]].P == jobs[i].P && jobs[first[k]].which == jobs[i].which &&
+                        jobs[first[k]].x == jobs[i].x)) ++k;
+      if (k == m) { first[m] = i; s1[m] = sv[i]; s2[m] = SleFwdArgs{}; p1[m] = pv[i]; ++m; continue; }
+      s2[k] = sv[i];
+      p1[k].y2 = pv[i].y; p1[k].ld_y2 = pv[i].ld_y; p1[k].xhat2 = pv[i].xhat; p1[k].rstd2 = pv[i].rstd;
+    }
+    RC(sle_proprio_fwd_multi(s1, s2, p1, m, 1.0f - c.dropout, cnt, a->HW, 512, c.n_cam, (long)c.batch * a->HW * 512, o.cam_stride,
                              Bfull * a->D, (long)c.batch * a->D, c.state_dim, st));
   } else {
     RC(sle_fwd_multi(sv, n, 1.0f / (1.0f - c.dropout), cnt, a->HW, 512, c.n_cam, (long)c.batch * a->HW * 512, o.cam_stride,
@@ -415,19 +426,29 @@
 }
 
 struct RowDot { const float *w, *b; float* out; long w_gs, b_gs; };
-struct LayerJob { const float* P; DenseLnIo t; RowDot dot; DenseLnDrop drop; };
-int dense_ln_multi(serl_agent* a, const DenseLn& L, const LayerJob* jobs, int n, int rows, int smax, hipStream_t st) {
-  SERL_REQUIRE(n >= 1 && n <= 3, "bad dense instance count");
-  const int splitk = split_for(a->split_budget, rows, L.N, L.groups * n, smax);
+struct LayerJob {
+  const float* P; DenseLnIo t; RowDot dot; DenseLnDrop drop;
+  int group = -1, lane = -1, slot = 0;
+};
+int dense_ln_multi(serl_agent* a, const DenseLn& L, const LayerJob* jobs, int n, int rows, int smax, hipStream_t st, int whole = 0) {
+  SERL_REQUIRE(n >= 1 && n <= kMaxMulti && whole >= 0 && whole <= 3, "bad dense instance count");
+  const int splitk = split_for(a->split_budget, rows, L.N, L.groups * (whole ? whole : n), smax);
   SERL_REQUIRE((long)L.groups * splitk * rows * L.N <= a->slabs_cap,
                "Dense layer: %d groups x %d K-splits x %d rows x width %d exceeds the slab scratch of %ld floats", L.groups, splitk,
                rows, L.N, a->slabs_cap);
-  GemmDesc gd[3];
-  LnFwdArgs lv[3];
+  GemmDesc gd[kMaxMulti];
+  LnFwdArgs lv[kMaxMulti];
   for (int i = 0; i < n; ++i) {
-    const LayerJob& j = jobs[i];
-    gd[i] = layer_fwd(L, j.P, j.t, rows, a->slabs_lane[i], splitk);
-    lv[i] = layer_ln_fwd(L, j.P, j.t, rows, gd[i], j.drop);
+    LayerJob j = jobs[i];
+    const int lane = j.lane < 0 ? i : j.lane;
+    SERL_REQUIRE(lane < 3 && j.group < L.groups && j.slot >= 0 && j.slot < L.groups, "bad dense job (lane %d, group %d, slot %d)", lane, j.group, j.slot);
+    const DenseLn Lj = j.group < 0 ? L : layer_group(L, j.group);
+    if (j.group >= 0) {
+      j.t = io_group(L, j.t, j.group, rows);
+      if (j.dot.out) { j.dot.w += j.group * j.dot.w_gs; j.dot.b += j.group * j.dot.b_gs; j.dot.out += (long)j.group * rows; }
+    }
+    gd[i] = layer_fwd(Lj, j.P, j.t, rows, a->slabs_lane[lane] + (long)j.slot * splitk * rows * L.N, splitk);
+    lv[i] = layer_ln_fwd(Lj, j.P, j.t, rows, gd[i], j.drop);
     lv[i].dot_w = j.dot.w; lv[i].dot_b = j.dot.b; lv[i].dot_out = j.dot.out;
     lv[i].dot_gstride = j.dot.w_gs; lv[i].dot_b_gstride = j.dot.b_gs;
   }
@@ -507,20 +528,39 @@
   return policy_dist_fwd_multi(pv, n, cnt, A, c.std_min, c.std_max, st);
 }
 
-struct CritJob { const float* P; CritBuf* cb; DenseLnDrop drop[kL]; };
+struct MemberSet { int n; int m[kMaxMulti]; };
+struct CritJob { const float* P; CritBuf* cb; DenseLnDrop drop[kL]; MemberSet only = {}; };
+MemberSet redq_members(const serl_agent* a, const RedqSel& sel, int others) {
+  MemberSet s{};
+  if (sel.n <= 0 || sel.n >= a->cfg.ensemble || a->opts.critic.dropout > 0.0) return s;
+  for (int k = 0; k < sel.n; ++k) {
+    bool seen = false;
+    for (int i = 0; i < s.n; ++i) seen = seen || s.m[i] == sel.idx[k];
+    if (seen) continue;
+    if (s.n + others >= kMaxMulti) return MemberSet{};
+    s.m[s.n++] = sel.idx[k];
+  }
+  return s;
+}
 int critic_fwd_multi(serl_agent* a, const CritJob* jobs, int n, int cnt, hipStream_t st) {
   const Offs& o = a->o;
   SERL_REQUIRE(n >= 1 && n <= 3, "bad critic instance count");
   for (int l = 0; l < o.nc; ++l) {
-    LayerJob d[3];
+    LayerJob d[kMaxMulti];
+    int nd = 0;
     for (int i = 0; i < n; ++i) {
       const float* P = jobs[i].P;
       CritBuf& cb = *jobs[i].cb;
-      d[i] = LayerJob{P, l ? mlp_io(o.c[l], cb.m.l[l - 1], cb.m.l[l], cnt) : mlp_io(o.c[0], cb.x, a->XA, cb.m.l[0], cnt), {}, jobs[i].drop[l]};
+      const MemberSet& only = jobs[i].only;
+      LayerJob j{P, l ? mlp_io(o.c[l], cb.m.l[l - 1], cb.m.l[l], cnt) : mlp_io(o.c[0], cb.x, a->XA, cb.m.l[0], cnt), {}, jobs[i].drop[l]};
       if (l == o.nc - 1)
-        d[i].dot = RowDot{P + o.c_hw, P + o.c_hb, cb.q, a->state_only ? o.c[l].N : 0, a->state_only ? 1 : 0};
+        j.dot = RowDot{P + o.c_hw, P + o.c_hb, cb.q, a->state_only ? o.c[l].N : 0, a->state_only ? 1 : 0};
+      j.lane = i;
+      SERL_REQUIRE(nd + std::max(only.n, 1) <= kMaxMulti, "critic forward: more jobs than a launch has instances");
+      if (!only.n) d[nd++] = j;
+      for (int k = 0; k < only.n; ++k) { j.group = only.m[k]; j.slot = k; d[nd++] = j; }
     }
-    RC(dense_ln_multi(a, o.c[l], d, n, cnt, critic_smax(l), st));
+    RC(dense_ln_multi(a, o.c[l], d, nd, cnt, critic_smax(l), st, n));
   }
   return SERL_OK;
 }
@@ -619,7 +659,7 @@
 }
 
 int critic_bwd(serl_agent* a, const float* P, CritBuf& cb, int cnt, bool pg, hipStream_t st, const LossArgs* loss, float dq_const,
-               const DenseLnDrop* sites) {
+               const DenseLnDrop* sites, int col0 = 0, int ncol = 0) {
   const Offs& o = a->o;
   float* G = pg ? a->Gc : nullptr;
   const LossArgs* rider = nullptr;
@@ -632,7 +672,13 @@
     const DenseLnIo t = l ? mlp_io(o.c[l], cb.m.l[l - 1], cb.m.l[l], cnt) : mlp_io(o.c[0], cb.x, a->XA, cb.m.l[0], cnt);
     RC(dense_ln_bwd(a, o.c[l], P, t, d, cnt, G, st, l == top ? &head : nullptr, sites[l]));
     if (l) RC(gemm_f32(layer_igrad(o.c[l], P, d, cnt, mlp_grad(o.c[l - 1], a->s[l - 1], cnt)), st));
-    else return igrad_sum(a, layer_igrad(o.c[0], P, d, cnt, nullptr, 0, 0), a->dx, a->XA, st);
+    else if (!ncol) return igrad_sum(a, layer_igrad(o.c[0], P, d, cnt, nullptr, 0, 0), a->dx, a->XA, st);
+    else {
+      const DenseLn& L = o.c[0];
+      SERL_REQUIRE(col0 >= 0 && ncol > 0 && col0 + ncol <= L.K, "critic backward: input columns [%d, %d) of %d", col0, col0 + ncol, L.K);
+      return igrad_sum(a, gemm_igrad(d.dpre, L.N, (long)cnt * L.N, P + L.W + (long)col0 * L.N, L.N, L.w_gs, nullptr, 0, 0, L.groups, cnt,
+                                     ncol, L.N), a->dx + col0, a->XA, st);
+    }
   }
   return SERL_OK;
 }
@@ -1418,6 +1464,7 @@
             c.backup_entropy ? a->aux + X_ALPHA : nullptr};
   set_noise(a, ej[0], pj, nz, off, cnt, global_count);
   CritJob cj[2] = {{a->theta_t, &a->critT, {}}, {a->theta, &a->crit, {}}};
+  cj[0].only = redq_members(a, sel, 1);
   mlp_sites(a, SERL_SITE_PI_NEXT, a->opts.policy.dropout, off, cnt, global_count, redq_row, pj.drop);
   mlp_sites(a, SERL_SITE_Q_TARGET, a->opts.critic.dropout, off, cnt, global_count, redq_row, cj[0].drop);
   mlp_sites(a, SERL_SITE_Q_ONLINE, a->opts.critic.dropout, off, cnt, global_count, redq_row, cj[1].drop);
@@ -1470,7 +1517,7 @@
   RC(policy_fwd_multi(a, pj, 2, cnt, st));
   const float* eps_pi = nz[PI].eps ? nz[PI].eps : nz[PI].eps_out;
   RC(critic_fwd_multi(a, &cj, 1, cnt, st));
-  RC(critic_bwd(a, a->theta, a->crit, cnt, false, st, nullptr, -1.0f / ((float)c.ensemble * (float)global_count), cj.drop));
+  RC(critic_bwd(a, a->theta, a->crit, cnt, false, st, nullptr, -1.0f / ((float)c.ensemble * (float)global_count), cj.drop, a->E, A));
   RC(policy_dist_bwd(a->dx + a->E, a->XA, a->crit.x + a->E, a->XA, a->pol.pre, a->pol.std, eps_pi, a->aux + X_ALPHA,
                      1.0f / (float)global_count, cnt, A, c.std_min, c.std_max, a->dpre, a->crit.q, c.ensemble,
                      a->SC + S_QPI, st, a->pol_mode));
diff --git a/serl_amd/csrc/bc.hip b/serl_amd/csrc/bc.hip
--- a/serl_amd/csrc/bc.hip
+++ b/serl_amd/csrc/bc.hip
@@ -209,7 +209,7 @@
   sv.x = c->feats; sv.K = P + c->cam.first; sv.mask = mask; sv.f = c->f;
   if (!mask && mask_keys) sle_tf_masks(sv, mask_keys, g.n_cam, n, 0);
   const ProprioArgs pv = layer_row_fwd(c->prop, P, prop_io(c, state));
-  RC(sle_proprio_fwd_multi(&sv, &pv, 1, 1.0f - g.dropout, n, c->HW, 512, g.n_cam, (long)n * c->HW * 512, c->cam.stride,
+  RC(sle_proprio_fwd_multi(&sv, nullptr, &pv, 1, 1.0f - g.dropout, n, c->HW, 512, g.n_cam, (long)n * c->HW * 512, c->cam.stride,
                            (long)n * c->D, (long)n * c->D, g.state_dim, st));
   const int S0 = split_under(n, kBottleneck, g.n_cam, 32);
   const DenseLnIo tc{c->f, c->D, (long)n * c->D, c->enc, c->E, kBottleneck, nullptr, nullptr};
diff --git a/serl_amd/csrc/classifier.hip b/serl_amd/csrc/classifier.hip
--- a/serl_amd/csrc/classifier.hip
+++ b/serl_amd/csrc/classifier.hip
@@ -435,7 +435,7 @@
   for (int i = 0; i < ni; ++i) { sv[i].x = t->feats; sv[i].K = P + c->cam.first; sv[i].f = t->f + i * nc * nD; }
   sv[0].mask = masks;
   if (!masks) sle_tf_masks(sv[0], keys, nc, n, 0);
-  RC(sle_proprio_fwd_multi(sv, nullptr, ni, kKeep, n, c->HW, 512, nc, (long)n * c->HW * 512, c->cam.stride, nD, nD, 0, st));
+  RC(sle_proprio_fwd_multi(sv, nullptr, nullptr, ni, kKeep, n, c->HW, 512, nc, (long)n * c->HW * 512, c->cam.stride, nD, nD, 0, st));
   const int S0 = split_under(n, kBottleneck, nc * ni, 32);
   GemmDesc g0[2];
   LnFwdArgs l0[2];
diff --git a/serl_amd/csrc/dense_layer.h b/serl_amd/csrc/dense_layer.h
--- a/serl_amd/csrc/dense_layer.h
+++ b/serl_amd/csrc/dense_layer.h
@@ -48,6 +48,19 @@
   float* dy; long ld_dy, dy_goff;
   float *dpre, *dg;
 };
+
+inline DenseLn layer_group(DenseLn L, int m) {
+  L.W += m * L.w_gs; L.b += m * L.p_gs;
+  if (L.ln) { L.g += m * L.p_gs; L.be += m * L.p_gs; }
+  L.groups = 1;
+  return L;
+}
+inline DenseLnIo io_group(const DenseLn& L, DenseLnIo t, int m, int rows) {
+  t.x += m * t.x_gs; t.y += m * t.y_goff;
+  if (t.xhat) t.xhat += (long)m * rows * L.N;
+  if (t.rstd) t.rstd += (long)m * rows;
+  return t;
+}
 
 inline GemmDesc layer_fwd(const DenseLn& L, const float* P, const DenseLnIo& t, int rows, float* slabs, int splitk) {
   return gemm_fwd(t.x, t.ldx, t.x_gs, P + L.W, L.w_gs, slabs, L.groups, rows, L.N, L.K, splitk);
diff --git a/serl_amd/csrc/heads.h b/serl_amd/csrc/heads.h
--- a/serl_amd/csrc/heads.h
+++ b/serl_amd/csrc/heads.h
@@ -62,8 +62,8 @@
   uint32_t tf_key[4][2]; long tf_rows, tf_row0;
 };
 struct ProprioArgs;
-int sle_proprio_fwd_multi(const SleFwdArgs* v, const ProprioArgs* pv, int n, float keep, int N, int HW, int Cc, int groups, long x_gs,
-                          long k_gs, long mask_gs, long f_gs, int state_dim, hipStream_t stream);
+int sle_proprio_fwd_multi(const SleFwdArgs* v, const SleFwdArgs* v2, const ProprioArgs* pv, int n, float keep, int N, int HW, int Cc,
+                          int groups, long x_gs, long k_gs, long mask_gs, long f_gs, int state_dim, hipStream_t stream);
 int sle_fwd_multi(const SleFwdArgs* v, int n, float keep_scale, int N, int HW, int Cc, int groups, long x_gs, long k_gs,
                   long mask_gs, long f_gs, hipStream_t stream);
 int sle_bwd(const float* x, const float* df, float* partial, int N, int HW, int Cc, int nsplit, int groups,
@@ -86,6 +86,7 @@
   const float* state; const float *W, *b, *gamma, *beta;
   float* y; long ld_y; float* xhat; float* rstd;
   const float* copy_src; long ld_copy_src; float* copy_dst; long ld_copy_dst; int copy_cols;
+  float* y2; long ld_y2; float* xhat2; float* rstd2;
 };
 int proprio_fwd_multi(const ProprioArgs* v, int n, int S, int rows, hipStream_t stream);
 int policy_dist_bwd(const float* da, long ld_da, const float* act, long ld_act, const float* pre,
diff --git a/serl_amd/csrc/heads.hip b/serl_amd/csrc/heads.hip
--- a/serl_amd/csrc/heads.hip
+++ b/serl_amd/csrc/heads.hip
@@ -859,24 +859,35 @@
   return SERL_OK;
 }
 
+struct LnFwdMulti { LnFwdArgs v[kMaxMulti]; int xend[kMaxMulti]; };
+__device__ __forceinline__ const LnFwdArgs& ln_instance(const LnFwdMulti& mv, int& row) {
+  int i = 0, blk = blockIdx.x;
+  while (i + 1 < kMaxMulti && blk >= mv.xend[i]) ++i;
+  if (i) blk -= mv.xend[i - 1];
+  row = blk * 4 + (threadIdx.x >> 6);
+  return mv.v[i];
+}
 template <int VPL, bool BLOCKED>
-__global__ __launch_bounds__(256) void ln_fwd_kernel(Multi<LnFwdArgs> mv) {
-  const LnFwdArgs& a = mv.v[blockIdx.y];
-  const int row = blockIdx.x * 4 + (threadIdx.x >> 6), lane = threadIdx.x & 63;
+__global__ __launch_bounds__(256) void ln_fwd_kernel(LnFwdMulti mv) {
+  int row;
+  const LnFwdArgs& a = ln_instance(mv, row);
+  const int lane = threadIdx.x & 63;
   if (row >= a.rows) return;
   ln_row<VPL, BLOCKED>(a, row, lane);
 }
 template <int VPL, bool BLOCKED>
-__global__ __launch_bounds__(256) void ln_fwd_drop_kernel(Multi<LnFwdArgs> mv) {
-  const LnFwdArgs& a = mv.v[blockIdx.y];
-  const int row = blockIdx.x * 4 + (threadIdx.x >> 6), lane = threadIdx.x & 63;
+__global__ __launch_bounds__(256) void ln_fwd_drop_kernel(LnFwdMulti mv) {
+  int row;
+  const LnFwdArgs& a = ln_instance(mv, row);
+  const int lane = threadIdx.x & 63;
   if (row >= a.rows) return;
   ln_row<VPL, BLOCKED, true>(a, row, lane);
 }
 template <int VPL, bool BLOCKED>
-__global__ __launch_bounds__(256) void plain_fwd_kernel(Multi<LnFwdArgs> mv) {
-  const LnFwdArgs& a = mv.v[blockIdx.y];
-  const int row = blockIdx.x * 4 + (threadIdx.x >> 6), lane = threadIdx.x & 63;
+__global__ __launch_bounds__(256) void plain_fwd_kernel(LnFwdMulti mv) {
+  int row;
+  const LnFwdArgs& a = ln_instance(mv, row);
+  const int lane = threadIdx.x & 63;
   if (row >= a.rows) return;
   plain_row<VPL, BLOCKED>(a, row, lane);
 }
@@ -933,20 +944,23 @@
 int ln_fwd_multi(const LnFwdArgs* as, int n, int D, hipStream_t stream) {
   SERL_REQUIRE(SERL_LN_WIDTH_OK(D), "LayerNorm width %d unsupported (a multiple of 64 in [64, 1024])", D);
   SERL_REQUIRE(n >= 1 && n <= kMaxMulti, "bad instance count %d", n);
-  Multi<LnFwdArgs> mv{};
-  int rows = 0;
+  LnFwdMulti mv{};
+  int blocks = 0;
   bool drop = false;
   for (int i = 0; i < n; ++i) {
+    SERL_REQUIRE(as[i].rows >= 1, "LayerNorm row: instance %d has no row", i);
     SERL_REQUIRE(as[i].act >= 0 && as[i].act < kActCount, "LayerNorm row: activation code %d is not tanh (0), relu (1) or swish (2)", as[i].act);
     SERL_REQUIRE(ln_drop_ok(as[i].drop, as[i].rows_per_group), "LayerNorm row: bad Dropout description (mode %d, keep %g)", as[i].drop.mode, as[i].drop.keep);
     mv.v[i] = as[i];
-    rows = std::max(rows, as[i].rows);
+    blocks += cdiv(as[i].rows, 4);
+    mv.xend[i] = blocks;
     drop = drop || as[i].drop.mode != kLnDropNone;
     SERL_REQUIRE((as[i].gamma == nullptr) == (as[0].gamma == nullptr) && (as[i].gamma == nullptr) == (as[i].beta == nullptr),
                  "LayerNorm row: instance %d %s a LayerNorm and instance 0 %s; plain and LayerNorm rows do not share a launch", i,
                  as[i].gamma ? "has" : "lacks", as[0].gamma ? "has" : "lacks");
   }
-  dim3 grid(cdiv(rows, 4), n);
+  for (int i = n; i < kMaxMulti; ++i) mv.xend[i] = blocks;
+  dim3 grid(blocks);
   if (!as[0].gamma) {
     SERL_REQUIRE(!drop, "plain row (no LayerNorm) with Dropout: not served");
     SERL_LN_LAUNCH(D, (plain_fwd_kernel<1, false>), (plain_fwd_kernel<4, true>), plain_fwd_kernel, grid, dim3(256), 0, stream, mv)
@@ -1341,14 +1355,54 @@
   float mean, rstd;
   ln_mean_rstd<64>(s1, s2, mean, rstd);
   const float xh = (v - mean) * rstd;
-  a.y[(long)row * a.ld_y + lane] = tanhf(xh * a.gamma[lane] + a.beta[lane]);
+  const float y = tanhf(xh * a.gamma[lane] + a.beta[lane]);
+  a.y[(long)row * a.ld_y + lane] = y;
   if (a.xhat) a.xhat[(long)row * 64 + lane] = xh;
   if (a.rstd && lane == 0) a.rstd[row] = rstd;
+  if (a.y2) {
+    a.y2[(long)row * a.ld_y2 + lane] = y;
+    if (a.xhat2) a.xhat2[(long)row * 64 + lane] = xh;
+    if (a.rstd2 && lane == 0) a.rstd2[row] = rstd;
+  }
   if (a.copy_dst && lane < a.copy_cols) a.copy_dst[(long)row * a.ld_copy_dst + lane] = a.copy_src[(long)row * a.ld_copy_src + lane];
 }
 
+__device__ __forceinline__ void sle_hash_u24(uint64_t seed, uint64_t blk, unsigned (&u)[8]) {
+  const uint64_t ctr = blk * 3ull;
+  const uint64_t h0 = mix64(seed ^ mix64(ctr)), h1 = mix64(seed ^ mix64(ctr + 1)), h2 = mix64(seed ^ mix64(ctr + 2));
+  u[0] = (unsigned)(h0 & 0xFFFFFF); u[1] = (unsigned)((h0 >> 24) & 0xFFFFFF); u[2] = (unsigned)((h0 >> 48) | ((h1 & 0xFF) << 16));
+  u[3] = (unsigned)((h1 >> 8) & 0xFFFFFF); u[4] = (unsigned)((h1 >> 32) & 0xFFFFFF); u[5] = (unsigned)((h1 >> 56) | ((h2 & 0xFFFF) << 8));
+  u[6] = (unsigned)((h2 >> 16) & 0xFFFFFF); u[7] = (unsigned)(h2 >> 40);
+}
+__device__ __forceinline__ void sle_drop_store(const SleFwdArgs& v, const float (&acc)[8], int cam, int n, int c, int Cc, long ms,
+                                               long fs, float keep_scale, unsigned keep_thr, float keep_p) {
+  float o[8];
+  if (v.mask) {
+    const uint8_t* m = v.mask + cam * ms + (long)n * Cc * 8 + (long)c * 8;
+#pragma unroll
+    for (int j = 0; j < 8; ++j) o[j] = m[j] ? acc[j] * keep_scale : 0.f;
+  } else if (v.gen == 2) {
+    const uint32_t k0 = v.tf_key[cam][0], k1 = v.tf_key[cam][1];
+    const uint64_t rowlen = (uint64_t)Cc * 8ull, total = (uint64_t)v.tf_rows * rowlen;
+    const uint64_t e0 = (uint64_t)(v.tf_row0 + n) * rowlen + (uint64_t)c * 8ull;
+#pragma unroll
+    for (int j = 0; j < 8; ++j) o[j] = bits_to_unit(random_bits_at(k0, k1, total, e0 + (uint64_t)j)) < keep_p ? acc[j] * keep_scale : 0.f;
+  } else if (v.gen) {
+    unsigned u[8];
+    sle_hash_u24(v.seed, ((uint64_t)cam * (uint64_t)v.rows_global + (uint64_t)(v.row_offset + n)) * (uint64_t)Cc + (uint64_t)c, u);
+#pragma unroll
+    for (int j = 0; j < 8; ++j) o[j] = u[j] < keep_thr ? acc[j] * keep_scale : 0.f;
+  } else {
+#pragma unroll
+    for (int j = 0; j < 8; ++j) o[j] = acc[j];
+  }
+  float* f = v.f + cam * fs + (long)n * Cc * 8 + (long)c * 8;
+  *reinterpret_cast<float4*>(f) = make_float4(o[0], o[1], o[2], o[3]);
+  *reinterpret_cast<float4*>(f + 4) = make_float4(o[4], o[5], o[6], o[7]);
+}
+
 template <int kSleNb, int kPx>
-__global__ __launch_bounds__(256) void sle_proprio_fwd_kernel(Multi<SleFwdArgs> mv, Multi<ProprioArgs> pv, int has_proprio,
+__global__ __launch_bounds__(256) void sle_proprio_fwd_kernel(Multi<SleFwdArgs> mv, Multi<SleFwdArgs> mv2, Multi<ProprioArgs> pv, int has_proprio,
                                                               float keep_scale, unsigned keep_thr, float keep_p, int N, int HW, int Cc,
                                                               long xs, long ks, long ms, long fs, int S, int nb_sle) {
   if ((int)blockIdx.x >= nb_sle) {
@@ -1393,52 +1447,32 @@
       }
     }
   }
-  float* f = v.f + blockIdx.y * fs + (long)n0 * Cc * 8 + (long)c * 8;
-  const uint8_t* mask = v.mask ? v.mask + blockIdx.y * ms + (long)n0 * Cc * 8 + (long)c * 8 : nullptr;
+  const SleFwdArgs& v2 = mv2.v[blockIdx.z];
 #pragma unroll
   for (int s = 0; s < kSleNb; ++s) {
     if (s >= ns) break;
-    if (mask) {
-      const uint8_t* m = mask + (long)s * Cc * 8;
-#pragma unroll
-      for (int j = 0; j < 8; ++j) acc[s][j] = m[j] ? acc[s][j] * keep_scale : 0.f;
-    } else if (v.gen == 2) {
-      const uint32_t k0 = v.tf_key[blockIdx.y][0], k1 = v.tf_key[blockIdx.y][1];
-      const uint64_t rowlen = (uint64_t)Cc * 8ull, total = (uint64_t)v.tf_rows * rowlen;
-      const uint64_t e0 = (uint64_t)(v.tf_row0 + n0 + s) * rowlen + (uint64_t)c * 8ull;
-#pragma unroll
-      for (int j = 0; j < 8; ++j)
-        acc[s][j] = bits_to_unit(random_bits_at(k0, k1, total, e0 + (uint64_t)j)) < keep_p ? acc[s][j] * keep_scale : 0.f;
-    } else if (v.gen) {
-      const uint64_t ctr = (((uint64_t)blockIdx.y * (uint64_t)v.rows_global + (uint64_t)(v.row_offset + n0 + s)) * (uint64_t)Cc + (uint64_t)c) * 3ull;
-      const uint64_t h0 = mix64(v.seed ^ mix64(ctr)), h1 = mix64(v.seed ^ mix64(ctr + 1)), h2 = mix64(v.seed ^ mix64(ctr + 2));
-      const unsigned u[8] = {(unsigned)(h0 & 0xFFFFFF), (unsigned)((h0 >> 24) & 0xFFFFFF), (unsigned)((h0 >> 48) | ((h1 & 0xFF) << 16)),
-                             (unsigned)((h1 >> 8) & 0xFFFFFF), (unsigned)((h1 >> 32) & 0xFFFFFF), (unsigned)((h1 >> 56) | ((h2 & 0xFFFF) << 8)),
-                             (unsigned)((h2 >> 16) & 0xFFFFFF), (unsigned)(h2 >> 40)};
-#pragma unroll
-      for (int j = 0; j < 8; ++j) acc[s][j] = u[j] < keep_thr ? acc[s][j] * keep_scale : 0.f;
-    }
-    *reinterpret_cast<float4*>(f + (long)s * Cc * 8) = make_float4(acc[s][0], acc[s][1], acc[s][2], acc[s][3]);
-    *reinterpret_cast<float4*>(f + (long)s * Cc * 8 + 4) = make_float4(acc[s][4], acc[s][5], acc[s][6], acc[s][7]);
-  }
-}
-
-int sle_proprio_fwd_multi(const SleFwdArgs* vs, const ProprioArgs* ps, int n, float keep, int N, int HW, int Cc, int groups, long x_gs,
-                          long k_gs, long mask_gs, long f_gs, int state_dim, hipStream_t stream) {
+    sle_drop_store(v, acc[s], blockIdx.y, n0 + s, c, Cc, ms, fs, keep_scale, keep_thr, keep_p);
+    if (v2.f) sle_drop_store(v2, acc[s], blockIdx.y, n0 + s, c, Cc, ms, fs, keep_scale, keep_thr, keep_p);
+  }
+}
+
+int sle_proprio_fwd_multi(const SleFwdArgs* vs, const SleFwdArgs* vs2, const ProprioArgs* ps, int n, float keep, int N, int HW, int Cc,
+                          int groups, long x_gs, long k_gs, long mask_gs, long f_gs, int state_dim, hipStream_t stream) {
   SERL_REQUIRE(n >= 1 && n <= kMaxMulti, "bad instance count %d", n);
-  Multi<SleFwdArgs> mv{};
+  Multi<SleFwdArgs> mv{}, mv2{};
   Multi<ProprioArgs> pv{};
   for (int i = 0; i < n; ++i) {
     mv.v[i] = vs[i];
+    if (vs2) mv2.v[i] = vs2[i];
     if (ps) { pv.v[i] = ps[i]; SERL_REQUIRE(!ps[i].copy_dst || ps[i].copy_cols <= 64, "copy_cols > 64"); }
   }
   const int nb = N <= 64 ? 2 : 4;
   const int nb_sle = cdiv(Cc, 256) * cdiv(N, nb), nb_prop = ps ? cdiv(N, 4) : 0;
   if (nb == 2)
-    SERL_LAUNCH_CHAIN((sle_proprio_fwd_kernel<2, 4>), dim3(nb_sle + nb_prop, groups, n), dim3(256), 0, stream, mv, pv, ps ? 1 : 0,
+    SERL_LAUNCH_CHAIN((sle_proprio_fwd_kernel<2, 4>), dim3(nb_sle + nb_prop, groups, n), dim3(256), 0, stream, mv, mv2, pv, ps ? 1 : 0,
                       1.0f / keep, (unsigned)(keep * 16777216.0f), keep, N, HW, Cc, x_gs, k_gs, mask_gs, f_gs, state_dim, nb_sle);
   else
-    SERL_LAUNCH_CHAIN((sle_proprio_fwd_kernel<4, 2>), dim3(nb_sle + nb_prop, groups, n), dim3(256), 0, stream, mv, pv, ps ? 1 : 0,
+    SERL_LAUNCH_CHAIN((sle_proprio_fwd_kernel<4, 2>), dim3(nb_sle + nb_prop, groups, n), dim3(256), 0, stream, mv, mv2, pv, ps ? 1 : 0,
                       1.0f / keep, (unsigned)(keep * 16777216.0f), keep, N, HW, Cc, x_gs, k_gs, mask_gs, f_gs, state_dim, nb_sle);
   SERL_HIP(hipGetLastError());
   return SERL_OK;
@@ -1975,8 +2009,12 @@
     const float u2 = (float)(uint32_t)((r >> 8) & 0xFFFFFF) * (1.0f / 16777216.0f);
     static_cast<float*>(j.out)[i0] = sqrtf(-2.f * logf(u1)) * cosf(6.283185307179586f * u2);
   } else {
-    const uint64_t r = mix64(j.seed ^ mix64((uint64_t)i + 0x51ED270Bull));
-    static_cast<uint8_t*>(j.out)[i0] = ((float)(uint32_t)(r >> 40) * (1.0f / 16777216.0f)) < j.keep ? 1 : 0;
+    unsigned u[8];
+    sle_hash_u24(j.seed, (uint64_t)(i / 8), u);
+    unsigned mine = 0;
+#pragma unroll
+    for (int k = 0; k < 8; ++k) mine = (i % 8) == k ? u[k] : mine;
+    static_cast<uint8_t*>(j.out)[i0] = mine < (unsigned)(j.keep * 16777216.0f) ? 1 : 0;
   }
 }
 __global__ void gen_noise_kernel(Multi<NoiseJob> mv) {
```

Result: no change. 440.8 grad-steps/s, median of 6 (+0.5%).
